# nyashiki/nshogi-engine

Hardware: NVIDIA B200
Metric: nn_leaf_evals_per_sec_batch256 (higher is better)
Workload: dtype bf16

## Files before the change

include/nsb_diag.h:

```cpp
#ifndef NSB_DIAG_H
#define NSB_DIAG_H

#include "nsb.h"

#ifdef __cplusplus
extern "C" {
#endif
#if defined(__GNUC__)
#pragma GCC visibility push(default)
#endif

int nsb_debug_trunk_timeline(nsb_ctx* ctx, int slot, const nsb_feature_bitboard* d_features, size_t n,
                             uint64_t* host_stamps, size_t max_stamps);
int nsb_debug_trunk_timeline_positions(nsb_ctx* ctx, int slot, const nsb_position* d_positions, size_t n,
                                       uint64_t* host_stamps, size_t max_stamps);

int nsb_debug_umma_probe(int gpu, int n_cols, int k_elems, int shift_rows, int layout, int iters,
                         float* max_err, double* cycles_per_mma);

int nsb_debug_bulk_rate_probe(int gpu, int ctas, int tile_bytes, int stages, int split, double* bytes_per_cycle);

#if defined(__GNUC__)
#pragma GCC visibility pop
#endif
#ifdef __cplusplus
}
#endif
#endif
```

nshogi-engine_b200/binding.py:

```python
from __future__ import annotations

import ctypes as C
import os
from typing import Optional

import numpy as np

HERE = os.path.dirname(os.path.abspath(__file__))
LIB_PATH = os.path.join(HERE, "libnsb.so")

NUM_SQUARES = 81
POLICY_SIZE = 2187
FEATURE_CHANNELS = 86
MAX_LEGAL_MOVES = 593
CACHE_MAX_MOVES = 164
DECODE_PROBS = 0
DECODE_LOGITS = 1
DECODE_BOTH = 2
DECODE_NAN_FALLBACK = 0x100
ROW_SKIP_SOFTMAX = 1

FEATURE_BITBOARD = np.dtype([("lo", "<u8"), ("hi", "<u8")])
POSITION = np.dtype(
    {
        "names": ["board", "side", "hands", "ply", "max_ply", "black_draw_value", "white_draw_value"],
        "formats": [("u1", (81,)), "u1", ("u1", (2, 7)), "<u2", "<u2", "<f4", "<f4"],
        "offsets": [0, 81, 82, 96, 98, 100, 104],
        "itemsize": 108,
    }
)


class NetDesc(C.Structure):
    _fields_ = [("in_channels", C.c_int32), ("channels", C.c_int32), ("blocks", C.c_int32),
                ("value_hidden", C.c_int32)]


class NsbError(RuntimeError):
    pass


_lib = None

_P = C.c_void_p
SIGNATURES = {
    "nsb_create": (C.c_int, [C.POINTER(_P), C.c_int, C.c_int, C.c_int, C.POINTER(NetDesc)]),
    "nsb_destroy": (None, [_P]),
    "nsb_bind_thread": (C.c_int, [_P]),
    "nsb_weight_blob_floats": (C.c_size_t, [C.POINTER(NetDesc)]),
    "nsb_weight_blob_random": (C.c_int, [C.POINTER(NetDesc), C.c_uint64, _P]),
    "nsb_load_weights": (C.c_int, [_P, _P, C.c_size_t]),
    "nsb_eval_async": (C.c_int, [_P, C.c_int, _P, C.c_size_t, _P, _P, _P]),
    "nsb_eval_decode_async": (C.c_int, [_P, C.c_int, _P, C.c_size_t, _P, _P, C.c_int, _P, _P, _P, _P]),
    "nsb_eval_positions_async": (C.c_int, [_P, C.c_int, _P, C.c_size_t, _P, _P, _P]),
    "nsb_eval_positions_decode_async": (C.c_int, [_P, C.c_int, _P, C.c_size_t, _P, _P, C.c_int, _P, _P, _P, _P]),
    "nsb_await": (C.c_int, [_P, C.c_int]),
    "nsb_is_computing": (C.c_int, [_P, C.c_int]),
    "nsb_eval_device": (C.c_int, [_P, C.c_int, _P, C.c_size_t, _P, _P, _P]),
    "nsb_eval_decode_device": (C.c_int, [_P, C.c_int, _P, C.c_size_t, _P, _P, C.c_int, _P, _P, _P, _P, _P]),
    "nsb_extract_device": (C.c_int, [_P, C.c_int, _P, C.c_size_t, C.c_int, C.c_int, _P]),
    "nsb_pack_positions_device": (C.c_int, [_P, C.c_int, _P, C.c_size_t, _P]),
    "nsb_decode_device": (C.c_int, [_P, C.c_int, _P, _P, _P, C.c_size_t, _P, _P, C.c_int, _P, _P]),
    "nsb_decode_device_ex": (C.c_int, [_P, C.c_int, _P, _P, _P, C.c_size_t, _P, _P, C.c_int, _P, _P, _P, _P]),
    "nsb_cache_create": (C.c_int, [_P, C.c_size_t]),
    "nsb_cache_clear": (C.c_int, [_P]),
    "nsb_cache_num_bundles": (C.c_uint64, [_P]),
    "nsb_cache_store_device": (C.c_int, [_P, C.c_int, _P, C.c_size_t, _P, _P, _P, _P, _P, _P]),
    "nsb_cache_probe_device": (C.c_int, [_P, C.c_int, _P, C.c_size_t, _P, _P, _P, _P, _P, _P, _P]),
    "nsb_eval_cached_decode_async": (C.c_int, [_P, C.c_int, _P, C.c_size_t, _P, _P, _P, C.c_int, _P, _P, _P, _P, _P]),
    "nsb_eval_positions_cached_decode_async": (C.c_int, [_P, C.c_int, _P, C.c_size_t, _P, _P, _P, C.c_int, _P, _P, _P, _P,
                                                         _P]),
    "nsb_eval_cached_decode_device": (C.c_int, [_P, C.c_int, _P, C.c_size_t, _P, _P, _P, C.c_int, _P, _P, _P, _P, _P]),
    "nsb_stream": (_P, [_P, C.c_int]),
    "nsb_set_timing": (C.c_int, [_P, C.c_int]),
    "nsb_trunk_time": (C.c_int, [_P, C.POINTER(C.c_double), C.POINTER(C.c_uint64)]),
    "nsb_trunk_time_reset": (C.c_int, [_P]),
    "nsb_launch_count": (C.c_uint64, [_P]),
    "nsb_trunk_kernel_name": (C.c_char_p, [_P]),
    "nsb_host_register": (C.c_int, [_P, C.c_size_t]),
    "nsb_host_unregister": (C.c_int, [_P]),
    "nsb_eval_request_async": (C.c_int, [_P, C.c_int, _P]),
    "nsb_cache_attach": (C.c_int, [_P, _P]),
    "nsb_set_io_mode": (C.c_int, [_P, C.c_int]),
    "nsb_io_mode": (C.c_int, [_P]),
    "nsb_host_alloc": (C.c_int, [C.POINTER(_P), C.c_size_t]),
    "nsb_host_free": (C.c_int, [_P]),
    "nsb_host_alloc_near": (C.c_int, [C.POINTER(_P), C.c_size_t, C.c_int]),
    "nsb_gpu_numa_node": (C.c_int, [C.c_int]),
    "nsb_numa_bind_thread": (C.c_int, [C.c_int]),
    "nsb_device_alloc": (C.c_int, [C.POINTER(_P), C.c_size_t]),
    "nsb_device_free": (C.c_int, [_P]),
    "nsb_memcpy_h2d": (C.c_int, [_P, _P, C.c_size_t]),
    "nsb_memcpy_d2h": (C.c_int, [_P, _P, C.c_size_t]),
    "nsb_memset_device": (C.c_int, [_P, C.c_int, C.c_size_t]),
    "nsb_device_sync": (C.c_int, []),
    "nsb_last_error": (C.c_char_p, []),
    "nsb_version": (C.c_char_p, []),
    "nsb_device_count": (C.c_int, []),
    "nsb_umma_selftest": (C.c_int, [C.c_int, C.c_int, C.c_int, C.c_int, C.POINTER(C.c_float), C.POINTER(C.c_float)]),
    "nsb_event_create": (C.c_int, [C.POINTER(_P)]),
    "nsb_event_destroy": (C.c_int, [_P]),
    "nsb_event_record": (C.c_int, [_P, _P, C.c_int]),
    "nsb_event_sync": (C.c_int, [_P]),
    "nsb_event_elapsed_ms": (C.c_int, [_P, _P, C.POINTER(C.c_float)]),
}


DIAG_SIGNATURES = {
    "nsb_debug_trunk_timeline": (C.c_int, [_P, C.c_int, _P, C.c_size_t, _P, C.c_size_t]),
    "nsb_debug_trunk_timeline_positions": (C.c_int, [_P, C.c_int, _P, C.c_size_t, _P, C.c_size_t]),
    "nsb_debug_umma_probe": (C.c_int, [C.c_int, C.c_int, C.c_int, C.c_int, C.c_int, C.c_int, C.POINTER(C.c_float),
                                       C.POINTER(C.c_double)]),
    "nsb_debug_bulk_rate_probe": (C.c_int, [C.c_int, C.c_int, C.c_int, C.c_int, C.c_int, C.POINTER(C.c_double)]),
}
DIAG_LIB_PATH = os.path.join(HERE, "libnsb_diag.so")
_diag = None


def diag_lib() -> C.CDLL:
    global _diag
    if _diag is None:
        if not os.path.exists(DIAG_LIB_PATH):
            raise NsbError(f"{DIAG_LIB_PATH} not built")
        l = C.CDLL(DIAG_LIB_PATH)
        for name, (res, args) in {**SIGNATURES, **DIAG_SIGNATURES}.items():
            fn = getattr(l, name)
            fn.restype = res
            fn.argtypes = args
        _diag = l
    return _diag


def lib() -> C.CDLL:
    global _lib
    if _lib is None:
        if not os.path.exists(LIB_PATH):
            raise NsbError(f"{LIB_PATH} not built: run `python -c 'import __graft_entry__ as g; g.build()'` "
                           "(there is no CPU fallback)")
        l = C.CDLL(LIB_PATH)
        for name, (res, args) in SIGNATURES.items():
            fn = getattr(l, name)
            fn.restype = res
            fn.argtypes = args
        _lib = l
    return _lib


def _check(rc: int, what: str) -> None:
    if rc != 0:
        msg = lib().nsb_last_error().decode()
        if _diag is not None and _diag.nsb_last_error():
            msg = msg or _diag.nsb_last_error().decode()
        raise NsbError(f"{what} failed ({rc}): {msg}")


def _ptr(a) -> Optional[int]:
    if a is None:
        return None
    if isinstance(a, np.ndarray):
        assert a.flags["C_CONTIGUOUS"], "host buffers must be C-contiguous"
        return a.ctypes.data
    return int(a)


def device_count() -> int:
    return lib().nsb_device_count()


def net_desc(channels: int, blocks: int, value_hidden: int = 256, in_channels: int = FEATURE_CHANNELS) -> NetDesc:
    return NetDesc(in_channels, channels, blocks, value_hidden)


def random_blob(desc: NetDesc, seed: int) -> np.ndarray:
    n = lib().nsb_weight_blob_floats(C.byref(desc))
    blob = np.empty(n, dtype=np.float32)
    _check(lib().nsb_weight_blob_random(C.byref(desc), seed, blob.ctypes.data), "nsb_weight_blob_random")
    return blob


class PinnedArray:

    def __init__(self, shape, dtype, gpu: Optional[int] = None):
        self.dtype = np.dtype(dtype)
        self.shape = tuple(shape) if isinstance(shape, (tuple, list)) else (int(shape),)
        nbytes = int(np.prod(self.shape)) * self.dtype.itemsize
        p = _P()
        if gpu is None:
            _check(lib().nsb_host_alloc(C.byref(p), nbytes), "nsb_host_alloc")
        else:
            _check(lib().nsb_host_alloc_near(C.byref(p), nbytes, gpu), "nsb_host_alloc_near")
        self._p = p
        buf = (C.c_uint8 * max(nbytes, 1)).from_address(p.value)
        self.array = np.frombuffer(buf, dtype=self.dtype, count=int(np.prod(self.shape))).reshape(self.shape)

    def free(self):
        if self._p is not None:
            self.array = None
            lib().nsb_host_free(self._p)
            self._p = None


class DecodeRequest(C.Structure):
    _fields_ = [("features", _P), ("positions", _P), ("n", C.c_size_t), ("hashes", _P), ("move_off", _P), ("move_idx", _P),
                ("mode", C.c_int), ("legal_out", _P), ("order_out", _P), ("win", _P), ("draw", _P), ("nan_flag", _P),
                ("hit_flag", _P), ("row_flags", _P), ("logits_out", _P)]


def host_register(arr: np.ndarray) -> bool:
    rc = lib().nsb_host_register(arr.ctypes.data, arr.nbytes)
    if rc < 0:
        _check(rc, "nsb_host_register")
    return rc == 0


def host_unregister(arr: np.ndarray):
    _check(lib().nsb_host_unregister(arr.ctypes.data), "nsb_host_unregister")


class DeviceBuffer:
    def __init__(self, nbytes: int):
        p = _P()
        _check(lib().nsb_device_alloc(C.byref(p), nbytes), "nsb_device_alloc")
        self.ptr = p.value
        self.nbytes = nbytes

    @classmethod
    def from_host(cls, a: np.ndarray) -> "DeviceBuffer":
        a = np.ascontiguousarray(a)
        d = cls(max(a.nbytes, 1))
        if a.nbytes:
            _check(lib().nsb_memcpy_h2d(d.ptr, a.ctypes.data, a.nbytes), "nsb_memcpy_h2d")
        return d

    def to_host(self, shape, dtype) -> np.ndarray:
        out = np.empty(shape, dtype=dtype)
        assert out.nbytes <= self.nbytes
        if out.nbytes:
            _check(lib().nsb_memcpy_d2h(out.ctypes.data, self.ptr, out.nbytes), "nsb_memcpy_d2h")
        return out

    def fill(self, byte: int):
        _check(lib().nsb_memset_device(self.ptr, byte, self.nbytes), "nsb_memset_device")

    def free(self):
        if self.ptr:
            lib().nsb_device_free(self.ptr)
            self.ptr = None


def gpu_numa_node(gpu: int = 0) -> int:
    return lib().nsb_gpu_numa_node(gpu)


def numa_bind_thread(gpu: int = 0) -> bool:
    return lib().nsb_numa_bind_thread(gpu) == 0


def device_sync():
    _check(lib().nsb_device_sync(), "nsb_device_sync")


def umma_selftest(n_cols: int, k_elems: int, shift_rows: int, gpu: int = 0):
    err, epi = C.c_float(-1.0), C.c_float(-1.0)
    _check(lib().nsb_umma_selftest(gpu, n_cols, k_elems, shift_rows, C.byref(err), C.byref(epi)),
           "nsb_umma_selftest")
    return float(err.value), float(epi.value)


def umma_probe(n_cols, k_elems, shift_rows, layout, iters=20, gpu=0):
    err, cyc = C.c_float(-1.0), C.c_double(0)
    _check(diag_lib().nsb_debug_umma_probe(gpu, n_cols, k_elems, shift_rows, layout, iters, C.byref(err), C.byref(cyc)),
           "nsb_debug_umma_probe")
    return float(err.value), float(cyc.value)


def bulk_rate_probe(ctas, tile_bytes, stages, split, gpu=0):
    v = C.c_double(0)
    _check(diag_lib().nsb_debug_bulk_rate_probe(gpu, ctas, tile_bytes, stages, split, C.byref(v)), "nsb_debug_bulk_rate_probe")
    return float(v.value)


class Event:

    def __init__(self):
        p = _P()
        _check(lib().nsb_event_create(C.byref(p)), "nsb_event_create")
        self._p = p

    def record(self, ctx: "Context", slot: int = 0):
        _check(ctx._l.nsb_event_record(self._p, ctx._h, slot), "nsb_event_record")

    def sync(self):
        _check(lib().nsb_event_sync(self._p), "nsb_event_sync")

    def elapsed_ms(self, stop: "Event") -> float:
        ms = C.c_float(0)
        _check(lib().nsb_event_elapsed_ms(self._p, stop._p, C.byref(ms)), "nsb_event_elapsed_ms")
        return float(ms.value)

    def destroy(self):
        if self._p is not None:
            lib().nsb_event_destroy(self._p)
            self._p = None


class Context:

    def __init__(self, desc: NetDesc, batch_max: int, slots: int = 1, gpu: int = 0,
                 blob: Optional[np.ndarray] = None, seed: Optional[int] = None, diag: bool = False):
        self.desc = desc
        self.batch_max = batch_max
        self.slots = slots
        self._l = diag_lib() if diag else lib()
        h = _P()
        _check(self._l.nsb_create(C.byref(h), gpu, batch_max, slots, C.byref(desc)), "nsb_create")
        self._h = h
        if blob is None and seed is not None:
            blob = random_blob(desc, seed)
        if blob is not None:
            self.load_weights(blob)

    def close(self):
        if self._h is not None:
            self._l.nsb_destroy(self._h)
            self._h = None

    def __enter__(self):
        return self

    def __exit__(self, *a):
        self.close()

    def load_weights(self, blob: np.ndarray):
        blob = np.ascontiguousarray(blob, dtype=np.float32)
        _check(self._l.nsb_load_weights(self._h, blob.ctypes.data, blob.size), "nsb_load_weights")

    def bind_thread(self):
        _check(self._l.nsb_bind_thread(self._h), "nsb_bind_thread")

    def eval_async(self, slot, features, n, policy, win, draw):
        _check(self._l.nsb_eval_async(self._h, slot, _ptr(features), n, _ptr(policy), _ptr(win), _ptr(draw)),
               "nsb_eval_async")

    def eval_decode_async(self, slot, features, n, move_off, move_idx, mode, legal_out, win, draw, nan_flag=None):
        _check(self._l.nsb_eval_decode_async(self._h, slot, _ptr(features), n, _ptr(move_off), _ptr(move_idx), mode,
                                           _ptr(legal_out), _ptr(win), _ptr(draw), _ptr(nan_flag)),
               "nsb_eval_decode_async")

    def eval_positions_async(self, slot, positions, n, policy, win, draw):
        _check(self._l.nsb_eval_positions_async(self._h, slot, _ptr(positions), n, _ptr(policy), _ptr(win),
                                              _ptr(draw)), "nsb_eval_positions_async")

    def eval_positions_decode_async(self, slot, positions, n, move_off, move_idx, mode, legal_out, win, draw,
                                    nan_flag=None):
        _check(self._l.nsb_eval_positions_decode_async(self._h, slot, _ptr(positions), n, _ptr(move_off),
                                                     _ptr(move_idx), mode, _ptr(legal_out), _ptr(win), _ptr(draw),
                                                     _ptr(nan_flag)), "nsb_eval_positions_decode_async")

    def await_(self, slot=0):
        _check(self._l.nsb_await(self._h, slot), "nsb_await")

    def is_computing(self, slot=0) -> bool:
        rc = self._l.nsb_is_computing(self._h, slot)
        if rc < 0:
            _check(rc, "nsb_is_computing")
        return rc == 1

    def eval_device(self, slot, d_features, n, d_policy, d_win, d_draw):
        _check(self._l.nsb_eval_device(self._h, slot, _ptr(d_features), n, _ptr(d_policy), _ptr(d_win), _ptr(d_draw)),
               "nsb_eval_device")

    def eval_decode_device(self, slot, d_features, n, d_off, d_idx, mode, d_policy, d_legal, d_win, d_draw, d_flag):
        _check(self._l.nsb_eval_decode_device(self._h, slot, _ptr(d_features), n, _ptr(d_off), _ptr(d_idx), mode,
                                            _ptr(d_policy), _ptr(d_legal), _ptr(d_win), _ptr(d_draw), _ptr(d_flag)),
               "nsb_eval_decode_device")

    def extract_device(self, slot, d_features, n, channels, channels_first, d_planes):
        _check(self._l.nsb_extract_device(self._h, slot, _ptr(d_features), n, channels, int(channels_first),
                                        _ptr(d_planes)), "nsb_extract_device")

    def pack_positions_device(self, slot, d_positions, n, d_features):
        _check(self._l.nsb_pack_positions_device(self._h, slot, _ptr(d_positions), n, _ptr(d_features)),
               "nsb_pack_positions_device")

    def decode_device(self, slot, d_policy, d_win, d_draw, n, d_off, d_idx, mode, d_legal, d_flag):
        _check(self._l.nsb_decode_device(self._h, slot, _ptr(d_policy), _ptr(d_win), _ptr(d_draw), n, _ptr(d_off),
                                       _ptr(d_idx), mode, _ptr(d_legal), _ptr(d_flag)), "nsb_decode_device")

    def decode_device_ex(self, slot, d_policy, d_win, d_draw, n, d_off, d_idx, mode, d_row_flags, d_legal, d_logits, d_flag):
        _check(self._l.nsb_decode_device_ex(self._h, slot, _ptr(d_policy), _ptr(d_win), _ptr(d_draw), n, _ptr(d_off),
                                          _ptr(d_idx), mode, _ptr(d_row_flags), _ptr(d_legal), _ptr(d_logits), _ptr(d_flag)),
               "nsb_decode_device_ex")

    def cache_create(self, memory_mb: int):
        _check(self._l.nsb_cache_create(self._h, memory_mb), "nsb_cache_create")

    def cache_clear(self):
        _check(self._l.nsb_cache_clear(self._h), "nsb_cache_clear")

    def cache_num_bundles(self) -> int:
        return int(self._l.nsb_cache_num_bundles(self._h))

    def cache_store_device(self, slot, d_hashes, n, d_off, d_legal, d_win, d_draw, d_skip=None, d_stored=None):
        _check(self._l.nsb_cache_store_device(self._h, slot, _ptr(d_hashes), n, _ptr(d_off), _ptr(d_legal), _ptr(d_win),
                                            _ptr(d_draw), _ptr(d_skip), _ptr(d_stored)), "nsb_cache_store_device")

    def cache_probe_device(self, slot, d_hashes, n, d_off, d_legal, d_win, d_draw, d_hit, d_miss_idx, d_miss_count):
        _check(self._l.nsb_cache_probe_device(self._h, slot, _ptr(d_hashes), n, _ptr(d_off), _ptr(d_legal), _ptr(d_win),
                                            _ptr(d_draw), _ptr(d_hit), _ptr(d_miss_idx), _ptr(d_miss_count)),
               "nsb_cache_probe_device")

    def eval_cached_decode_async(self, slot, features, n, hashes, move_off, move_idx, mode, legal_out, win, draw,
                                 nan_flag=None, hit_flag=None):
        _check(self._l.nsb_eval_cached_decode_async(self._h, slot, _ptr(features), n, _ptr(hashes), _ptr(move_off),
                                                  _ptr(move_idx), mode, _ptr(legal_out), _ptr(win), _ptr(draw),
                                                  _ptr(nan_flag), _ptr(hit_flag)), "nsb_eval_cached_decode_async")

    def eval_positions_cached_decode_async(self, slot, positions, n, hashes, move_off, move_idx, mode, legal_out, win,
                                           draw, nan_flag=None, hit_flag=None):
        _check(self._l.nsb_eval_positions_cached_decode_async(self._h, slot, _ptr(positions), n, _ptr(hashes),
                                                            _ptr(move_off), _ptr(move_idx), mode, _ptr(legal_out),
                                                            _ptr(win), _ptr(draw), _ptr(nan_flag), _ptr(hit_flag)),
               "nsb_eval_positions_cached_decode_async")

    def eval_cached_decode_device(self, slot, d_features, n, d_hashes, d_off, d_idx, mode, d_legal, d_win, d_draw,
                                  d_flag, d_hit):
        _check(self._l.nsb_eval_cached_decode_device(self._h, slot, _ptr(d_features), n, _ptr(d_hashes), _ptr(d_off),
                                                   _ptr(d_idx), mode, _ptr(d_legal), _ptr(d_win), _ptr(d_draw),
                                                   _ptr(d_flag), _ptr(d_hit)), "nsb_eval_cached_decode_device")

    def debug_trunk_timeline(self, slot, d_features, n, positions=False):
        nl = 2 * self.desc.blocks + 2
        out = np.zeros(nl * 4 + 16 + 3 * 1024, dtype=np.uint64)
        fn = self._l.nsb_debug_trunk_timeline_positions if positions else self._l.nsb_debug_trunk_timeline
        _check(fn(self._h, slot, _ptr(d_features), n, out.ctypes.data, out.size), "nsb_debug_trunk_timeline")
        return out[:nl * 4].reshape(nl, 4), out[nl * 4:]

    def eval_request_async(self, slot, n, move_off, move_idx, mode, legal_out, win, draw, features=None, positions=None,
                           hashes=None, order_out=None, nan_flag=None, hit_flag=None, row_flags=None, logits_out=None):
        r = DecodeRequest(_ptr(features), _ptr(positions), n, _ptr(hashes), _ptr(move_off), _ptr(move_idx), mode,
                          _ptr(legal_out), _ptr(order_out), _ptr(win), _ptr(draw), _ptr(nan_flag), _ptr(hit_flag),
                          _ptr(row_flags), _ptr(logits_out))
        _check(self._l.nsb_eval_request_async(self._h, slot, C.byref(r)), "nsb_eval_request_async")

    def cache_attach(self, owner: "Context"):
        _check(self._l.nsb_cache_attach(self._h, owner._h), "nsb_cache_attach")

    def set_io_mode(self, direct: bool):
        _check(self._l.nsb_set_io_mode(self._h, 1 if direct else 0), "nsb_set_io_mode")

    def io_mode(self) -> str:
        return "direct" if self._l.nsb_io_mode(self._h) == 1 else "staged"

    def stream(self, slot=0) -> int:
        return self._l.nsb_stream(self._h, slot) or 0

    def set_timing(self, on: bool):
        _check(self._l.nsb_set_timing(self._h, int(on)), "nsb_set_timing")

    def trunk_time(self):
        s, n = C.c_double(0), C.c_uint64(0)
        _check(self._l.nsb_trunk_time(self._h, C.byref(s), C.byref(n)), "nsb_trunk_time")
        return float(s.value), int(n.value)

    def trunk_time_reset(self):
        _check(self._l.nsb_trunk_time_reset(self._h), "nsb_trunk_time_reset")

    def trunk_kernel_name(self) -> str:
        return self._l.nsb_trunk_kernel_name(self._h).decode()

    def launch_count(self) -> int:
        return int(self._l.nsb_launch_count(self._h))
```

nshogi-engine_b200/csrc/epilogue.cuh:

```cuda
#pragma once
#include <stdint.h>

#include "umma.cuh"

namespace nsb {

__host__ __device__ constexpr bool is_real_slot(int n) { return (n % 100) < 90 && ((n % 100) % 10) < 9; }

template <int NCG>
struct EpilogueMask {
    uint32_t m[NCG * 4];
    template <int COL0>
    __device__ __forceinline__ void init_at(int lane) {
#pragma unroll
        for (int G = 0; G < NCG * 4; ++G) {
            uint32_t v = 0;
#pragma unroll
            for (int q4 = 0; q4 < 4; ++q4) {
                const int n = COL0 + 8 * G + 2 * q4;
                const uint32_t c = (is_real_slot(n) ? 0x0000FFFFu : 0u) | (is_real_slot(n + 1) ? 0xFFFF0000u : 0u);
                v = (lane & 3) == q4 ? c : v;
            }
            m[G] = v;
        }
    }
    __device__ __forceinline__ void init(int col0, int lane) {
        if (col0 == 0) init_at<0>(lane);
        else init_at<96>(lane);
    }
};

template <int NCG, bool kResidual, int LBS = 2>
__device__ __forceinline__ void epilogue_half(int lb, uint32_t taddr, uint32_t buf, uint32_t pitch, int chunk0,
                                              int col0, const float (&bias)[4], const EpilogueMask<NCG>& mask,
                                              int lane) {
    const int mk = lane >> 3, mi = lane & 7;
    uint32_t v[NCG][16];
#pragma unroll
    for (int cg = 0; cg < NCG; ++cg) tmem_ld_16x256b_x4(taddr + ((uint32_t)(lb * 16) << 16) + cg * 32, v[cg]);
    const uint32_t row_addr =
        buf + (uint32_t)(chunk0 + lb * LBS + (mk & 1)) * pitch + (uint32_t)(col0 + 8 * (mk >> 1) + mi) * 16u;
    uint32_t xr[NCG][2][4];
    if (kResidual) {
#pragma unroll
        for (int cg = 0; cg < NCG; ++cg)
#pragma unroll
            for (int h = 0; h < 2; ++h)
                ldmatrix_x4_trans(row_addr + (uint32_t)(cg * 32 + h * 16) * 16u, xr[cg][h][0], xr[cg][h][1],
                                  xr[cg][h][2], xr[cg][h][3]);
    }
    tmem_ld_wait();
    const float b0 = lb ? bias[2] : bias[0], b1 = lb ? bias[3] : bias[1];
    const uint64_t bb0 = pack_f32x2(b0, b0), bb1 = pack_f32x2(b1, b1);
#pragma unroll
    for (int cg = 0; cg < NCG; ++cg)
#pragma unroll
        for (int h = 0; h < 2; ++h) {
            uint32_t p[4];
#pragma unroll
            for (int m = 0; m < 4; ++m) {
                const int g = 2 * h + (m >> 1), rh = m & 1;
                uint64_t x = add_f32x2(pack_u32x2(v[cg][4 * g + 2 * rh + 0], v[cg][4 * g + 2 * rh + 1]), rh ? bb1 : bb0);
                if (kResidual) x = add_f32x2(x, pack_u32x2(xr[cg][h][m] << 16, xr[cg][h][m] & 0xFFFF0000u));
                p[m] = pack_relu_bf16x2(x) & mask.m[cg * 4 + g];
            }
            stmatrix_x4_trans(row_addr + (uint32_t)(cg * 32 + h * 16) * 16u, p[0], p[1], p[2], p[3]);
        }
}

template <int NCG, bool kResidual>
__device__ __forceinline__ void epilogue_warp(uint32_t taddr, uint32_t buf, uint32_t pitch, int chunk0, int col0,
                                              const float (&bias)[4], const EpilogueMask<NCG>& mask, int lane) {
#pragma unroll
    for (int lb = 0; lb < 2; ++lb)
        epilogue_half<NCG, kResidual>(lb, taddr, buf, pitch, chunk0, col0, bias, mask, lane);
}

}
```

nshogi-engine_b200/csrc/nsb_api.cu:

```cuda
#include <cuda_runtime.h>
#include <stdarg.h>
#include <stdio.h>
#include <stdlib.h>
#include <string.h>

#include <map>
#include <mutex>
#include <new>
#include <vector>

#include "nsb_internal.h"
#ifdef NSB_DIAG
#include "../../include/nsb_diag.h"
#endif

namespace nsb {

static thread_local char g_err[512] = "";

void set_error(const char* fmt, ...) {
    va_list ap;
    va_start(ap, fmt);
    vsnprintf(g_err, sizeof g_err, fmt, ap);
    va_end(ap);
}

static std::mutex g_host_mu;
enum class HostKind { Alloc, NodeAlloc, Registered, Adopted };
struct HostRange {
    size_t bytes = 0;
    bool direct = true;
    HostKind kind = HostKind::Alloc;
};
static std::map<uintptr_t, HostRange> g_host_allocs;

static bool host_mapped(const void* p, size_t bytes) {
    if (p == nullptr) return false;
    const uintptr_t a = (uintptr_t)p;
    std::lock_guard<std::mutex> lock(g_host_mu);
    auto it = g_host_allocs.upper_bound(a);
    if (it == g_host_allocs.begin()) return false;
    --it;
    return it->second.direct && a + bytes <= it->first + it->second.bytes;
}

struct Slot {
    cudaStream_t stream = nullptr;
    nsb_feature_bitboard* d_feat = nullptr;
    nsb_position* d_pos = nullptr;
    float *d_policy = nullptr, *d_win = nullptr, *d_draw = nullptr, *d_legal = nullptr;
    uint32_t* d_off = nullptr;
    uint16_t* d_idx = nullptr;
    uint16_t* d_order = nullptr;
    uint8_t* d_flag = nullptr;
    uint8_t* d_rowflags = nullptr;
    float* d_logits = nullptr;
    uint64_t* d_hash = nullptr;
    uint8_t* d_hit = nullptr;
    int* d_miss_idx = nullptr;
    int* d_miss_count = nullptr;
    std::vector<cudaEvent_t> ev;
    size_t ev_used = 0;
};

}

struct nsb_ctx {
    int gpu = 0, batch_max = 0, num_sms = 0;
    int max_pairs = 0;
    bool use_ts = false;
    bool direct_io = false;
    bool fuse_pack = true;
    int duo_ctas = 0;
    int cluster128 = 1;
    bool duo_always = false;
    bool quad = false;
    nsb::DeviceNet net_duo{};
    void* d_duo_tiles = nullptr;
    double t_classic_wave = 0.129, t_duo_single = 0.157, t_duo_pair = 0.215;
    bool calibrated = false;
    nsb::DeviceCache cache{};
    bool cache_owned = false;
    nsb_net_desc desc{};
    bool loaded = false, timing = false;
    nsb::DeviceNet net{};
    void* d_weights[6] = {nullptr, nullptr, nullptr, nullptr, nullptr, nullptr};
    std::vector<nsb::Slot> slots;
    uint64_t launches = 0;
    double trunk_ms = 0.0;
    uint64_t trunk_launches = 0;
};

using namespace nsb;

#define NSB_CUDA(call)                                                                        \
    do {                                                                                      \
        cudaError_t e__ = (call);                                                             \
        if (e__ != cudaSuccess) {                                                             \
            set_error("%s failed: %s (%s:%d)", #call, cudaGetErrorString(e__), __FILE__, __LINE__); \
            return NSB_ERR_CUDA;                                                              \
        }                                                                                     \
    } while (0)

static int check_ctx(nsb_ctx* c, int slot) {
    if (!c) {
        set_error("null ctx");
        return NSB_ERR_INVALID;
    }
    if (slot < 0 || slot >= (int)c->slots.size()) {
        set_error("slot %d out of range [0,%d)", slot, (int)c->slots.size());
        return NSB_ERR_INVALID;
    }
    return 0;
}

static int check_batch(nsb_ctx* c, size_t n, bool need_weights) {
    if (n > (size_t)c->batch_max) {
        set_error("batch %zu exceeds batch_max %d", n, c->batch_max);
        return NSB_ERR_INVALID;
    }
    if (need_weights && !c->loaded) {
        set_error("weights not loaded (call nsb_load_weights first)");
        return NSB_ERR_STATE;
    }
    return 0;
}

static bool mode_ok(int mode) {
    const int kind = mode & NSB_DECODE_MODE_MASK;
    return (mode & ~(NSB_DECODE_MODE_MASK | NSB_DECODE_NAN_FALLBACK)) == 0 &&
           (kind == NSB_DECODE_PROBS || kind == NSB_DECODE_LOGITS || kind == NSB_DECODE_BOTH);
}

static int check_offsets(const uint32_t* off, size_t n, const char* who) {
    if (off[0] != 0) {
        set_error("%s: move_off must start at 0", who);
        return NSB_ERR_INVALID;
    }
    for (size_t i = 0; i < n; ++i) {
        if (off[i + 1] < off[i] || off[i + 1] - off[i] > (uint32_t)NSB_MAX_LEGAL_MOVES) {
            set_error("%s: move_off[%zu..%zu] = %u..%u: rows must hold 0..%d moves", who, i, i + 1, off[i], off[i + 1],
                      NSB_MAX_LEGAL_MOVES);
            return NSB_ERR_INVALID;
        }
    }
    return 0;
}

static int check_positions_net(const nsb_ctx* c, const char* who) {
    if (c->desc.in_channels != NSB_FEATURE_CHANNELS) {
        set_error("%s: packed positions expand to the %d planes of SimpleFeatures; this net takes %d channels (feed bitboards)",
                  who, NSB_FEATURE_CHANNELS, c->desc.in_channels);
        return NSB_ERR_INVALID;
    }
    return 0;
}

static bool dense_outputs_mapped(size_t n, const float* policy, const float* win, const float* draw) {
    return host_mapped(policy, n * kPolicySize * sizeof(float)) && host_mapped(win, n * sizeof(float)) &&
           host_mapped(draw, n * sizeof(float));
}

extern "C" {

const char* nsb_last_error(void) { return g_err; }
const char* nsb_version(void) { return "nsb 0.3 (sm_100a: tcgen05 position-stationary trunk, cta_group::2 pair trunk, device-resident eval cache)"
#ifdef NSB_DIAG
           " [diagnostic build]"
#endif
        ; }

int nsb_device_count(void) {
    int n = 0;
    if (cudaGetDeviceCount(&n) != cudaSuccess) {
        cudaGetLastError();
        return 0;
    }
    return n;
}

int nsb_create(nsb_ctx** out, int gpu, int batch_max, int slots, const nsb_net_desc* net) {
    if (!out || !net || batch_max <= 0 || batch_max > 65535 || slots < 1 || slots > 16) {
        set_error("nsb_create: bad arguments (batch_max 1..65535, slots 1..16)");
        return NSB_ERR_INVALID;
    }
    if ((net->channels != 128 && net->channels != 192 && net->channels != 256) || net->blocks < 1 || net->blocks > 80 ||
        net->in_channels < 1 || net->in_channels > kMaxInChannels || net->value_hidden < 1 ||
        net->value_hidden > kMaxHidden) {
        set_error("nsb_create: unsupported net (channels 128|192|256, blocks 1..80, in_channels<=%d, hidden<=%d)",
                  kMaxInChannels, kMaxHidden);
        return NSB_ERR_INVALID;
    }
    int ndev = 0;
    if (cudaGetDeviceCount(&ndev) != cudaSuccess || gpu < 0 || gpu >= ndev) {
        cudaGetLastError();
        set_error("nsb_create: no CUDA device %d (found %d); this library has no CPU fallback", gpu, ndev);
        return NSB_ERR_NO_DEVICE;
    }
    cudaDeviceProp prop;
    NSB_CUDA(cudaGetDeviceProperties(&prop, gpu));
    if (prop.major != 10) {
        set_error("nsb_create: device %d is sm_%d%d; the kernels are built for sm_100a only", gpu, prop.major,
                  prop.minor);
        return NSB_ERR_NO_DEVICE;
    }
    NSB_CUDA(cudaSetDevice(gpu));
    int rc = trunk_fused_prepare(net->channels);
    if (rc) return rc;
    int max_pairs = 0;
    const char* t256 = getenv("NSB_TRUNK256");
    const char* t128 = getenv("NSB_TRUNK128");
#ifndef NSB_DIAG
    if ((t256 && strcmp(t256, "single") == 0) || (t128 && strcmp(t128, "ts") == 0)) {
        set_error("nsb_create: NSB_TRUNK256=single / NSB_TRUNK128=ts exist in the diagnostic build only (libnsb_diag.so)");
        return NSB_ERR_INVALID;
    }
#endif
    if (net->channels == 192 || (net->channels == 256 && !(t256 && strcmp(t256, "single") == 0))) {
        if ((rc = trunk_pair_prepare(net->channels, &max_pairs))) return rc;
        if (max_pairs > prop.multiProcessorCount / 2) max_pairs = prop.multiProcessorCount / 2;
    }
    const bool is128 = net->channels == 128;
    const bool use_ts = is128 && t128 && strcmp(t128, "ts") == 0;
    const int cluster128 = (is128 && t128 && strcmp(t128, "mc2") == 0) ? 2 : (is128 && t128 && strcmp(t128, "mc4") == 0) ? 4 : 1;
    const bool want_quad = is128 && (t128 ? strcmp(t128, "quad") == 0 : slots >= 4);
    const bool want_duo = is128 && !use_ts && !want_quad && (t128 ? strcmp(t128, "duo") == 0 : true);
    const bool duo_always = want_duo && (t128 ? true : slots >= 2);
#ifdef NSB_DIAG
    if (use_ts && (rc = trunk_ts_prepare())) return rc;
#endif
    int duo_ctas = 0;
    if (want_duo && (rc = trunk_duo_prepare(&duo_ctas))) return rc;
    if (want_quad && (rc = trunk_quad_prepare())) return rc;
    nsb_ctx* c = new (std::nothrow) nsb_ctx();
    if (!c) {
        set_error("out of host memory");
        return NSB_ERR_NOMEM;
    }
    c->gpu = gpu;
    c->batch_max = batch_max;
    c->num_sms = prop.multiProcessorCount;
    c->max_pairs = max_pairs;
    c->use_ts = use_ts;
    c->duo_ctas = duo_ctas;
    c->duo_always = duo_always;
    c->quad = want_quad;
    c->cluster128 = cluster128;
    if (const char* dc = getenv("NSB_DUO_CTAS")) c->duo_ctas = duo_ctas > 0 ? atoi(dc) : 0;
    if (const char* fp = getenv("NSB_FUSE_PACK")) c->fuse_pack = strcmp(fp, "0") != 0;
    c->direct_io = slots == 1;
    if (const char* io = getenv("NSB_IO")) c->direct_io = strcmp(io, "direct") == 0;
    c->desc = *net;
    c->slots.resize(slots);
    const size_t B = (size_t)batch_max;
    for (auto& s : c->slots) {
        cudaError_t e = cudaStreamCreateWithFlags(&s.stream, cudaStreamNonBlocking);
        if (e == cudaSuccess) e = cudaMalloc(&s.d_feat, B * (size_t)net->in_channels * sizeof(nsb_feature_bitboard));
        if (e == cudaSuccess) e = cudaMalloc(&s.d_pos, B * sizeof(nsb_position));
        if (e == cudaSuccess) e = cudaMalloc(&s.d_policy, B * kPolicySize * sizeof(float));
        if (e == cudaSuccess) e = cudaMalloc(&s.d_win, B * sizeof(float));
        if (e == cudaSuccess) e = cudaMalloc(&s.d_draw, B * sizeof(float));
        if (e == cudaSuccess) e = cudaMalloc(&s.d_legal, B * NSB_MAX_LEGAL_MOVES * sizeof(float));
        if (e == cudaSuccess) e = cudaMalloc(&s.d_off, (B + 1) * sizeof(uint32_t));
        if (e == cudaSuccess) e = cudaMalloc(&s.d_idx, B * NSB_MAX_LEGAL_MOVES * sizeof(uint16_t));
        if (e == cudaSuccess) e = cudaMalloc(&s.d_order, B * NSB_MAX_LEGAL_MOVES * sizeof(uint16_t));
        if (e == cudaSuccess) e = cudaMalloc(&s.d_flag, B);
        if (e == cudaSuccess) e = cudaMalloc(&s.d_rowflags, B);
        if (e != cudaSuccess) {
            set_error("nsb_create: device allocation failed: %s", cudaGetErrorString(e));
            nsb_destroy(c);
            return e == cudaErrorMemoryAllocation ? NSB_ERR_NOMEM : NSB_ERR_CUDA;
        }
    }
    *out = c;
    return 0;
}

void nsb_destroy(nsb_ctx* c) {
    if (!c) return;
    cudaSetDevice(c->gpu);
    for (auto& s : c->slots) {
        if (s.stream) cudaStreamSynchronize(s.stream);
        cudaFree(s.d_feat); cudaFree(s.d_pos); cudaFree(s.d_policy); cudaFree(s.d_win); cudaFree(s.d_draw);
        cudaFree(s.d_legal); cudaFree(s.d_off); cudaFree(s.d_idx); cudaFree(s.d_order); cudaFree(s.d_flag); cudaFree(s.d_rowflags); cudaFree(s.d_logits);
        cudaFree(s.d_hash); cudaFree(s.d_hit); cudaFree(s.d_miss_idx); cudaFree(s.d_miss_count);
        for (cudaEvent_t e : s.ev) cudaEventDestroy(e);
        if (s.stream) cudaStreamDestroy(s.stream);
    }
    for (void* p : c->d_weights) cudaFree(p);
    cudaFree(c->d_duo_tiles);
    if (c->cache_owned) {
        cudaFree(c->cache.entries);
        cudaFree(c->cache.meta);
    }
    delete c;
}

int nsb_bind_thread(nsb_ctx* c) {
    if (!c) {
        set_error("null ctx");
        return NSB_ERR_INVALID;
    }
    NSB_CUDA(cudaSetDevice(c->gpu));
    return 0;
}

size_t nsb_weight_blob_floats(const nsb_net_desc* net) { return net ? blob_floats(*net) : 0; }

int nsb_weight_blob_random(const nsb_net_desc* net, uint64_t seed, float* blob) {
    if (!net || !blob) {
        set_error("nsb_weight_blob_random: null argument");
        return NSB_ERR_INVALID;
    }
    blob_random(*net, seed, blob);
    return 0;
}

static int calibrate_kernel_choice(nsb_ctx* c);

int nsb_load_weights(nsb_ctx* c, const float* blob, size_t n_floats) {
    if (!c || !blob) {
        set_error("nsb_load_weights: null argument");
        return NSB_ERR_INVALID;
    }
    if (n_floats != blob_floats(c->desc)) {
        set_error("nsb_load_weights: blob has %zu floats, net needs %zu", n_floats, blob_floats(c->desc));
        return NSB_ERR_INVALID;
    }
    NSB_CUDA(cudaSetDevice(c->gpu));
    for (auto& s : c->slots) NSB_CUDA(cudaStreamSynchronize(s.stream));
    c->loaded = false;
    const nsb_net_desc& d = c->desc;
    const int C = d.channels, H = d.value_hidden, NL = 2 * d.blocks + 2;
    int stages = stages_per_pass(d);
    std::vector<uint16_t> tiles((size_t)stages * kStageBytes / 2);
    std::vector<float> bias((size_t)NL * C), fc1t((size_t)81 * H), fc1b(H), fc2(2 * (size_t)H), fc2b(2);
    pack_weights(d, blob, tiles.data(), bias.data(), fc1t.data(), fc1b.data(), fc2.data(), fc2b.data());
    const bool ts_only = c->use_ts || c->quad || (c->duo_ctas > 0 && c->duo_always);
    std::vector<uint16_t> ts_tiles;
    int ts_stages = 0;
    if (ts_only || c->duo_ctas > 0) {
        ts_stages = ts_steps_per_pass(d);
        ts_tiles.assign((size_t)ts_stages * 2048, 0);
        pack_weights_ts(d, blob, ts_tiles.data());
        if (ts_only) {
            stages = ts_stages;
            tiles.swap(ts_tiles);
        }
    }
    const void* src[6] = {tiles.data(), bias.data(), fc1t.data(), fc1b.data(), fc2.data(), fc2b.data()};
    const size_t bytes[6] = {tiles.size() * 2, bias.size() * 4, fc1t.size() * 4, fc1b.size() * 4, fc2.size() * 4,
                             fc2b.size() * 4};
    for (int i = 0; i < 6; ++i) {
        if (c->d_weights[i]) {
            cudaFree(c->d_weights[i]);
            c->d_weights[i] = nullptr;
        }
        NSB_CUDA(cudaMalloc(&c->d_weights[i], bytes[i]));
        NSB_CUDA(cudaMemcpy(c->d_weights[i], src[i], bytes[i], cudaMemcpyHostToDevice));
    }
    DeviceNet& n = c->net;
    n.channels = C;
    n.blocks = d.blocks;
    n.in_channels = d.in_channels;
    n.stem_steps = stem_steps(d.in_channels);
    n.hidden = H;
    n.num_layers = NL;
    n.stages_per_pass = stages;
    n.tiles = static_cast<const uint8_t*>(c->d_weights[0]);
    n.bias = static_cast<const float*>(c->d_weights[1]);
    n.fc1t = static_cast<const float*>(c->d_weights[2]);
    n.fc1b = static_cast<const float*>(c->d_weights[3]);
    n.fc2 = static_cast<const float*>(c->d_weights[4]);
    n.fc2b = static_cast<const float*>(c->d_weights[5]);
    if (c->duo_ctas > 0 && !c->duo_always) {
        cudaFree(c->d_duo_tiles);
        c->d_duo_tiles = nullptr;
        NSB_CUDA(cudaMalloc(&c->d_duo_tiles, ts_tiles.size() * 2));
        NSB_CUDA(cudaMemcpy(c->d_duo_tiles, ts_tiles.data(), ts_tiles.size() * 2, cudaMemcpyHostToDevice));
        c->net_duo = n;
        c->net_duo.stages_per_pass = ts_stages;
        c->net_duo.tiles = static_cast<const uint8_t*>(c->d_duo_tiles);
    } else {
        c->net_duo = n;
    }
    c->loaded = true;
    return calibrate_kernel_choice(c);
}

static bool use_duo(const nsb_ctx* c, int n) {
    if (c->duo_ctas <= 0) return false;
    if (c->duo_always) return true;
    const int groups = (n + 1) / 2, sms = c->num_sms;
    const double classic = c->t_classic_wave * ((groups + sms - 1) / sms);
    const int full = groups / (2 * sms), rest = groups % (2 * sms);
    const double duo = c->t_duo_pair * full + (rest == 0 ? 0.0 : rest <= sms ? c->t_duo_single : c->t_duo_pair);
    return duo < classic;
}

static int calibrate_kernel_choice(nsb_ctx* c) {
    const int sms = c->num_sms;
    if (c->duo_ctas <= 0 || c->duo_always || c->batch_max <= 2 * sms) return 0;
    Slot& s = c->slots[0];
    const int n_wave = 2 * sms, n_pair = c->batch_max < 4 * sms ? c->batch_max : 4 * sms;
    NSB_CUDA(cudaMemsetAsync(s.d_feat, 0, (size_t)n_pair * c->desc.in_channels * sizeof(nsb_feature_bitboard), s.stream));
    cudaEvent_t e0, e1;
    NSB_CUDA(cudaEventCreate(&e0));
    NSB_CUDA(cudaEventCreate(&e1));
    auto best_of = [&](bool duo, int n, double* out) -> int {
        EvalArgs a{};
        a.features = s.d_feat;
        a.n = n;
        a.win = s.d_win;
        a.draw = s.d_draw;
        float best = 1e30f;
        for (int it = 0; it < 4; ++it) {
            NSB_CUDA(cudaEventRecord(e0, s.stream));
            const int k = duo ? launch_trunk_duo(c->net_duo, a, sms, c->duo_ctas, s.stream) : launch_trunk_fused(c->net, a, sms, s.stream);
            if (k < 0) return k;
            NSB_CUDA(cudaGetLastError());
            NSB_CUDA(cudaEventRecord(e1, s.stream));
            NSB_CUDA(cudaEventSynchronize(e1));
            float ms = 0.f;
            NSB_CUDA(cudaEventElapsedTime(&ms, e0, e1));
            if (it > 0 && ms < best) best = ms;
        }
        *out = best;
        return 0;
    };
    int rc = best_of(false, n_wave, &c->t_classic_wave);
    if (!rc) rc = best_of(true, n_wave, &c->t_duo_single);
    if (!rc) rc = best_of(true, n_pair, &c->t_duo_pair);
    cudaEventDestroy(e0);
    cudaEventDestroy(e1);
    c->calibrated = rc == 0;
    return rc;
}


static int run_trunk(nsb_ctx* c, Slot& s, const EvalArgs& a) {
    if (c->timing) {
        while (s.ev.size() < s.ev_used + 2) {
            cudaEvent_t e;
            NSB_CUDA(cudaEventCreate(&e));
            s.ev.push_back(e);
        }
        NSB_CUDA(cudaEventRecord(s.ev[s.ev_used], s.stream));
    }
    int k = c->max_pairs > 0 ? launch_trunk_pair(c->net, a, c->max_pairs, s.stream)
            : c->quad        ? launch_trunk_quad(c->net, a, c->num_sms, s.stream)
            : use_duo(c, a.n) ? launch_trunk_duo(c->net_duo, a, c->num_sms, c->duo_ctas, s.stream)
#ifdef NSB_DIAG
            : c->use_ts      ? launch_trunk_ts(c->net, a, c->num_sms, s.stream)
#endif
                             : launch_trunk_fused(c->net, a, c->num_sms, s.stream, c->cluster128);
    if (k < 0) return k;
    NSB_CUDA(cudaGetLastError());
    c->launches += (uint64_t)k;
    if (c->timing) {
        NSB_CUDA(cudaEventRecord(s.ev[s.ev_used + 1], s.stream));
        s.ev_used += 2;
    }
    return 0;
}

static int harvest_timing(nsb_ctx* c, Slot& s) {
    for (size_t i = 0; i + 1 < s.ev_used; i += 2) {
        float ms = 0.f;
        NSB_CUDA(cudaEventElapsedTime(&ms, s.ev[i], s.ev[i + 1]));
        c->trunk_ms += ms;
        c->trunk_launches += 1;
    }
    s.ev_used = 0;
    return 0;
}


int nsb_eval_async(nsb_ctx* c, int slot, const nsb_feature_bitboard* features, size_t n, float* policy,
                   float* win, float* draw) {
    int rc = check_ctx(c, slot);
    if (rc) return rc;
    if ((rc = check_batch(c, n, true))) return rc;
    if (!features || !policy || !win || !draw) {
        set_error("nsb_eval_async: null buffer");
        return NSB_ERR_INVALID;
    }
    if (n == 0) return 0;
    Slot& s = c->slots[slot];
    if (c->direct_io && host_mapped(features, n * (size_t)c->desc.in_channels * sizeof(nsb_feature_bitboard)) &&
        dense_outputs_mapped(n, policy, win, draw)) {
        EvalArgs a{};
        a.features = features;
        a.n = (int)n;
        a.policy = policy;
        a.win = win;
        a.draw = draw;
        return run_trunk(c, s, a);
    }
    NSB_CUDA(cudaMemcpyAsync(s.d_feat, features, n * (size_t)c->desc.in_channels * sizeof(nsb_feature_bitboard),
                             cudaMemcpyHostToDevice, s.stream));
    EvalArgs a{};
    a.features = s.d_feat;
    a.n = (int)n;
    a.policy = s.d_policy;
    a.win = s.d_win;
    a.draw = s.d_draw;
    if ((rc = run_trunk(c, s, a))) return rc;
    NSB_CUDA(cudaMemcpyAsync(policy, s.d_policy, n * kPolicySize * sizeof(float), cudaMemcpyDeviceToHost,
                             s.stream));
    NSB_CUDA(cudaMemcpyAsync(win, s.d_win, n * sizeof(float), cudaMemcpyDeviceToHost, s.stream));
    NSB_CUDA(cudaMemcpyAsync(draw, s.d_draw, n * sizeof(float), cudaMemcpyDeviceToHost, s.stream));
    return 0;
}

static bool decode_buffers_mapped(size_t n, size_t total, const uint32_t* move_off, const uint16_t* move_idx,
                                  const float* legal_out, const float* win, const float* draw, const uint8_t* nan_flag) {
    return host_mapped(move_off, (n + 1) * sizeof(uint32_t)) && host_mapped(move_idx, (total ? total : 1) * sizeof(uint16_t)) &&
           host_mapped(legal_out, (total ? total : 1) * sizeof(float)) && host_mapped(win, n * sizeof(float)) &&
           host_mapped(draw, n * sizeof(float)) && (nan_flag == nullptr || host_mapped(nan_flag, n));
}

static int stage1(nsb_ctx* c, Slot& s, size_t n, const nsb_position** fused) {
    if (c->fuse_pack) {
        *fused = s.d_pos;
        return 0;
    }
    *fused = nullptr;
    int k = launch_pack_positions(s.d_pos, n, s.d_feat, s.stream);
    if (k < 0) return k;
    NSB_CUDA(cudaGetLastError());
    c->launches += (uint64_t)k;
    return 0;
}

static int eval_request(nsb_ctx* c, int slot, const nsb_decode_request& r, const char* who);

int nsb_eval_request_async(nsb_ctx* c, int slot, const nsb_decode_request* request) {
    if (!request) {
        set_error("nsb_eval_request_async: null request");
        return NSB_ERR_INVALID;
    }
    return eval_request(c, slot, *request, "nsb_eval_request_async");
}

int nsb_eval_decode_async(nsb_ctx* c, int slot, const nsb_feature_bitboard* features, size_t n,
                          const uint32_t* move_off, const uint16_t* move_idx, int mode, float* legal_out,
                          float* win, float* draw, uint8_t* nan_flag) {
    nsb_decode_request r{};
    r.features = features;
    r.n = n;
    r.move_off = move_off;
    r.move_idx = move_idx;
    r.mode = mode;
    r.legal_out = legal_out;
    r.win = win;
    r.draw = draw;
    r.nan_flag = nan_flag;
    if (!features) {
        set_error("nsb_eval_decode_async: null buffer or bad mode");
        return NSB_ERR_INVALID;
    }
    return eval_request(c, slot, r, "nsb_eval_decode_async");
}

int nsb_eval_positions_async(nsb_ctx* c, int slot, const nsb_position* positions, size_t n, float* policy,
                             float* win, float* draw) {
    int rc = check_ctx(c, slot);
    if (rc) return rc;
    if ((rc = check_batch(c, n, true))) return rc;
    if (!positions || !policy || !win || !draw) {
        set_error("nsb_eval_positions_async: null buffer");
        return NSB_ERR_INVALID;
    }
    if ((rc = check_positions_net(c, "nsb_eval_positions_async"))) return rc;
    if (n == 0) return 0;
    Slot& s = c->slots[slot];
    if (c->direct_io && c->fuse_pack && host_mapped(positions, n * sizeof(nsb_position)) &&
        dense_outputs_mapped(n, policy, win, draw)) {
        EvalArgs a{};
        a.positions = positions;
        a.n = (int)n;
        a.policy = policy;
        a.win = win;
        a.draw = draw;
        return run_trunk(c, s, a);
    }
    NSB_CUDA(cudaMemcpyAsync(s.d_pos, positions, n * sizeof(nsb_position), cudaMemcpyHostToDevice, s.stream));
    const nsb_position* fused = nullptr;
    if ((rc = stage1(c, s, n, &fused))) return rc;
    EvalArgs a{};
    a.features = s.d_feat;
    a.positions = fused;
    a.n = (int)n;
    a.policy = s.d_policy;
    a.win = s.d_win;
    a.draw = s.d_draw;
    if ((rc = run_trunk(c, s, a))) return rc;
    NSB_CUDA(cudaMemcpyAsync(policy, s.d_policy, n * kPolicySize * sizeof(float), cudaMemcpyDeviceToHost, s.stream));
    NSB_CUDA(cudaMemcpyAsync(win, s.d_win, n * sizeof(float), cudaMemcpyDeviceToHost, s.stream));
    NSB_CUDA(cudaMemcpyAsync(draw, s.d_draw, n * sizeof(float), cudaMemcpyDeviceToHost, s.stream));
    return 0;
}

int nsb_eval_positions_decode_async(nsb_ctx* c, int slot, const nsb_position* positions, size_t n,
                                    const uint32_t* move_off, const uint16_t* move_idx, int mode,
                                    float* legal_out, float* win, float* draw, uint8_t* nan_flag) {
    nsb_decode_request r{};
    r.positions = positions;
    r.n = n;
    r.move_off = move_off;
    r.move_idx = move_idx;
    r.mode = mode;
    r.legal_out = legal_out;
    r.win = win;
    r.draw = draw;
    r.nan_flag = nan_flag;
    if (!positions) {
        set_error("nsb_eval_positions_decode_async: null buffer or bad mode");
        return NSB_ERR_INVALID;
    }
    return eval_request(c, slot, r, "nsb_eval_positions_decode_async");
}

int nsb_await(nsb_ctx* c, int slot) {
    int rc = check_ctx(c, slot);
    if (rc) return rc;
    Slot& s = c->slots[slot];
    NSB_CUDA(cudaStreamSynchronize(s.stream));
    return harvest_timing(c, s);
}

int nsb_is_computing(nsb_ctx* c, int slot) {
    int rc = check_ctx(c, slot);
    if (rc) return rc;
    cudaError_t e = cudaStreamQuery(c->slots[slot].stream);
    if (e == cudaSuccess) return 0;
    if (e == cudaErrorNotReady) return 1;
    set_error("cudaStreamQuery failed: %s", cudaGetErrorString(e));
    return NSB_ERR_CUDA;
}


int nsb_eval_device(nsb_ctx* c, int slot, const nsb_feature_bitboard* d_features, size_t n, float* d_policy,
                    float* d_win, float* d_draw) {
    int rc = check_ctx(c, slot);
    if (rc) return rc;
    if (n > 65535u * 64u) {
        set_error("nsb_eval_device: n too large");
        return NSB_ERR_INVALID;
    }
    if (!c->loaded) {
        set_error("weights not loaded");
        return NSB_ERR_STATE;
    }
    if (!d_features || !d_win || !d_draw) {
        set_error("nsb_eval_device: null buffer");
        return NSB_ERR_INVALID;
    }
    if (n == 0) return 0;
    EvalArgs a{};
    a.features = d_features;
    a.n = (int)n;
    a.policy = d_policy;
    a.win = d_win;
    a.draw = d_draw;
    return run_trunk(c, c->slots[slot], a);
}

int nsb_eval_decode_device(nsb_ctx* c, int slot, const nsb_feature_bitboard* d_features, size_t n,
                           const uint32_t* d_move_off, const uint16_t* d_move_idx, int mode, float* d_policy,
                           float* d_legal_out, float* d_win, float* d_draw, uint8_t* d_nan_flag) {
    int rc = check_ctx(c, slot);
    if (rc) return rc;
    if (!c->loaded) {
        set_error("weights not loaded");
        return NSB_ERR_STATE;
    }
    if (!d_features || !d_win || !d_draw || !d_move_off || !d_move_idx || !d_legal_out || !mode_ok(mode)) {
        set_error("nsb_eval_decode_device: null buffer or bad mode");
        return NSB_ERR_INVALID;
    }
    if (n == 0) return 0;
    EvalArgs a{};
    a.features = d_features;
    a.n = (int)n;
    a.policy = d_policy;
    a.win = d_win;
    a.draw = d_draw;
    a.move_off = d_move_off;
    a.move_idx = d_move_idx;
    a.legal_out = d_legal_out;
    a.nan_flag = d_nan_flag;
    a.decode_mode = mode;
    return run_trunk(c, c->slots[slot], a);
}


int nsb_cache_create(nsb_ctx* c, size_t memory_mb) {
    int rc = check_ctx(c, 0);
    if (rc) return rc;
    if (memory_mb == 0 || memory_mb > 160 * 1024) {
        set_error("nsb_cache_create: memory_mb must be in 1..163840");
        return NSB_ERR_INVALID;
    }
    if (c->cache.num_bundles) {
        set_error("nsb_cache_create: this ctx already has a cache");
        return NSB_ERR_STATE;
    }
    NSB_CUDA(cudaSetDevice(c->gpu));
    const unsigned long long bundles = (unsigned long long)memory_mb * 1024ull * 1024ull / (3ull * sizeof(CacheEntry) + 4ull);
    DeviceCache dc{};
    dc.num_bundles = bundles;
    cudaError_t e = cudaMalloc(&dc.entries, bundles * 3ull * sizeof(CacheEntry));
    if (e == cudaSuccess) e = cudaMalloc(&dc.meta, bundles * sizeof(uint32_t));
    const size_t B = (size_t)c->batch_max;
    for (auto& s : c->slots) {
        if (e == cudaSuccess) e = cudaMalloc(&s.d_hash, B * sizeof(uint64_t));
        if (e == cudaSuccess) e = cudaMalloc(&s.d_hit, B);
        if (e == cudaSuccess) e = cudaMalloc(&s.d_miss_idx, B * sizeof(int));
        if (e == cudaSuccess) e = cudaMalloc(&s.d_miss_count, sizeof(int));
    }
    if (e != cudaSuccess) {
        cudaFree(dc.entries);
        cudaFree(dc.meta);
        set_error("nsb_cache_create: device allocation of %zu MiB failed: %s", memory_mb, cudaGetErrorString(e));
        return e == cudaErrorMemoryAllocation ? NSB_ERR_NOMEM : NSB_ERR_CUDA;
    }
    c->cache = dc;
    c->cache_owned = true;
    return nsb_cache_clear(c);
}

int nsb_cache_attach(nsb_ctx* c, nsb_ctx* owner) {
    int rc = check_ctx(c, 0);
    if (rc) return rc;
    if (!owner || owner == c || !owner->cache.num_bundles || owner->gpu != c->gpu) {
        set_error("nsb_cache_attach: the owner must be another ctx of the same device that has a cache");
        return NSB_ERR_INVALID;
    }
    if (c->cache.num_bundles) {
        set_error("nsb_cache_attach: this ctx already has a cache");
        return NSB_ERR_STATE;
    }
    NSB_CUDA(cudaSetDevice(c->gpu));
    const size_t B = (size_t)c->batch_max;
    cudaError_t e = cudaSuccess;
    for (auto& s : c->slots) {
        if (e == cudaSuccess) e = cudaMalloc(&s.d_hash, B * sizeof(uint64_t));
        if (e == cudaSuccess) e = cudaMalloc(&s.d_hit, B);
        if (e == cudaSuccess) e = cudaMalloc(&s.d_miss_idx, B * sizeof(int));
        if (e == cudaSuccess) e = cudaMalloc(&s.d_miss_count, sizeof(int));
    }
    if (e != cudaSuccess) {
        set_error("nsb_cache_attach: device allocation failed: %s", cudaGetErrorString(e));
        return e == cudaErrorMemoryAllocation ? NSB_ERR_NOMEM : NSB_ERR_CUDA;
    }
    c->cache = owner->cache;
    c->cache_owned = false;
    return 0;
}

int nsb_cache_clear(nsb_ctx* c) {
    int rc = check_ctx(c, 0);
    if (rc) return rc;
    if (!c->cache.num_bundles) {
        set_error("nsb_cache_clear: no cache (call nsb_cache_create)");
        return NSB_ERR_STATE;
    }
    for (auto& s : c->slots) NSB_CUDA(cudaStreamSynchronize(s.stream));
    int k = launch_cache_clear(c->cache, c->slots[0].stream);
    NSB_CUDA(cudaGetLastError());
    c->launches += (uint64_t)k;
    NSB_CUDA(cudaStreamSynchronize(c->slots[0].stream));
    return 0;
}

const char* nsb_trunk_kernel_name(nsb_ctx* c) {
    if (!c) return "";
    if (c->max_pairs > 0)
        return c->desc.channels == 192 ? "trunk_pair_kernel (192 ch, cta_group::2 CTA pair, Cout halves padded to 128 rows)"
                                       : "trunk_pair_kernel (256 ch, cta_group::2 CTA pair)";
    if (c->quad) return "trunk_quad_kernel (128 ch, 4 positions per CTA, weights via TMEM, 1 CTA per SM)";
    if (c->duo_ctas > 0 && c->duo_always) {
        static thread_local char name[96];
        snprintf(name, sizeof name, "trunk_duo_kernel (128 ch, weights via TMEM, %d CTA%s per SM)", c->duo_ctas,
                 c->duo_ctas == 1 ? "" : "s");
        return name;
    }
    if (c->duo_ctas > 0) return "trunk_fused_kernel<128> (trunk_duo_kernel for batches where two CTAs per SM are faster)";
    if (c->use_ts) return "trunk_ts_kernel (128 ch, weights via TMEM, experimental)";
    return c->desc.channels == 128 ? "trunk_fused_kernel<128>" : "trunk_fused_kernel<256>";
}

uint64_t nsb_cache_num_bundles(nsb_ctx* c) { return c ? (uint64_t)c->cache.num_bundles : 0; }

static int check_cache(nsb_ctx* c, int slot, const char* who) {
    int rc = check_ctx(c, slot);
    if (rc) return rc;
    if (!c->cache.num_bundles) {
        set_error("%s: no cache (call nsb_cache_create)", who);
        return NSB_ERR_STATE;
    }
    return 0;
}

int nsb_cache_store_device(nsb_ctx* c, int slot, const uint64_t* d_hashes, size_t n, const uint32_t* d_move_off,
                           const float* d_legal, const float* d_win, const float* d_draw, const uint8_t* d_skip,
                           uint8_t* d_stored) {
    int rc = check_cache(c, slot, "nsb_cache_store_device");
    if (rc) return rc;
    if (!d_hashes || !d_move_off || !d_legal || !d_win || !d_draw) {
        set_error("nsb_cache_store_device: null buffer");
        return NSB_ERR_INVALID;
    }
    int k = launch_cache_store(c->cache, d_hashes, n, d_move_off, d_legal, d_win, d_draw, d_skip, d_stored,
                               c->slots[slot].stream);
    NSB_CUDA(cudaGetLastError());
    c->launches += (uint64_t)k;
    return 0;
}

int nsb_cache_probe_device(nsb_ctx* c, int slot, const uint64_t* d_hashes, size_t n, const uint32_t* d_move_off,
                           float* d_legal_out, float* d_win, float* d_draw, uint8_t* d_hit, int* d_miss_idx,
                           int* d_miss_count) {
    int rc = check_cache(c, slot, "nsb_cache_probe_device");
    if (rc) return rc;
    if (!d_hashes || !d_move_off || !d_legal_out || !d_win || !d_draw || !d_hit || !d_miss_idx || !d_miss_count) {
        set_error("nsb_cache_probe_device: null buffer");
        return NSB_ERR_INVALID;
    }
    Slot& s = c->slots[slot];
    NSB_CUDA(cudaMemsetAsync(d_miss_count, 0, sizeof(int), s.stream));
    int k = launch_cache_probe(c->cache, d_hashes, n, d_move_off, d_legal_out, d_win, d_draw, d_hit, nullptr, d_miss_idx,
                               d_miss_count, s.stream);
    NSB_CUDA(cudaGetLastError());
    c->launches += (uint64_t)k;
    return 0;
}

static int eval_cached_enqueue(nsb_ctx* c, Slot& s, const nsb_feature_bitboard* d_features,
                               const nsb_position* d_positions, size_t n,
                               const uint64_t* d_hashes, const uint32_t* d_off, const uint16_t* d_idx, int mode,
                               float* d_legal, float* d_win, float* d_draw, uint8_t* d_nan_flag, uint8_t* d_hit) {
    NSB_CUDA(cudaMemsetAsync(s.d_miss_count, 0, sizeof(int), s.stream));
    int k = launch_cache_probe(c->cache, d_hashes, n, d_off, d_legal, d_win, d_draw, d_hit, d_nan_flag, s.d_miss_idx,
                               s.d_miss_count, s.stream, nullptr, mode);
    NSB_CUDA(cudaGetLastError());
    c->launches += (uint64_t)k;
    EvalArgs a{};
    a.features = d_features;
    a.positions = d_positions;
    a.n = (int)n;
    a.win = d_win;
    a.draw = d_draw;
    a.move_off = d_off;
    a.move_idx = d_idx;
    a.legal_out = d_legal;
    a.nan_flag = d_nan_flag;
    a.decode_mode = mode;
    a.index = s.d_miss_idx;
    a.count = s.d_miss_count;
    a.hashes = d_hashes;
    a.cache = c->cache;
    return run_trunk(c, s, a);
}

int nsb_eval_cached_decode_device(nsb_ctx* c, int slot, const nsb_feature_bitboard* d_features, size_t n,
                                  const uint64_t* d_hashes, const uint32_t* d_move_off, const uint16_t* d_move_idx,
                                  int mode, float* d_legal_out, float* d_win, float* d_draw, uint8_t* d_nan_flag,
                                  uint8_t* d_hit) {
    int rc = check_cache(c, slot, "nsb_eval_cached_decode_device");
    if (rc) return rc;
    if ((rc = check_batch(c, n, true))) return rc;
    if (!d_features || !d_hashes || !d_move_off || !d_move_idx || !d_legal_out || !d_win || !d_draw || !d_hit ||
        !mode_ok(mode)) {
        set_error("nsb_eval_cached_decode_device: null buffer or bad mode");
        return NSB_ERR_INVALID;
    }
    if (n == 0) return 0;
    return eval_cached_enqueue(c, c->slots[slot], d_features, nullptr, n, d_hashes, d_move_off, d_move_idx, mode, d_legal_out, d_win,
                               d_draw, d_nan_flag, d_hit);
}

int nsb_eval_cached_decode_async(nsb_ctx* c, int slot, const nsb_feature_bitboard* features, size_t n,
                                 const uint64_t* hashes, const uint32_t* move_off, const uint16_t* move_idx, int mode,
                                 float* legal_out, float* win, float* draw, uint8_t* nan_flag, uint8_t* hit_flag) {
    nsb_decode_request r{};
    r.features = features;
    r.n = n;
    r.hashes = hashes;
    r.move_off = move_off;
    r.move_idx = move_idx;
    r.mode = mode;
    r.legal_out = legal_out;
    r.win = win;
    r.draw = draw;
    r.nan_flag = nan_flag;
    r.hit_flag = hit_flag;
    int rc = check_cache(c, slot, "nsb_eval_cached_decode_async");
    if (rc) return rc;
    if (!features || !hashes) {
        set_error("nsb_eval_cached_decode_async: null buffer or bad mode");
        return NSB_ERR_INVALID;
    }
    return eval_request(c, slot, r, "nsb_eval_cached_decode_async");
}

int nsb_eval_positions_cached_decode_async(nsb_ctx* c, int slot, const nsb_position* positions, size_t n,
                                           const uint64_t* hashes, const uint32_t* move_off, const uint16_t* move_idx,
                                           int mode, float* legal_out, float* win, float* draw, uint8_t* nan_flag,
                                           uint8_t* hit_flag) {
    nsb_decode_request r{};
    r.positions = positions;
    r.n = n;
    r.hashes = hashes;
    r.move_off = move_off;
    r.move_idx = move_idx;
    r.mode = mode;
    r.legal_out = legal_out;
    r.win = win;
    r.draw = draw;
    r.nan_flag = nan_flag;
    r.hit_flag = hit_flag;
    int rc = check_cache(c, slot, "nsb_eval_positions_cached_decode_async");
    if (rc) return rc;
    if (!positions || !hashes) {
        set_error("nsb_eval_positions_cached_decode_async: null buffer or bad mode");
        return NSB_ERR_INVALID;
    }
    return eval_request(c, slot, r, "nsb_eval_positions_cached_decode_async");
}

static int eval_request(nsb_ctx* c, int slot, const nsb_decode_request& r, const char* who) {
    int rc = r.hashes ? check_cache(c, slot, who) : check_ctx(c, slot);
    if (rc) return rc;
    const size_t n = r.n;
    if ((rc = check_batch(c, n, true))) return rc;
    if ((r.features != nullptr) == (r.positions != nullptr) || !r.move_off || !r.move_idx || !r.legal_out || !r.win || !r.draw ||
        !mode_ok(r.mode)) {
        set_error("%s: null buffer or bad mode", who);
        return NSB_ERR_INVALID;
    }
    if (r.positions && (rc = check_positions_net(c, who))) return rc;
    if (n == 0) return 0;
    if ((rc = check_offsets(r.move_off, n, who))) return rc;
    const size_t total = r.move_off[n];
    const bool both = (r.mode & NSB_DECODE_MODE_MASK) == NSB_DECODE_BOTH;
    const uint8_t* row_flags = both ? r.row_flags : nullptr;
    float* logits_out = both ? r.logits_out : nullptr;
    Slot& s = c->slots[slot];
    const size_t in_bytes = r.features ? n * (size_t)c->desc.in_channels * sizeof(nsb_feature_bitboard) : n * sizeof(nsb_position);
    const void* in = r.features ? (const void*)r.features : (const void*)r.positions;

    EvalArgs a{};
    a.n = (int)n;
    a.decode_mode = r.mode;
    const bool direct = c->direct_io && (r.features || c->fuse_pack) && host_mapped(in, in_bytes) &&
                        decode_buffers_mapped(n, total, r.move_off, r.move_idx, r.legal_out, r.win, r.draw, r.nan_flag) &&
                        (!r.hashes || host_mapped(r.hashes, n * sizeof(uint64_t))) && (!r.hit_flag || host_mapped(r.hit_flag, n)) &&
                        (!r.order_out || host_mapped(r.order_out, (total ? total : 1) * sizeof(uint16_t))) &&
                        (!row_flags || host_mapped(row_flags, n)) &&
                        (!logits_out || host_mapped(logits_out, (total ? total : 1) * sizeof(float)));
    const uint64_t* hashes = r.hashes;
    uint8_t* hit = r.hit_flag ? r.hit_flag : s.d_hit;
    if (direct) {
        a.features = r.features;
        a.positions = r.positions;
        a.win = r.win;
        a.draw = r.draw;
        a.move_off = r.move_off;
        a.move_idx = r.move_idx;
        a.legal_out = r.legal_out;
        a.order_out = r.order_out;
        a.nan_flag = r.nan_flag ? r.nan_flag : (r.hashes ? s.d_flag : nullptr);
        a.row_flags = row_flags;
        a.logits_out = logits_out;
    } else {
        NSB_CUDA(cudaMemcpyAsync(r.features ? (void*)s.d_feat : (void*)s.d_pos, in, in_bytes, cudaMemcpyHostToDevice, s.stream));
        a.features = s.d_feat;
        if (r.positions && (rc = stage1(c, s, n, &a.positions))) return rc;
        if (r.hashes) {
            NSB_CUDA(cudaMemcpyAsync(s.d_hash, r.hashes, n * sizeof(uint64_t), cudaMemcpyHostToDevice, s.stream));
            hashes = s.d_hash;
            hit = s.d_hit;
        }
        NSB_CUDA(cudaMemcpyAsync(s.d_off, r.move_off, (n + 1) * sizeof(uint32_t), cudaMemcpyHostToDevice, s.stream));
        if (total)
            NSB_CUDA(cudaMemcpyAsync(s.d_idx, r.move_idx, total * sizeof(uint16_t), cudaMemcpyHostToDevice, s.stream));
        a.win = s.d_win;
        a.draw = s.d_draw;
        a.move_off = s.d_off;
        a.move_idx = s.d_idx;
        a.legal_out = s.d_legal;
        a.order_out = r.order_out ? s.d_order : nullptr;
        a.nan_flag = s.d_flag;
        if (row_flags) {
            NSB_CUDA(cudaMemcpyAsync(s.d_rowflags, row_flags, n, cudaMemcpyHostToDevice, s.stream));
            a.row_flags = s.d_rowflags;
        }
        if (logits_out) {
            if (!s.d_logits) NSB_CUDA(cudaMalloc(&s.d_logits, (size_t)c->batch_max * NSB_MAX_LEGAL_MOVES * sizeof(float)));
            a.logits_out = s.d_logits;
        }
    }
    if (r.hashes) {
        NSB_CUDA(cudaMemsetAsync(s.d_miss_count, 0, sizeof(int), s.stream));
        int k = launch_cache_probe(c->cache, hashes, n, a.move_off, a.legal_out, a.win, a.draw, hit, a.nan_flag, s.d_miss_idx,
                                   s.d_miss_count, s.stream, a.order_out, r.mode, a.row_flags, a.logits_out);
        NSB_CUDA(cudaGetLastError());
        c->launches += (uint64_t)k;
        a.index = s.d_miss_idx;
        a.count = s.d_miss_count;
        a.hashes = hashes;
        a.cache = c->cache;
    }
    if ((rc = run_trunk(c, s, a))) return rc;
    if (direct) return 0;
    if (total) {
        NSB_CUDA(cudaMemcpyAsync(r.legal_out, s.d_legal, total * sizeof(float), cudaMemcpyDeviceToHost, s.stream));
        if (r.order_out)
            NSB_CUDA(cudaMemcpyAsync(r.order_out, s.d_order, total * sizeof(uint16_t), cudaMemcpyDeviceToHost, s.stream));
        if (logits_out)
            NSB_CUDA(cudaMemcpyAsync(logits_out, s.d_logits, total * sizeof(float), cudaMemcpyDeviceToHost, s.stream));
    }
    NSB_CUDA(cudaMemcpyAsync(r.win, s.d_win, n * sizeof(float), cudaMemcpyDeviceToHost, s.stream));
    NSB_CUDA(cudaMemcpyAsync(r.draw, s.d_draw, n * sizeof(float), cudaMemcpyDeviceToHost, s.stream));
    if (r.nan_flag) NSB_CUDA(cudaMemcpyAsync(r.nan_flag, s.d_flag, n, cudaMemcpyDeviceToHost, s.stream));
    if (r.hashes && r.hit_flag) NSB_CUDA(cudaMemcpyAsync(r.hit_flag, s.d_hit, n, cudaMemcpyDeviceToHost, s.stream));
    return 0;
}

#ifdef NSB_DIAG
static int debug_timeline(nsb_ctx* c, int slot, const nsb_feature_bitboard* d_features, const nsb_position* d_positions,
                          size_t n, uint64_t* host_stamps, size_t max_stamps) {
    int rc = check_ctx(c, slot);
    if (rc) return rc;
    if (!c->loaded || (!d_features && !d_positions) || !host_stamps || n == 0) {
        set_error("nsb_debug_trunk_timeline: bad arguments or weights not loaded");
        return NSB_ERR_INVALID;
    }
    const size_t need = (size_t)c->net.num_layers * 4 + 16 + 3 * 1024;
    if (max_stamps < need) {
        set_error("nsb_debug_trunk_timeline: need room for %zu stamps", need);
        return NSB_ERR_INVALID;
    }
    Slot& s = c->slots[slot];
    unsigned long long* d_t = nullptr;
    NSB_CUDA(cudaMalloc(&d_t, need * 8));
    NSB_CUDA(cudaMemsetAsync(d_t, 0, need * 8, s.stream));
    EvalArgs a{};
    a.features = d_features;
    a.positions = d_positions;
    a.n = (int)n;
    a.policy = s.d_policy;
    a.win = s.d_win;
    a.draw = s.d_draw;
    a.timeline = d_t;
    if (n > (size_t)c->batch_max) {
        cudaFree(d_t);
        set_error("nsb_debug_trunk_timeline: n exceeds batch_max");
        return NSB_ERR_INVALID;
    }
    rc = run_trunk(c, s, a);
    if (rc == 0) {
        cudaError_t e = cudaStreamSynchronize(s.stream);
        if (e == cudaSuccess) e = cudaMemcpy(host_stamps, d_t, need * 8, cudaMemcpyDeviceToHost);
        if (e != cudaSuccess) {
            set_error("nsb_debug_trunk_timeline: %s", cudaGetErrorString(e));
            rc = NSB_ERR_CUDA;
        }
    }
    cudaFree(d_t);
    return rc;
}

int nsb_debug_trunk_timeline(nsb_ctx* c, int slot, const nsb_feature_bitboard* d_features, size_t n,
                             uint64_t* host_stamps, size_t max_stamps) {
    return debug_timeline(c, slot, d_features, nullptr, n, host_stamps, max_stamps);
}

int nsb_debug_trunk_timeline_positions(nsb_ctx* c, int slot, const nsb_position* d_positions, size_t n,
                                       uint64_t* host_stamps, size_t max_stamps) {
    return debug_timeline(c, slot, nullptr, d_positions, n, host_stamps, max_stamps);
}

#endif

int nsb_extract_device(nsb_ctx* c, int slot, const nsb_feature_bitboard* d_features, size_t n, int channels,
                       int channels_first, float* d_planes) {
    int rc = check_ctx(c, slot);
    if (rc) return rc;
    if (!d_features || !d_planes || channels < 1 || channels > 1024) {
        set_error("nsb_extract_device: bad arguments");
        return NSB_ERR_INVALID;
    }
    int k = launch_extract(d_features, n, channels, channels_first, d_planes, c->slots[slot].stream);
    if (k < 0) return k;
    NSB_CUDA(cudaGetLastError());
    c->launches += (uint64_t)k;
    return 0;
}

int nsb_pack_positions_device(nsb_ctx* c, int slot, const nsb_position* d_positions, size_t n,
                              nsb_feature_bitboard* d_features) {
    int rc = check_ctx(c, slot);
    if (rc) return rc;
    if (!d_positions || !d_features) {
        set_error("nsb_pack_positions_device: null buffer");
        return NSB_ERR_INVALID;
    }
    int k = launch_pack_positions(d_positions, n, d_features, c->slots[slot].stream);
    if (k < 0) return k;
    NSB_CUDA(cudaGetLastError());
    c->launches += (uint64_t)k;
    return 0;
}

int nsb_decode_device(nsb_ctx* c, int slot, const float* d_policy, const float* d_win, const float* d_draw,
                      size_t n, const uint32_t* d_move_off, const uint16_t* d_move_idx, int mode,
                      float* d_legal_out, uint8_t* d_nan_flag) {
    int rc = check_ctx(c, slot);
    if (rc) return rc;
    return nsb_decode_device_ex(c, slot, d_policy, d_win, d_draw, n, d_move_off, d_move_idx, mode, nullptr, d_legal_out,
                                nullptr, d_nan_flag);
}

int nsb_decode_device_ex(nsb_ctx* c, int slot, const float* d_policy, const float* d_win, const float* d_draw,
                         size_t n, const uint32_t* d_move_off, const uint16_t* d_move_idx, int mode,
                         const uint8_t* d_row_flags, float* d_legal_out, float* d_logits_out, uint8_t* d_nan_flag) {
    int rc = check_ctx(c, slot);
    if (rc) return rc;
    if (!d_policy || !d_win || !d_draw || !d_move_off || !d_move_idx || !d_legal_out || !mode_ok(mode)) {
        set_error("nsb_decode_device: null buffer or bad mode");
        return NSB_ERR_INVALID;
    }
    int k = launch_decode(d_policy, d_win, d_draw, n, d_move_off, d_move_idx, mode, d_legal_out, d_nan_flag,
                          c->slots[slot].stream, d_row_flags, d_logits_out);
    if (k < 0) return k;
    NSB_CUDA(cudaGetLastError());
    c->launches += (uint64_t)k;
    return 0;
}

void* nsb_stream(nsb_ctx* c, int slot) {
    if (check_ctx(c, slot)) return nullptr;
    return c->slots[slot].stream;
}

int nsb_set_timing(nsb_ctx* c, int enabled) {
    if (!c) {
        set_error("null ctx");
        return NSB_ERR_INVALID;
    }
    c->timing = enabled != 0;
    return 0;
}

int nsb_trunk_time(nsb_ctx* c, double* sum_ms, uint64_t* launches) {
    if (!c) {
        set_error("null ctx");
        return NSB_ERR_INVALID;
    }
    if (sum_ms) *sum_ms = c->trunk_ms;
    if (launches) *launches = c->trunk_launches;
    return 0;
}

int nsb_trunk_time_reset(nsb_ctx* c) {
    if (!c) {
        set_error("null ctx");
        return NSB_ERR_INVALID;
    }
    c->trunk_ms = 0.0;
    c->trunk_launches = 0;
    return 0;
}

uint64_t nsb_launch_count(nsb_ctx* c) { return c ? c->launches : 0; }


int nsb_host_alloc(void** out, size_t bytes) {
    if (!out) return NSB_ERR_INVALID;
    NSB_CUDA(cudaHostAlloc(out, bytes ? bytes : 1, cudaHostAllocPortable | cudaHostAllocMapped));
    std::lock_guard<std::mutex> lock(g_host_mu);
    g_host_allocs[(uintptr_t)*out] = HostRange{bytes ? bytes : 1, true, HostKind::Alloc};
    return 0;
}
int nsb_host_alloc_near(void** out, size_t bytes, int gpu) {
    if (!out) return NSB_ERR_INVALID;
    int node = -1;
    void* p = alloc_near_gpu(bytes ? bytes : 1, gpu, &node);
    if (!p) {
        set_error("nsb_host_alloc_near: mmap of %zu bytes failed", bytes);
        return NSB_ERR_NOMEM;
    }
    const cudaError_t e = cudaHostRegister(p, bytes ? bytes : 1, cudaHostRegisterPortable | cudaHostRegisterMapped);
    if (e != cudaSuccess) {
        cudaGetLastError();
        free_near_gpu(p, bytes ? bytes : 1);
        set_error("nsb_host_alloc_near: cudaHostRegister failed: %s", cudaGetErrorString(e));
        return NSB_ERR_CUDA;
    }
    void* dp = nullptr;
    const bool direct = cudaHostGetDevicePointer(&dp, p, 0) == cudaSuccess && dp == p;
    if (!direct) cudaGetLastError();
    std::lock_guard<std::mutex> lock(g_host_mu);
    g_host_allocs[(uintptr_t)p] = HostRange{bytes ? bytes : 1, direct, HostKind::NodeAlloc};
    *out = p;
    return 0;
}
int nsb_gpu_numa_node(int gpu) { return gpu_numa_node(gpu); }
int nsb_numa_bind_thread(int gpu) { return numa_bind_thread_to_gpu(gpu); }
int nsb_host_free(void* p) {
    HostRange r{};
    bool known = false;
    {
        std::lock_guard<std::mutex> lock(g_host_mu);
        auto it = g_host_allocs.find((uintptr_t)p);
        if (it != g_host_allocs.end()) {
            r = it->second;
            known = true;
            g_host_allocs.erase(it);
        }
    }
    if (known && r.kind == HostKind::NodeAlloc) {
        NSB_CUDA(cudaHostUnregister(p));
        free_near_gpu(p, r.bytes);
        return 0;
    }
    NSB_CUDA(cudaFreeHost(p));
    return 0;
}
static std::map<uintptr_t, HostRange>::iterator host_find_locked(const void* p, size_t bytes) {
    const uintptr_t a = (uintptr_t)p;
    auto it = g_host_allocs.upper_bound(a);
    if (it == g_host_allocs.begin()) return g_host_allocs.end();
    --it;
    return a + bytes <= it->first + it->second.bytes ? it : g_host_allocs.end();
}

int nsb_host_register(void* p, size_t bytes) {
    if (!p || bytes == 0) {
        set_error("nsb_host_register: bad arguments");
        return NSB_ERR_INVALID;
    }
    {
        std::lock_guard<std::mutex> lock(g_host_mu);
        auto it = host_find_locked(p, bytes);
        if (it != g_host_allocs.end()) {
            if (it->second.kind != HostKind::Adopted) return NSB_HOST_ALREADY_LOCKED;
            void* dp = nullptr;
            if (cudaHostGetDevicePointer(&dp, p, 0) == cudaSuccess && dp == p) return NSB_HOST_ALREADY_LOCKED;
            cudaGetLastError();
            g_host_allocs.erase(it);
        }
    }
    const cudaError_t e = cudaHostRegister(p, bytes, cudaHostRegisterPortable | cudaHostRegisterMapped);
    const bool adopted = e == cudaErrorHostMemoryAlreadyRegistered;
    if (adopted) {
        cudaGetLastError();
    } else if (e != cudaSuccess) {
        cudaGetLastError();
        set_error("cudaHostRegister failed: %s", cudaGetErrorString(e));
        return NSB_ERR_CUDA;
    }
    void* dp = nullptr;
    const bool direct = cudaHostGetDevicePointer(&dp, p, 0) == cudaSuccess && dp == p;
    if (!direct) cudaGetLastError();
    if (direct || !adopted) {
        std::lock_guard<std::mutex> lock(g_host_mu);
        g_host_allocs[(uintptr_t)p] = HostRange{bytes, direct, adopted ? HostKind::Adopted : HostKind::Registered};
    }
    return adopted ? NSB_HOST_ALREADY_LOCKED : NSB_OK;
}
int nsb_host_unregister(void* p) {
    bool ours = false;
    {
        std::lock_guard<std::mutex> lock(g_host_mu);
        auto it = g_host_allocs.find((uintptr_t)p);
        if (it != g_host_allocs.end() && it->second.kind != HostKind::Alloc && it->second.kind != HostKind::NodeAlloc) {
            ours = it->second.kind == HostKind::Registered;
            g_host_allocs.erase(it);
        }
    }
    if (ours) NSB_CUDA(cudaHostUnregister(p));
    return 0;
}
int nsb_set_io_mode(nsb_ctx* c, int mode) {
    if (!c || (mode != NSB_IO_STAGED && mode != NSB_IO_DIRECT)) {
        set_error("nsb_set_io_mode: bad arguments");
        return NSB_ERR_INVALID;
    }
    c->direct_io = mode == NSB_IO_DIRECT;
    return 0;
}
int nsb_io_mode(nsb_ctx* c) { return c && c->direct_io ? NSB_IO_DIRECT : NSB_IO_STAGED; }
int nsb_device_alloc(void** out, size_t bytes) {
    if (!out) return NSB_ERR_INVALID;
    NSB_CUDA(cudaMalloc(out, bytes ? bytes : 1));
    return 0;
}
int nsb_device_free(void* p) {
    NSB_CUDA(cudaFree(p));
    return 0;
}
int nsb_memcpy_h2d(void* dst, const void* src, size_t bytes) {
    NSB_CUDA(cudaMemcpy(dst, src, bytes, cudaMemcpyHostToDevice));
    return 0;
}
int nsb_memcpy_d2h(void* dst, const void* src, size_t bytes) {
    NSB_CUDA(cudaMemcpy(dst, src, bytes, cudaMemcpyDeviceToHost));
    return 0;
}
int nsb_memset_device(void* dst, int value, size_t bytes) {
    NSB_CUDA(cudaMemset(dst, value, bytes));
    return 0;
}
int nsb_device_sync(void) {
    NSB_CUDA(cudaDeviceSynchronize());
    return 0;
}

int nsb_umma_selftest(int gpu, int n_cols, int k_elems, int shift_rows, float* max_err, float* epi_err) {
    return umma_selftest(gpu, n_cols, k_elems, shift_rows, max_err, epi_err);
}

#ifdef NSB_DIAG
int nsb_debug_umma_probe(int gpu, int n_cols, int k_elems, int shift_rows, int layout, int iters, float* max_err,
                         double* cycles_per_mma) {
    return umma_probe(gpu, n_cols, k_elems, shift_rows, layout, iters, max_err, cycles_per_mma);
}

int nsb_debug_bulk_rate_probe(int gpu, int ctas, int tile_bytes, int stages, int split, double* bytes_per_cycle) {
    return bulk_rate_probe(gpu, ctas, tile_bytes, stages, split, bytes_per_cycle);
}

#endif

int nsb_event_create(void** out) {
    if (!out) return NSB_ERR_INVALID;
    cudaEvent_t e;
    NSB_CUDA(cudaEventCreate(&e));
    *out = e;
    return 0;
}
int nsb_event_destroy(void* ev) {
    NSB_CUDA(cudaEventDestroy(static_cast<cudaEvent_t>(ev)));
    return 0;
}
int nsb_event_record(void* ev, nsb_ctx* c, int slot) {
    int rc = check_ctx(c, slot);
    if (rc) return rc;
    NSB_CUDA(cudaEventRecord(static_cast<cudaEvent_t>(ev), c->slots[slot].stream));
    return 0;
}
int nsb_event_sync(void* ev) {
    NSB_CUDA(cudaEventSynchronize(static_cast<cudaEvent_t>(ev)));
    return 0;
}
int nsb_event_elapsed_ms(void* start, void* stop, float* ms) {
    if (!ms) return NSB_ERR_INVALID;
    NSB_CUDA(cudaEventElapsedTime(ms, static_cast<cudaEvent_t>(start), static_cast<cudaEvent_t>(stop)));
    return 0;
}

}
```

nshogi-engine_b200/csrc/nsb_internal.h:

```cpp
#pragma once
#include <cuda_runtime.h>
#include <stddef.h>
#include <stdint.h>

#include "../../include/nsb.h"

namespace nsb {

constexpr int kSquares = NSB_NUM_SQUARES;
constexpr int kPolicyPlanes = NSB_POLICY_PLANES;
constexpr int kPolicySize = NSB_POLICY_SIZE;
constexpr int kStemCin = 128;
constexpr int kMaxInChannels = 96;
constexpr int kFirstScalarChannel = 82;
__host__ __device__ constexpr int stem_twins(int in_channels) { return in_channels > kFirstScalarChannel ? in_channels - kFirstScalarChannel : 0; }
__host__ __device__ constexpr int stem_steps(int in_channels) { return in_channels + stem_twins(in_channels) <= 96 ? 6 : 8; }
__host__ __device__ constexpr int stem_source_channel(int ci, int in_channels) {
    return ci < in_channels ? ci : (ci < in_channels + stem_twins(in_channels) ? kFirstScalarChannel + (ci - in_channels) : -1);
}
constexpr int kStageBytes = 16384;
constexpr int kMaxHidden = 256;

template <int C>
struct TrunkGeom {
    static_assert(C == 128 || C == 256, "trunk width must be 128 or 256");
    static constexpr int KCH = C / 8;
    static constexpr int NPOS = (C == 128) ? 2 : 1;
    static constexpr int NCOLS = NPOS * 96;
    static constexpr int NHALF = C / 128;
    static constexpr int GUARD = 12;
    static constexpr int SPITCH = (GUARD + NCOLS + 11) | 1;
    static constexpr int BUF_BYTES = ((KCH * SPITCH * 16 + 127) / 128) * 128;
    static constexpr int NSTAGES = 6;
    static constexpr int KC64 = C / 64;
    static constexpr int TMEM_COLS = 256;
    static constexpr int SCRATCH_FLOATS = NPOS * kPolicySize;
    static constexpr int OFF_BUF_A = 0;
    static constexpr int OFF_BUF_B = OFF_BUF_A + BUF_BYTES;
    static constexpr int OFF_RING = OFF_BUF_B + BUF_BYTES;
    static constexpr int OFF_SCRATCH = OFF_RING + NSTAGES * kStageBytes;
    static constexpr int OFF_FEAT = OFF_SCRATCH + ((SCRATCH_FLOATS * 4 + 15) / 16) * 16;
    static constexpr int OFF_VBUF = OFF_FEAT + NPOS * kMaxInChannels * 16;
    static constexpr int OFF_RED = OFF_VBUF + ((NPOS * 81 * 4 + 15) / 16) * 16;
    static constexpr int OFF_BARS = OFF_RED + ((8 * NPOS * 2 * 4 + NPOS * 2 * 4 + 15) / 16) * 16;
    static constexpr int SMEM_BYTES = OFF_BARS + (2 * NSTAGES + 2) * 8 + 16 + 128;
    static_assert(NCOLS % 16 == 0 && NCOLS <= 256, "UMMA N");
    static_assert(NHALF * NCOLS <= TMEM_COLS, "TMEM columns");
    static_assert(SMEM_BYTES <= 232448, "exceeds 227 KB of shared memory");
};

template <int C_>
struct PairGeom {
    static_assert(C_ == 192 || C_ == 256, "pair trunk width must be 192 or 256");
    static constexpr int C = C_;
    static constexpr int KCH = C / 8;
    static constexpr int NCOLS = 96;
    static constexpr int NPAIR = 2 * NCOLS;
    static constexpr int GUARD = 12;
    static constexpr int SPITCH = (GUARD + NCOLS + 11) | 1;
    static constexpr int BUF_BYTES = ((KCH * SPITCH * 16 + 127) / 128) * 128;
    static constexpr int XCH = C / 16;
    static constexpr int QUADS = XCH / 4;
    static constexpr int XROW = 89 * 16;
    static constexpr int XPITCH = (NCOLS + 1) * 16;
    static constexpr int XBUF_BYTES = XCH * XPITCH;
    static constexpr int NSTAGES = C == 256 ? 5 : 7;
    static constexpr int KC64 = C / 64;
    static constexpr int TMEM_COLS = 256;
    static constexpr int NBARS = 2 * NSTAGES + 4;
    static constexpr int OFF_BUF_A = 0;
    static constexpr int OFF_BUF_B = OFF_BUF_A + BUF_BYTES;
    static constexpr int OFF_XBUF = OFF_BUF_B + BUF_BYTES;
    static constexpr int OFF_RING = OFF_XBUF + XBUF_BYTES;
    static constexpr int OFF_FEAT = OFF_RING + NSTAGES * kStageBytes;
    static constexpr int OFF_VBUF = OFF_FEAT + kMaxInChannels * 16;
    static constexpr int OFF_RED = OFF_VBUF + ((81 * 4 + 15) / 16) * 16;
    static constexpr int OFF_BARS = OFF_RED + ((8 * 2 * 4 + 2 * 4 + 15) / 16) * 16;
    static constexpr int SMEM_BYTES = OFF_BARS + NBARS * 8 + 16 + 128;
    static_assert(kPolicySize * 4 <= XBUF_BYTES, "logits scratch aliases the exchange buffer");
    static_assert(SMEM_BYTES <= 232448, "exceeds 227 KB of shared memory");
};

struct DeviceNet {
    int channels;
    int blocks;
    int in_channels;
    int stem_steps;
    int hidden;
    int num_layers;
    int stages_per_pass;
    const uint8_t* tiles;
    const float* bias;
    const float* fc1t;
    const float* fc1b;
    const float* fc2;
    const float* fc2b;
};

struct CacheEntry {
    uint64_t hash;
    uint32_t n;
    uint32_t pad0;
    float win, draw;
    float policy[NSB_CACHE_MAX_MOVES];
    uint32_t pad1[2];
};
static_assert(sizeof(CacheEntry) == 688, "cache entry is 688 bytes (16-byte multiple)");
struct DeviceCache {
    CacheEntry* entries;
    uint32_t* meta;
    unsigned long long num_bundles;
};

struct EvalArgs {
    const nsb_feature_bitboard* features;
    const nsb_position* positions;
    int n;
    float* policy;
    float* win;
    float* draw;
    const uint32_t* move_off;
    const uint16_t* move_idx;
    float* legal_out;
    uint16_t* order_out;
    uint8_t* nan_flag;
    int decode_mode;
    const uint8_t* row_flags;
    float* logits_out;
    unsigned long long* timeline;
    const int* index;
    const int* count;
    const uint64_t* hashes;
    DeviceCache cache;
};

size_t blob_floats(const nsb_net_desc& d);
void blob_random(const nsb_net_desc& d, uint64_t seed, float* blob);
int stages_per_pass(const nsb_net_desc& d);
int ts_steps_per_pass(const nsb_net_desc& d);
void pack_weights_ts(const nsb_net_desc& d, const float* blob, uint16_t* stream);
void pack_weights(const nsb_net_desc& d, const float* blob, uint16_t* tiles, float* bias,
                  float* fc1t, float* fc1b, float* fc2, float* fc2b);

int launch_extract(const nsb_feature_bitboard* d_fb, size_t n, int channels, int channels_first,
                   float* d_planes, cudaStream_t s);
int launch_pack_positions(const nsb_position* d_pos, size_t n, nsb_feature_bitboard* d_fb,
                          cudaStream_t s);
int launch_decode(const float* d_policy, const float* d_win, const float* d_draw, size_t n,
                  const uint32_t* d_off, const uint16_t* d_idx, int mode, float* d_out,
                  uint8_t* d_flag, cudaStream_t s, const uint8_t* d_row_flags = nullptr, float* d_logits_out = nullptr);
int launch_trunk_fused(const DeviceNet& net, const EvalArgs& a, int num_sms, cudaStream_t s, int cluster = 1);
int launch_cache_probe(const DeviceCache& c, const uint64_t* d_hashes, size_t n, const uint32_t* d_off, float* d_legal,
                       float* d_win, float* d_draw, uint8_t* d_hit, uint8_t* d_nan_flag, int* d_miss_idx, int* d_miss_count,
                       cudaStream_t s, uint16_t* d_order = nullptr, int mode = 0, const uint8_t* d_row_flags = nullptr,
                       float* d_logits_out = nullptr);
int launch_cache_store(const DeviceCache& c, const uint64_t* d_hashes, size_t n, const uint32_t* d_off,
                       const float* d_legal, const float* d_win, const float* d_draw, const uint8_t* d_skip,
                       uint8_t* d_stored, cudaStream_t s);
int launch_cache_clear(const DeviceCache& c, cudaStream_t s);
int trunk_fused_prepare(int channels);
int trunk_ts_prepare();
int launch_trunk_ts(const DeviceNet& net, const EvalArgs& a, int num_sms, cudaStream_t s);
int trunk_duo_prepare(int* ctas_per_sm);
int launch_trunk_duo(const DeviceNet& net, const EvalArgs& a, int num_sms, int ctas_per_sm, cudaStream_t s);
int trunk_quad_prepare();
int launch_trunk_quad(const DeviceNet& net, const EvalArgs& a, int num_sms, cudaStream_t s);
int trunk_pair_prepare(int channels, int* max_pairs);
int launch_trunk_pair(const DeviceNet& net, const EvalArgs& a, int max_pairs, cudaStream_t s);
int umma_probe(int gpu, int n_cols, int k_elems, int shift_rows, int layout, int iters, float* max_err,
               double* cycles_per_mma);
int bulk_rate_probe(int gpu, int ctas, int tile_bytes, int stages, int split, double* bytes_per_cycle);
int umma_selftest(int gpu, int n_cols, int k_elems, int shift_rows, float* max_err, float* epi_err);

void set_error(const char* fmt, ...);

int gpu_numa_node(int gpu);
int numa_bind_thread_to_gpu(int gpu);
void* alloc_near_gpu(size_t bytes, int gpu, int* node_out);
void free_near_gpu(void* p, size_t bytes);

}
```

nshogi-engine_b200/csrc/trunk_common.cuh:

```cuda
#pragma once
#include <cuda_bf16.h>
#include <cuda_runtime.h>
#include <stdint.h>

#include "cache_device.cuh"
#include "decode_device.cuh"
#include "epilogue.cuh"
#include "nsb_internal.h"
#include "pack_device.cuh"
#include "umma.cuh"

namespace nsb {

constexpr int kThreads = 384;
constexpr int kEpiThreads = 256;
constexpr int kEpiWarps = kEpiThreads / 32;
constexpr uint32_t kEpiBar = 1;

constexpr int kFcPrefetch = 27;

__device__ __forceinline__ uint4 plane_bits(uint4 f) {
    uint32_t s0 = f.x;
    uint32_t s1 = (f.y & 0x7FFFFFFFu) | (f.z << 31);
    uint32_t s2 = (f.z >> 1) & 0x1FFFFu;
    if ((f.z >> 24) & 1u) {
        const uint32_t r0 = __brev(s2), r1 = __brev(s1), r2 = __brev(s0);
        s0 = __funnelshift_r(r0, r1, 15);
        s1 = __funnelshift_r(r1, r2, 15);
        s2 = r2 >> 15;
    }
    const float v = __uint_as_float(f.w);
    const uint32_t hi = (uint32_t)f32_to_bf16_bits(v);
    const float rest = v - __uint_as_float(hi << 16);
    const uint32_t lo = (rest == rest && (hi & 0x7F80u) != 0x7F80u) ? (uint32_t)f32_to_bf16_bits(rest) : 0u;
    return make_uint4(s0, s1, s2, hi | (lo << 16));
}

__device__ __forceinline__ unsigned long long* eval_timeline(const EvalArgs& a) {
#ifdef NSB_DIAG
    return a.timeline;
#else
    (void)a;
    return nullptr;
#endif
}

__device__ __forceinline__ int eval_count(const EvalArgs& a) { return a.count ? __ldg(a.count) : a.n; }
__device__ __forceinline__ int eval_index(const EvalArgs& a, int li, int n_eff) {
    return li < n_eff ? (a.index ? __ldg(a.index + li) : li) : -1;
}

template <int NPOS, int SPITCH, int GUARD, int NT = kEpiThreads>
__device__ __forceinline__ void expand_features(const DeviceNet& net, const EvalArgs& a, int n_eff, int li0, uint4* featS,
                                                uint8_t* stem_buf, int et, unsigned long long* tl,
                                                uint32_t bar = kEpiBar) {
    const int IN = net.in_channels, stem_chunks = 2 * net.stem_steps;
    if (a.positions != nullptr) {
        const int pos = et >> 5, lane = et & 31;
        if (pos < NPOS) {
            uint4* mine = featS + pos * IN;
            const int b = eval_index(a, li0 + pos, n_eff);
            if (b >= 0) {
                pack_position_warp(a.positions + b, lane, mine, [&](int c, uint4 f) { mine[c] = plane_bits(f); });
            } else {
                for (int c = lane; c < IN; c += 32) mine[c] = make_uint4(0, 0, 0, 0);
            }
        }
    } else {
        for (int i = et; i < NPOS * IN; i += NT) {
            const int pos = i / IN, c = i - pos * IN;
            const int b = eval_index(a, li0 + pos, n_eff);
            uint4 f = make_uint4(0, 0, 0, 0);
            if (b >= 0) f = __ldg(reinterpret_cast<const uint4*>(a.features) + (size_t)b * IN + c);
            featS[i] = plane_bits(f);
        }
    }
    if (tl) tl[9] = clock64();
    named_bar_sync(bar, NT);
    if (tl) tl[3] = clock64();
    for (int item = et; item < NPOS * stem_chunks * 9; item += NT) {
        const int pos = item / (stem_chunks * 9);
        const int r2 = item - pos * (stem_chunks * 9);
        const int j = r2 / 9, row = r2 - j * 9;
        const int bit0 = 9 * row, wi = bit0 >> 5, sh = bit0 & 31;
        uint32_t field[8], val[8];
#pragma unroll
        for (int e = 0; e < 8; ++e) {
            const int c = j * 8 + e;
            uint4 f = make_uint4(0, 0, 0, 0);
            const int src = stem_source_channel(c, IN);
            if (src >= 0) f = featS[pos * IN + src];
            const uint32_t lo = wi == 0 ? f.x : (wi == 1 ? f.y : f.z);
            const uint32_t hi = wi == 0 ? f.y : (wi == 1 ? f.z : 0u);
            field[e] = __funnelshift_r(lo, hi, sh);
            val[e] = c < IN ? (f.w & 0xFFFFu) : (f.w >> 16);
        }
        uint8_t* dst = stem_buf + (size_t)((j * SPITCH + GUARD + pos * 100 + row * 10) * 16);
#pragma unroll
        for (int col = 0; col < 9; ++col) {
            uint32_t w[4];
#pragma unroll
            for (int e2 = 0; e2 < 4; ++e2) {
                const uint32_t a0 = val[2 * e2] & (0u - ((field[2 * e2] >> col) & 1u));
                const uint32_t a1 = val[2 * e2 + 1] & (0u - ((field[2 * e2 + 1] >> col) & 1u));
                w[e2] = a0 | (a1 << 16);
            }
            *reinterpret_cast<uint4*>(dst + col * 16) = make_uint4(w[0], w[1], w[2], w[3]);
        }
    }
    if (tl) tl[10] = clock64();
}

template <int COL0>
__device__ __forceinline__ void head_read(uint32_t taddr, float bias, int hp, float* scratch, float* vbuf, int lane) {
#pragma unroll
    for (int j = 0; j < 3; ++j) {
        uint32_t v[32];
        tmem_ld32(taddr + j * 32, v);
        tmem_ld_wait();
        if (lane < 7) {
            float* dst = hp < kPolicyPlanes ? scratch + hp * 81 : vbuf;
            const bool relu = hp == kPolicyPlanes;
#pragma unroll
            for (int i = 0; i < 32; ++i) {
                const int n = COL0 + j * 32 + i;
                if (is_real_slot(n)) {
                    const int pos = n / 100, m = n % 100, t = (m / 10) * 9 + (m % 10);
                    const float x = __uint_as_float(v[i]) + bias;
                    dst[(relu ? pos * 81 : pos * kPolicySize) + t] = relu ? fmaxf(x, 0.f) : x;
                }
            }
        }
    }
}

__device__ __forceinline__ void fc1_prefetch(const DeviceNet& net, int et, float (&wpre)[kFcPrefetch]) {
    const int H = net.hidden;
#pragma unroll
    for (int t = 0; t < kFcPrefetch; ++t) wpre[t] = et < H ? __ldg(net.fc1t + (size_t)t * H + et) : 0.f;
}

template <int NPOS, int NT>
__device__ __forceinline__ void decode_tail(const EvalArgs& a, int n_eff, int li0, float* scratch, const float* wd, int et,
                                            uint32_t bar = kEpiBar) {
    constexpr int NW = NT / 32;
    const int ew = et >> 5, lane = et & 31;
    if (ew < NPOS) {
        const int b = eval_index(a, li0 + ew, n_eff);
        if (b >= 0) {
            const uint32_t mb = __ldg(a.move_off + b), me = __ldg(a.move_off + b + 1);
            const int m = (int)(me - mb);
            const float w = wd[ew * 2 + 0], d = wd[ew * 2 + 1];
            const int rf = a.row_flags ? (int)__ldg(a.row_flags + b) : 0;
            float* row = scratch + ew * kPolicySize;
            float* lout = a.logits_out ? a.logits_out + mb : nullptr;
            bool nan_found;
            if (a.hashes != nullptr) {
                const uint64_t hash = __ldg(a.hashes + b);
                auto store = [&](const float (&v)[kDecodePerLane]) {
                    cache_store_warp_from(a.cache, hash, m, [&](int k) { return v[k]; }, w, d, lane);
                };
                nan_found = a.order_out ? warp_decode_row<true>(row, a.move_idx + mb, m, a.decode_mode, rf, w, d, a.legal_out + mb, lout, lane, row, store)
                                        : warp_decode_row<false>(row, a.move_idx + mb, m, a.decode_mode, rf, w, d, a.legal_out + mb, lout, lane, nullptr, store);
            } else {
                nan_found = a.order_out ? warp_decode_row<true>(row, a.move_idx + mb, m, a.decode_mode, rf, w, d, a.legal_out + mb, lout, lane, row)
                                        : warp_decode_row<false>(row, a.move_idx + mb, m, a.decode_mode, rf, w, d, a.legal_out + mb, lout, lane);
            }
            if (a.nan_flag && lane == 0) a.nan_flag[b] = nan_found ? 1 : 0;
        }
    }
    if (a.order_out != nullptr) {
        named_bar_sync(bar, NT);
        const int pos = ew % NPOS;
        const int b = eval_index(a, li0 + pos, n_eff);
        uint16_t* ostage = reinterpret_cast<uint16_t*>(scratch + pos * kPolicySize + 608);
        if (b >= 0) {
            const uint32_t mb = __ldg(a.move_off + b), me = __ldg(a.move_off + b + 1);
            rank_row_coop(scratch + pos * kPolicySize, (int)(me - mb), ew / NPOS, NW / NPOS, lane, ostage);
        }
        named_bar_sync(bar, NT);
        if (b >= 0) {
            const uint32_t mb = __ldg(a.move_off + b), me = __ldg(a.move_off + b + 1);
            rank_row_copy_out(ostage, (int)(me - mb), ew / NPOS, NW / NPOS, lane, a.order_out + mb);
        }
    }
}

__device__ __forceinline__ int block_steps(const DeviceNet& net, int L, int kc) { return (L == 0 && kc == 1) ? net.stem_steps - 4 : 4; }

template <int NPOS, int NT>
__device__ __forceinline__ void heads_tail_small(const DeviceNet& net, const EvalArgs& a, int n_eff, int li0,
                                                 float* scratch, const float* vbuf, float* red, int et,
                                                 uint32_t bar = kEpiBar) {
    constexpr int NW = NT / 32;
    const int ew = et >> 5, lane = et & 31;
    const int H = net.hidden;
    if (a.policy != nullptr) {
        for (int idx = et; idx < NPOS * kPolicySize; idx += NT) {
            const int pos = idx / kPolicySize, b = eval_index(a, li0 + pos, n_eff);
            if (b >= 0) a.policy[(size_t)b * kPolicySize + (idx - pos * kPolicySize)] = scratch[idx];
        }
    }
    float o[NPOS][2];
#pragma unroll
    for (int pos = 0; pos < NPOS; ++pos) o[pos][0] = o[pos][1] = 0.f;
    for (int h = et; h < H; h += NT) {
        float acc[NPOS];
        const float b1 = __ldg(net.fc1b + h);
#pragma unroll
        for (int pos = 0; pos < NPOS; ++pos) acc[pos] = b1;
#pragma unroll 9
        for (int t = 0; t < 81; ++t) {
            const float w = __ldg(net.fc1t + (size_t)t * H + h);
#pragma unroll
            for (int pos = 0; pos < NPOS; ++pos) acc[pos] += w * vbuf[pos * 81 + t];
        }
        const float w0 = __ldg(net.fc2 + h), w1 = __ldg(net.fc2 + H + h);
#pragma unroll
        for (int pos = 0; pos < NPOS; ++pos) {
            const float hid = fmaxf(acc[pos], 0.f);
            o[pos][0] += w0 * hid;
            o[pos][1] += w1 * hid;
        }
    }
#pragma unroll
    for (int pos = 0; pos < NPOS; ++pos)
#pragma unroll
        for (int k = 0; k < 2; ++k) {
            const float s = warp_sum(o[pos][k]);
            if (lane == 0) red[(ew * NPOS + pos) * 2 + k] = s;
        }
    named_bar_sync(bar, NT);
    if (et < NPOS * 2) {
        const int pos = et >> 1, k = et & 1;
        float s = __ldg(net.fc2b + k);
#pragma unroll
        for (int qq = 0; qq < NW; ++qq) s += red[(qq * NPOS + pos) * 2 + k];
        const float val = 1.0f / (1.0f + expf(-s));
        red[NW * NPOS * 2 + pos * 2 + k] = val;
        const int b = eval_index(a, li0 + pos, n_eff);
        if (b >= 0) (k == 0 ? a.win : a.draw)[b] = val;
    }
    if (a.move_off != nullptr) {
        named_bar_sync(bar, NT);
        decode_tail<NPOS, NT>(a, n_eff, li0, scratch, red + NW * NPOS * 2, et, bar);
    }
    named_bar_sync(bar, NT);
}

template <int NPOS>
__device__ __forceinline__ void heads_tail(const DeviceNet& net, const EvalArgs& a, int n_eff, int li0, float* scratch,
                                           const float* vbuf, float* red, const float (&wpre)[kFcPrefetch], int et,
                                           unsigned long long* tl) {
    const int ew = et >> 5, lane = et & 31;
    const int H = net.hidden;
    if (a.policy != nullptr) {
        for (int idx = et; idx < NPOS * kPolicySize; idx += kEpiThreads) {
            const int pos = idx / kPolicySize, b = eval_index(a, li0 + pos, n_eff);
            if (b >= 0) a.policy[(size_t)b * kPolicySize + (idx - pos * kPolicySize)] = scratch[idx];
        }
    }
    if (tl) tl[5] = clock64();
    {
        float o[NPOS][2];
#pragma unroll
        for (int pos = 0; pos < NPOS; ++pos) o[pos][0] = o[pos][1] = 0.f;
        if (et < H) {
            const int h = et;
            float acc[NPOS];
            const float b1 = __ldg(net.fc1b + h);
            const float w0 = __ldg(net.fc2 + h), w1 = __ldg(net.fc2 + H + h);
#pragma unroll
            for (int pos = 0; pos < NPOS; ++pos) acc[pos] = b1;
#pragma unroll
            for (int t0 = 0; t0 < 81; t0 += kFcPrefetch) {
                float w[kFcPrefetch];
#pragma unroll
                for (int t = 0; t < kFcPrefetch; ++t)
                    w[t] = t0 == 0 ? wpre[t] : __ldg(net.fc1t + (size_t)(t0 + t) * H + h);
#pragma unroll
                for (int t = 0; t < kFcPrefetch; ++t)
#pragma unroll
                    for (int pos = 0; pos < NPOS; ++pos) acc[pos] += w[t] * vbuf[pos * 81 + t0 + t];
            }
#pragma unroll
            for (int pos = 0; pos < NPOS; ++pos) {
                const float hid = fmaxf(acc[pos], 0.f);
                o[pos][0] = w0 * hid;
                o[pos][1] = w1 * hid;
            }
        }
#pragma unroll
        for (int pos = 0; pos < NPOS; ++pos)
#pragma unroll
            for (int k = 0; k < 2; ++k) {
                const float s = warp_sum(o[pos][k]);
                if (lane == 0) red[(ew * NPOS + pos) * 2 + k] = s;
            }
        named_bar_sync(kEpiBar, kEpiThreads);
        if (et < NPOS * 2) {
            const int pos = et >> 1, k = et & 1;
            float s = __ldg(net.fc2b + k);
#pragma unroll
            for (int qq = 0; qq < kEpiWarps; ++qq) s += red[(qq * NPOS + pos) * 2 + k];
            const float val = 1.0f / (1.0f + expf(-s));
            red[kEpiWarps * NPOS * 2 + pos * 2 + k] = val;
            const int b = eval_index(a, li0 + pos, n_eff);
            if (b >= 0) (k == 0 ? a.win : a.draw)[b] = val;
        }
    }
    if (tl) tl[6] = clock64();
    if (a.move_off != nullptr) {
        named_bar_sync(kEpiBar, kEpiThreads);
        decode_tail<NPOS, kEpiThreads>(a, n_eff, li0, scratch, red + kEpiWarps * NPOS * 2, et);
    }
    named_bar_sync(kEpiBar, kEpiThreads);
    if (tl) tl[7] = clock64();
}

}
```

nshogi-engine_b200/csrc/trunk_tmem.cu:

```cuda
#include <cuda_bf16.h>
#include <cuda_runtime.h>
#include <stdint.h>

#include "trunk_common.cuh"

namespace nsb {

namespace {

template <int NGRP_>
struct TmemGeom {
    static constexpr int C = 128;
    static constexpr int KCH = C / 8;
    static constexpr int NGRP = NGRP_;
    static constexpr int NPOS = 2;
    static constexpr int QPOS = NGRP * NPOS;
    static constexpr int NCOLS = NPOS * 96;
    static constexpr int GUARD = 12;
    static constexpr int SPITCH = (GUARD + NCOLS + 11) | 1;
    static constexpr int BUF_BYTES = ((KCH * SPITCH * 16 + 127) / 128) * 128;
    static constexpr int KC64 = C / 64;
    static constexpr int TMEM_COLS = 256 * NGRP;
    static constexpr int A_COL0 = NGRP * NCOLS;
    static constexpr int A_STAGES = 4 * NGRP;
    static constexpr int A_STAGE_COLS = 16;
    static constexpr int THREADS = 128 * (2 + NGRP);
    static constexpr int GRP_THREADS = 128;
    static constexpr int EPI_WARPS = GRP_THREADS / 32;
    static constexpr int MMA_WARP = 4 + 4 * NGRP;
    static constexpr int MIN_BLOCKS = NGRP == 1 ? 2 : 1;
    static constexpr int PRODUCER_REGS = 72, EPI_REGS = NGRP == 1 ? 128 : 168, MMA_REGS = 40;
    static constexpr int NBARS = 2 * A_STAGES + 2;
    static constexpr int SCRATCH_BYTES = ((NPOS * kPolicySize * 4 + 15) / 16) * 16;
    static constexpr int FEAT_BYTES = NPOS * kMaxInChannels * 16;
    static constexpr int VBUF_BYTES = ((NPOS * 81 * 4 + 15) / 16) * 16;
    static constexpr int RED_BYTES = ((EPI_WARPS * NPOS * 2 * 4 + NPOS * 2 * 4 + 15) / 16) * 16;
    static constexpr int GRP_BYTES = 2 * BUF_BYTES;
    static constexpr int OFF_BUF_A = 0;
    static constexpr int OFF_BUF_B = BUF_BYTES;
    static constexpr int OFF_VBUF = NGRP * GRP_BYTES;
    static constexpr int OFF_RED = OFF_VBUF + NGRP * VBUF_BYTES;
    static constexpr int OFF_BARS = OFF_RED + NGRP * RED_BYTES;
    static constexpr int SMEM_BYTES = OFF_BARS + NBARS * 8 + 16 + 128;
    static_assert(BUF_BYTES == 55040, "each group has the duo kernel's activation layout");
    static_assert(NGRP > 1 || (OFF_VBUF == 110080 && OFF_RED == 110736 && OFF_BARS == 110816 && SMEM_BYTES == 111040),
                  "one group keeps the duo kernel's shared memory map");
    static_assert(SCRATCH_BYTES <= BUF_BYTES && FEAT_BYTES <= BUF_BYTES, "aliases fit into buffer A");
    static_assert(A_COL0 + A_STAGES * A_STAGE_COLS == TMEM_COLS, "accumulators + the ring fill the allocation");
    static_assert(MIN_BLOCKS * (SMEM_BYTES + 1024) <= 233472, "MIN_BLOCKS CTAs per SM");
    static_assert(128 * (PRODUCER_REGS + NGRP * EPI_REGS + MMA_REGS) <= 65536 / MIN_BLOCKS,
                  "re-balanced registers of MIN_BLOCKS CTAs fit the SM");
};

template <int NGRP>
__device__ __forceinline__ void trunk_tmem_body(const DeviceNet& net, const EvalArgs& a) {
    using G = TmemGeom<NGRP>;
    constexpr int C = G::C;
    extern __shared__ uint8_t smem_raw[];
    uint8_t* smem = reinterpret_cast<uint8_t*>(((uintptr_t)smem_raw + 127) & ~(uintptr_t)127);
    const uint32_t sbase = smem_u32(smem);
    const uint32_t bars = sbase + G::OFF_BARS;
    auto bar_afull = [&](int s) { return bars + 8u * s; };
    auto bar_aempty = [&](int s) { return bars + 8u * (G::A_STAGES + s); };
    const uint32_t bar_act = bars + 8u * (2 * G::A_STAGES);
    const uint32_t bar_acc = bars + 8u * (2 * G::A_STAGES + 1);
    volatile uint32_t* tmem_holder = reinterpret_cast<volatile uint32_t*>(smem + G::OFF_BARS + 8 * G::NBARS);

    const int warp = threadIdx.x >> 5, lane = threadIdx.x & 31;
    const int n_eff = eval_count(a);
    const int units = (n_eff + G::QPOS - 1) / G::QPOS;
    const int my_passes =
        (int)blockIdx.x < units ? (units - (int)blockIdx.x + (int)gridDim.x - 1) / (int)gridDim.x : 0;
    const int NL = net.num_layers;
    const bool stamp = eval_timeline(a) && blockIdx.x == 0;
    unsigned long long* cta_rec = (eval_timeline(a) && blockIdx.x < 1024) ? eval_timeline(a) + 4 * NL + 16 + 3 * blockIdx.x : nullptr;
    if (cta_rec && threadIdx.x == 0) {
        unsigned smid;
        unsigned long long t;
        asm volatile("mov.u32 %0, %%smid;" : "=r"(smid));
        asm volatile("mov.u64 %0, %%globaltimer;" : "=l"(t));
        cta_rec[0] = smid;
        cta_rec[1] = t;
    }

    for (int i = threadIdx.x; i < G::NGRP * G::GRP_BYTES / 16; i += G::THREADS)
        reinterpret_cast<uint4*>(smem)[i] = make_uint4(0, 0, 0, 0);
    if (threadIdx.x == 0) {
        for (int s = 0; s < G::A_STAGES; ++s) {
            mbar_init(bar_afull(s), 4);
            mbar_init(bar_aempty(s), 1);
        }
        mbar_init(bar_act, G::NGRP * G::EPI_WARPS);
        mbar_init(bar_acc, 1);
        fence_mbar_init();
    }
    fence_proxy_async_smem();
    if (warp == G::MMA_WARP) tmem_alloc(smem_u32(const_cast<uint32_t*>(tmem_holder)), G::TMEM_COLS);
    tc_fence_before();
    __syncthreads();
    tc_fence_after();
    const uint32_t tmem_base = *tmem_holder;

    if (warp < 4) {
        setmaxnreg_dec<G::PRODUCER_REGS>();
        const int row = threadIdx.x;
        const uint32_t lane_addr = tmem_base + ((uint32_t)(warp * 32) << 16) + G::A_COL0;
        const int steps_per_pass = net.stages_per_pass;
        uint32_t slot = 0, phase = 0;
        auto load_stage = [&](uint4 (&dst)[4], const uint4* s) {
            dst[0] = __ldg(s);
            dst[1] = __ldg(s + 1);
            dst[2] = __ldg(s + 256);
            dst[3] = __ldg(s + 257);
        };
        auto store_stage = [&](const uint4 (&buf)[4]) {
            mbar_wait(bar_aempty(slot), phase ^ 1u);
            tc_fence_after();
            asm volatile(
                "tcgen05.st.sync.aligned.32x32b.x16.b32 [%0], "
                "{%1, %2, %3, %4, %5, %6, %7, %8, %9, %10, %11, %12, %13, %14, %15, %16};"
                ::"r"(lane_addr + slot * G::A_STAGE_COLS), "r"(buf[0].x), "r"(buf[0].y), "r"(buf[0].z), "r"(buf[0].w),
                  "r"(buf[1].x), "r"(buf[1].y), "r"(buf[1].z), "r"(buf[1].w), "r"(buf[2].x), "r"(buf[2].y), "r"(buf[2].z),
                  "r"(buf[2].w), "r"(buf[3].x), "r"(buf[3].y), "r"(buf[3].z), "r"(buf[3].w)
                : "memory");
            tmem_st_wait();
            tc_fence_before();
            __syncwarp();
            if (lane == 0) mbar_arrive(bar_afull(slot));
            if (++slot == G::A_STAGES) { slot = 0; phase ^= 1u; }
        };
        const int stages_per_pass = steps_per_pass / 2;
        for (int p = 0; p < my_passes; ++p) {
            const uint4* src = reinterpret_cast<const uint4*>(net.tiles) + (size_t)row * 2;
            uint4 b0[4], b1[4], b2[4];
            int ld = 0, st = 0;
            if (ld < stages_per_pass) { load_stage(b0, src + (size_t)ld * 512); ++ld; }
            if (ld < stages_per_pass) { load_stage(b1, src + (size_t)ld * 512); ++ld; }
            if (ld < stages_per_pass) { load_stage(b2, src + (size_t)ld * 512); ++ld; }
            for (;;) {
                store_stage(b0); ++st;
                if (ld < stages_per_pass) { load_stage(b0, src + (size_t)ld * 512); ++ld; }
                if (st >= stages_per_pass) break;
                store_stage(b1); ++st;
                if (ld < stages_per_pass) { load_stage(b1, src + (size_t)ld * 512); ++ld; }
                if (st >= stages_per_pass) break;
                store_stage(b2); ++st;
                if (ld < stages_per_pass) { load_stage(b2, src + (size_t)ld * 512); ++ld; }
                if (st >= stages_per_pass) break;
            }
        }
    } else if (warp >= G::MMA_WARP) {
        setmaxnreg_dec<G::MMA_REGS>();
        if (warp == G::MMA_WARP) {
            constexpr uint32_t idesc = make_idesc_bf16_f32(128, G::NCOLS);
            constexpr uint32_t b_lbo = G::SPITCH * 16;
            uint32_t slot = 0, phase = 0, act_phase = 0;
            for (int p = 0; p < my_passes; ++p) {
                for (int L = 0; L < NL; ++L) {
                    mbar_wait(bar_act, act_phase);
                    act_phase ^= 1u;
                    tc_fence_after();
                    if (stamp && p == 0 && lane == 0) eval_timeline(a)[4 * L + 0] = clock64();
                    const bool head = (L == NL - 1);
                    const uint32_t in_buf = sbase + ((L & 1) ? G::OFF_BUF_A : G::OFF_BUF_B);
                    const int ntaps = head ? 1 : 9;
                    for (int kc = 0; kc < G::KC64; ++kc) {
                        const int halves = block_steps(net, L, kc) / 2;
                        for (int tap = 0; tap < ntaps; ++tap) {
                            const int shift = head ? 0 : (tap / 3 - 1) * 10 + (tap % 3 - 1);
                            const uint32_t b_base = in_buf + (uint32_t)((kc * 8 * G::SPITCH + G::GUARD + shift) * 16);
                            if (halves == 2) {
                                const uint32_t s0 = slot, s1 = (slot + 1) % G::A_STAGES;
                                const uint32_t ph1 = s1 == 0 ? phase ^ 1u : phase;
                                mbar_wait(bar_afull(s0), phase);
                                mbar_wait(bar_afull(s1), ph1);
                                tc_fence_after();
                                if (elect_one()) {
#pragma unroll
                                    for (int h = 0; h < 2; ++h) {
                                        const uint32_t a_base = tmem_base + G::A_COL0 + (h ? s1 : s0) * G::A_STAGE_COLS;
#pragma unroll
                                        for (int g = 0; g < G::NGRP; ++g) {
                                            const uint32_t b_lo = smem_desc_lo(b_base + g * G::GRP_BYTES, b_lbo);
#pragma unroll
                                            for (int k2 = 0; k2 < 2; ++k2) {
                                                const int k = 2 * h + k2;
                                                umma_bf16_ts(tmem_base + g * G::NCOLS, a_base + k2 * 8,
                                                             smem_desc_from(b_lo + (uint32_t)(2 * k * G::SPITCH), 128),
                                                             idesc, (uint32_t)((kc | tap | k) != 0));
                                            }
                                        }
                                        umma_commit(bar_aempty(h ? s1 : s0));
                                    }
                                }
                                __syncwarp();
                                slot = (slot + 2) % G::A_STAGES;
                                if (slot < 2) phase ^= 1u;
                                continue;
                            }
                            for (int h = 0; h < halves; ++h) {
                                mbar_wait(bar_afull(slot), phase);
                                tc_fence_after();
                                if (elect_one()) {
                                    const uint32_t a_base = tmem_base + G::A_COL0 + slot * G::A_STAGE_COLS;
#pragma unroll
                                    for (int g = 0; g < G::NGRP; ++g) {
                                        const uint32_t b_lo =
                                            smem_desc_lo(b_base + g * G::GRP_BYTES, b_lbo) + (uint32_t)(4 * h * G::SPITCH);
#pragma unroll
                                        for (int k2 = 0; k2 < 2; ++k2)
                                            umma_bf16_ts(tmem_base + g * G::NCOLS, a_base + k2 * 8,
                                                         smem_desc_from(b_lo + (uint32_t)(2 * k2 * G::SPITCH), 128),
                                                         idesc, (uint32_t)((kc | tap | h | k2) != 0));
                                    }
                                    umma_commit(bar_aempty(slot));
                                }
                                __syncwarp();
                                if (++slot == G::A_STAGES) { slot = 0; phase ^= 1u; }
                            }
                        }
                    }
                    if (elect_one()) umma_commit(bar_acc);
                    __syncwarp();
                    if (stamp && p == 0 && lane == 0) eval_timeline(a)[4 * L + 1] = clock64();
                }
            }
        }
    } else {
        setmaxnreg_inc<G::EPI_REGS>();
        const int g = NGRP == 1 ? 0 : (warp - 4) >> 2;
        const int et = threadIdx.x - 128 - g * G::GRP_THREADS;
        const int q = warp & 3;
        const uint32_t bar = kEpiBar + g;
        uint8_t* gsmem = smem + g * G::GRP_BYTES;
        const uint32_t bufA = sbase + g * G::GRP_BYTES + G::OFF_BUF_A, bufB = sbase + g * G::GRP_BYTES + G::OFF_BUF_B;
        float* scratch = reinterpret_cast<float*>(gsmem + G::OFF_BUF_A);
        uint4* featS = reinterpret_cast<uint4*>(gsmem + G::OFF_BUF_A);
        float* vbuf = reinterpret_cast<float*>(smem + G::OFF_VBUF + g * G::VBUF_BYTES);
        float* red = reinterpret_cast<float*>(smem + G::OFF_RED + g * G::RED_BYTES);
        const uint32_t taddr = tmem_base + ((uint32_t)(q * 32) << 16) + g * G::NCOLS;
        const bool stamper = stamp && g == 0 && et == 0;
        EpilogueMask<3> mask0, mask1;
        mask0.init(0, lane);
        mask1.init(96, lane);
        uint32_t acc_phase = 0;
        for (int p = 0; p < my_passes; ++p) {
            const int b0 = ((int)blockIdx.x + p * (int)gridDim.x) * G::QPOS + g * G::NPOS;

            expand_features<G::NPOS, G::SPITCH, G::GUARD, G::GRP_THREADS>(net, a, n_eff, b0, featS, gsmem + G::OFF_BUF_B, et, nullptr, bar);
            named_bar_sync(bar, G::GRP_THREADS);
            for (int i = et; i < G::FEAT_BYTES / 16; i += G::GRP_THREADS) featS[i] = make_uint4(0, 0, 0, 0);
            fence_proxy_async_smem();
            __syncwarp();
            if (lane == 0) mbar_arrive(bar_act);

            for (int L = 0; L < NL - 1; ++L) {
                float bias[4];
#pragma unroll
                for (int k = 0; k < 4; ++k)
                    bias[k] = __ldg(net.bias + (size_t)L * C + 64 * (k >> 1) + 16 * q + 8 * (k & 1) + (lane >> 2));
                mbar_wait(bar_acc, acc_phase);
                acc_phase ^= 1u;
                tc_fence_after();
                if (stamper && p == 0) eval_timeline(a)[4 * L + 2] = clock64();
                const uint32_t out_buf = ((L & 1) ? bufB : bufA) + G::GUARD * 16;
                const bool residual = (L >= 2) && ((L & 1) == 0);
#pragma unroll
                for (int part = 0; part < 2; ++part)
#pragma unroll
                    for (int lb = 0; lb < 2; ++lb) {
                        if (residual)
                            epilogue_half<3, true, 8>(lb, taddr + 96 * part, out_buf, G::SPITCH * 16, 2 * q, 96 * part, bias,
                                                      part ? mask1 : mask0, lane);
                        else
                            epilogue_half<3, false, 8>(lb, taddr + 96 * part, out_buf, G::SPITCH * 16, 2 * q, 96 * part, bias,
                                                       part ? mask1 : mask0, lane);
                    }
                tc_fence_before();
                fence_proxy_async_smem();
                __syncwarp();
                if (lane == 0) mbar_arrive(bar_act);
                if (stamper && p == 0) eval_timeline(a)[4 * L + 3] = clock64();
            }

            const int hp = 7 * q + lane;
            const float hbias = lane < 7 ? __ldg(net.bias + (size_t)(NL - 1) * C + hp) : 0.f;
            mbar_wait(bar_acc, acc_phase);
            acc_phase ^= 1u;
            tc_fence_after();
            head_read<0>(taddr, hbias, hp, scratch, vbuf, lane);
            head_read<96>(taddr + 96, hbias, hp, scratch, vbuf, lane);
            tc_fence_before();
            named_bar_sync(bar, G::GRP_THREADS);
            heads_tail_small<G::NPOS, G::GRP_THREADS>(net, a, n_eff, b0, scratch, vbuf, red, et, bar);
            if (p + 1 < my_passes) {
                for (int i = et; i < G::SCRATCH_BYTES / 16; i += G::GRP_THREADS)
                    reinterpret_cast<uint4*>(scratch)[i] = make_uint4(0, 0, 0, 0);
                named_bar_sync(bar, G::GRP_THREADS);
            }
        }
    }

    tc_fence_before();
    __syncthreads();
    if (cta_rec && threadIdx.x == 0) {
        unsigned long long t;
        asm volatile("mov.u64 %0, %%globaltimer;" : "=l"(t));
        cta_rec[2] = t;
    }
    if (warp == G::MMA_WARP) {
        __syncwarp();
        tmem_dealloc(tmem_base, G::TMEM_COLS);
    }
}

__global__ void __launch_bounds__(TmemGeom<1>::THREADS, TmemGeom<1>::MIN_BLOCKS)
    trunk_duo_kernel(const DeviceNet net, const EvalArgs a) { trunk_tmem_body<1>(net, a); }
__global__ void __launch_bounds__(TmemGeom<2>::THREADS, TmemGeom<2>::MIN_BLOCKS)
    trunk_quad_kernel(const DeviceNet net, const EvalArgs a) { trunk_tmem_body<2>(net, a); }

template <int NGRP>
constexpr auto tmem_kernel = NGRP == 1 ? trunk_duo_kernel : trunk_quad_kernel;

template <int NGRP>
int tmem_prepare(int* ctas_per_sm) {
    using G = TmemGeom<NGRP>;
    cudaError_t e = cudaFuncSetAttribute(tmem_kernel<NGRP>, cudaFuncAttributeMaxDynamicSharedMemorySize, G::SMEM_BYTES);
    if (e == cudaSuccess)
        e = cudaFuncSetAttribute(tmem_kernel<NGRP>, cudaFuncAttributePreferredSharedMemoryCarveout, 100);
    int nb = 0;
    if (e == cudaSuccess)
        e = cudaOccupancyMaxActiveBlocksPerMultiprocessor(&nb, tmem_kernel<NGRP>, G::THREADS, G::SMEM_BYTES);
    if (e != cudaSuccess || nb < 1) {
        set_error("trunk %s: cannot configure the kernel: %s (is this an sm_100a device?)", NGRP == 1 ? "duo" : "quad",
                  cudaGetErrorString(e));
        return NSB_ERR_NO_DEVICE;
    }
    if (ctas_per_sm) *ctas_per_sm = nb < G::MIN_BLOCKS ? G::MIN_BLOCKS : nb;
    return 0;
}

template <int NGRP>
int tmem_launch(const DeviceNet& net, const EvalArgs& a, int num_sms, int ctas_per_sm, cudaStream_t s) {
    using G = TmemGeom<NGRP>;
    if (a.n <= 0) return 0;
    const int units = (a.n + G::QPOS - 1) / G::QPOS;
    const int cap = num_sms * (ctas_per_sm > 0 ? ctas_per_sm : 1);
    const int grid = units < cap ? units : cap;
    tmem_kernel<NGRP><<<grid, G::THREADS, G::SMEM_BYTES, s>>>(net, a);
    return 1;
}

}

int trunk_duo_prepare(int* ctas_per_sm) { return tmem_prepare<1>(ctas_per_sm); }

int launch_trunk_duo(const DeviceNet& net, const EvalArgs& a, int num_sms, int ctas_per_sm, cudaStream_t s) {
    return tmem_launch<1>(net, a, num_sms, ctas_per_sm, s);
}

int trunk_quad_prepare() { return tmem_prepare<2>(nullptr); }

int launch_trunk_quad(const DeviceNet& net, const EvalArgs& a, int num_sms, cudaStream_t s) {
    return tmem_launch<2>(net, a, num_sms, 1, s);
}

}
```

nshogi-engine_b200/csrc/umma.cuh:

```cuda
#pragma once
#include <cuda_bf16.h>
#include <stdint.h>

namespace nsb {

__device__ __forceinline__ uint32_t smem_u32(const void* p) {
    return (uint32_t)__cvta_generic_to_shared(p);
}

__device__ __forceinline__ bool elect_one() {
    uint32_t pred;
    asm volatile(
        "{\n\t.reg .pred P1;\n\t"
        "elect.sync _|P1, 0xffffffff;\n\t"
        "selp.u32 %0, 1, 0, P1;\n\t}"
        : "=r"(pred));
    return pred != 0;
}

__device__ __forceinline__ void mbar_init(uint32_t bar, uint32_t count) {
    asm volatile("mbarrier.init.shared::cta.b64 [%0], %1;" ::"r"(bar), "r"(count) : "memory");
}
__device__ __forceinline__ void fence_mbar_init() {
    asm volatile("fence.mbarrier_init.release.cluster;" ::: "memory");
}
__device__ __forceinline__ void mbar_arrive(uint32_t bar) {
    asm volatile("mbarrier.arrive.shared::cta.b64 _, [%0];" ::"r"(bar) : "memory");
}
__device__ __forceinline__ void mbar_arrive_expect_tx(uint32_t bar, uint32_t bytes) {
    asm volatile("mbarrier.arrive.expect_tx.shared::cta.b64 _, [%0], %1;" ::"r"(bar), "r"(bytes)
                 : "memory");
}
__device__ __forceinline__ bool mbar_try_wait(uint32_t bar, uint32_t parity) {
    uint32_t done;
    asm volatile(
        "{\n\t.reg .pred p;\n\t"
        "mbarrier.try_wait.parity.shared::cta.b64 p, [%1], %2;\n\t"
        "selp.u32 %0, 1, 0, p;\n\t}"
        : "=r"(done)
        : "r"(bar), "r"(parity)
        : "memory");
    return done != 0;
}
__device__ __forceinline__ void mbar_wait(uint32_t bar, uint32_t parity) {
    while (!mbar_try_wait(bar, parity)) {
    }
}

__device__ __forceinline__ void fence_proxy_async_smem() {
    asm volatile("fence.proxy.async.shared::cta;" ::: "memory");
}
__device__ __forceinline__ void tc_fence_before() {
    asm volatile("tcgen05.fence::before_thread_sync;" ::: "memory");
}
__device__ __forceinline__ void tc_fence_after() {
    asm volatile("tcgen05.fence::after_thread_sync;" ::: "memory");
}
__device__ __forceinline__ void named_bar_sync(uint32_t id, uint32_t nthreads) {
    asm volatile("bar.sync %0, %1;" ::"r"(id), "r"(nthreads) : "memory");
}
__device__ __forceinline__ void named_bar_arrive(uint32_t id, uint32_t nthreads) {
    asm volatile("bar.arrive %0, %1;" ::"r"(id), "r"(nthreads) : "memory");
}

__device__ __forceinline__ void bulk_g2s(uint32_t dst_smem, const void* src, uint32_t bytes,
                                         uint32_t bar) {
    asm volatile(
        "cp.async.bulk.shared::cluster.global.mbarrier::complete_tx::bytes [%0], [%1], %2, [%3];"
        ::"r"(dst_smem), "l"(src), "r"(bytes), "r"(bar)
        : "memory");
}

__device__ __forceinline__ void bulk_g2s_multicast(uint32_t dst_smem, const void* src, uint32_t bytes, uint32_t bar,
                                                   uint16_t cta_mask) {
    asm volatile(
        "cp.async.bulk.shared::cluster.global.mbarrier::complete_tx::bytes.multicast::cluster [%0], [%1], %2, [%3], %4;"
        ::"r"(dst_smem), "l"(src), "r"(bytes), "r"(bar), "h"(cta_mask)
        : "memory");
}

__device__ __forceinline__ void tmem_alloc(uint32_t dst_smem, uint32_t ncols) {
    asm volatile("tcgen05.alloc.cta_group::1.sync.aligned.shared::cta.b32 [%0], %1;" ::"r"(dst_smem),
                 "r"(ncols)
                 : "memory");
    asm volatile("tcgen05.relinquish_alloc_permit.cta_group::1.sync.aligned;" ::: "memory");
}
__device__ __forceinline__ void tmem_dealloc(uint32_t taddr, uint32_t ncols) {
    asm volatile("tcgen05.dealloc.cta_group::1.sync.aligned.b32 %0, %1;" ::"r"(taddr), "r"(ncols)
                 : "memory");
}

__device__ __forceinline__ uint64_t make_smem_desc(uint32_t smem_addr, uint32_t lbo_bytes,
                                                   uint32_t sbo_bytes) {
    uint64_t d = 0;
    d |= (uint64_t)((smem_addr & 0x3FFFFu) >> 4);
    d |= (uint64_t)((lbo_bytes >> 4) & 0x3FFFu) << 16;
    d |= (uint64_t)((sbo_bytes >> 4) & 0x3FFFu) << 32;
    d |= 1ull << 46;
    return d;
}

__device__ __forceinline__ uint32_t smem_desc_lo(uint32_t smem_addr, uint32_t lbo_bytes) {
    return ((smem_addr & 0x3FFFFu) >> 4) | ((lbo_bytes >> 4) << 16);
}
__device__ __forceinline__ uint64_t smem_desc_from(uint32_t lo, uint32_t sbo_bytes) {
    return ((uint64_t)(((sbo_bytes >> 4) & 0x3FFFu) | (1u << 14)) << 32) | lo;
}

__host__ __device__ constexpr uint32_t make_idesc_bf16_f32(int m, int n) {
    return (1u << 4) | (1u << 7) | (1u << 10) | ((uint32_t)(n >> 3) << 17) |
           ((uint32_t)(m >> 4) << 24);
}

__device__ __forceinline__ void umma_bf16(uint32_t d_tmem, uint64_t a_desc, uint64_t b_desc,
                                          uint32_t idesc, uint32_t accumulate) {
    asm volatile(
        "{\n\t.reg .pred p;\n\t"
        "setp.ne.b32 p, %4, 0;\n\t"
        "tcgen05.mma.cta_group::1.kind::f16 [%0], %1, %2, %3, p;\n\t}"
        ::"r"(d_tmem), "l"(a_desc), "l"(b_desc), "r"(idesc), "r"(accumulate)
        : "memory");
}
__device__ __forceinline__ void umma_bf16_ts(uint32_t d_tmem, uint32_t a_tmem, uint64_t b_desc, uint32_t idesc,
                                             uint32_t accumulate) {
    asm volatile(
        "{\n\t.reg .pred p;\n\t"
        "setp.ne.b32 p, %4, 0;\n\t"
        "tcgen05.mma.cta_group::1.kind::f16 [%0], [%1], %2, %3, p;\n\t}"
        ::"r"(d_tmem), "r"(a_tmem), "l"(b_desc), "r"(idesc), "r"(accumulate)
        : "memory");
}
__device__ __forceinline__ void tmem_st_32x32b_x8(uint32_t taddr, const uint32_t (&v)[8]) {
    asm volatile("tcgen05.st.sync.aligned.32x32b.x8.b32 [%0], {%1, %2, %3, %4, %5, %6, %7, %8};" ::"r"(taddr),
                 "r"(v[0]), "r"(v[1]), "r"(v[2]), "r"(v[3]), "r"(v[4]), "r"(v[5]), "r"(v[6]), "r"(v[7])
                 : "memory");
}
__device__ __forceinline__ void tmem_st_32x32b_x32(uint32_t taddr, const uint32_t (&v)[32]) {
    asm volatile(
        "tcgen05.st.sync.aligned.32x32b.x32.b32 [%0], "
        "{%1, %2, %3, %4, %5, %6, %7, %8, %9, %10, %11, %12, %13, %14, %15, %16, "
        "%17, %18, %19, %20, %21, %22, %23, %24, %25, %26, %27, %28, %29, %30, %31, %32};"
        ::"r"(taddr), "r"(v[0]), "r"(v[1]), "r"(v[2]), "r"(v[3]), "r"(v[4]), "r"(v[5]), "r"(v[6]), "r"(v[7]), "r"(v[8]),
          "r"(v[9]), "r"(v[10]), "r"(v[11]), "r"(v[12]), "r"(v[13]), "r"(v[14]), "r"(v[15]), "r"(v[16]), "r"(v[17]),
          "r"(v[18]), "r"(v[19]), "r"(v[20]), "r"(v[21]), "r"(v[22]), "r"(v[23]), "r"(v[24]), "r"(v[25]), "r"(v[26]),
          "r"(v[27]), "r"(v[28]), "r"(v[29]), "r"(v[30]), "r"(v[31])
        : "memory");
}
__device__ __forceinline__ void tmem_st_32x32b_x32(uint32_t taddr, const uint4 (&q)[8]) {
    asm volatile(
        "tcgen05.st.sync.aligned.32x32b.x32.b32 [%0], "
        "{%1, %2, %3, %4, %5, %6, %7, %8, %9, %10, %11, %12, %13, %14, %15, %16, "
        "%17, %18, %19, %20, %21, %22, %23, %24, %25, %26, %27, %28, %29, %30, %31, %32};"
        ::"r"(taddr), "r"(q[0].x), "r"(q[0].y), "r"(q[0].z), "r"(q[0].w), "r"(q[1].x), "r"(q[1].y), "r"(q[1].z), "r"(q[1].w),
          "r"(q[2].x), "r"(q[2].y), "r"(q[2].z), "r"(q[2].w), "r"(q[3].x), "r"(q[3].y), "r"(q[3].z), "r"(q[3].w),
          "r"(q[4].x), "r"(q[4].y), "r"(q[4].z), "r"(q[4].w), "r"(q[5].x), "r"(q[5].y), "r"(q[5].z), "r"(q[5].w),
          "r"(q[6].x), "r"(q[6].y), "r"(q[6].z), "r"(q[6].w), "r"(q[7].x), "r"(q[7].y), "r"(q[7].z), "r"(q[7].w)
        : "memory");
}
__device__ __forceinline__ void tmem_st_32x32b_x16(uint32_t taddr, const uint4 (&q)[8]) {
    asm volatile(
        "tcgen05.st.sync.aligned.32x32b.x16.b32 [%0], "
        "{%1, %2, %3, %4, %5, %6, %7, %8, %9, %10, %11, %12, %13, %14, %15, %16};"
        ::"r"(taddr), "r"(q[0].x), "r"(q[0].y), "r"(q[0].z), "r"(q[0].w), "r"(q[1].x), "r"(q[1].y), "r"(q[1].z), "r"(q[1].w),
          "r"(q[2].x), "r"(q[2].y), "r"(q[2].z), "r"(q[2].w), "r"(q[3].x), "r"(q[3].y), "r"(q[3].z), "r"(q[3].w)
        : "memory");
}
__device__ __forceinline__ void tmem_st_32x32b_x16(uint32_t taddr, const uint32_t* v) {
    asm volatile(
        "tcgen05.st.sync.aligned.32x32b.x16.b32 [%0], "
        "{%1, %2, %3, %4, %5, %6, %7, %8, %9, %10, %11, %12, %13, %14, %15, %16};"
        ::"r"(taddr), "r"(v[0]), "r"(v[1]), "r"(v[2]), "r"(v[3]), "r"(v[4]), "r"(v[5]), "r"(v[6]), "r"(v[7]), "r"(v[8]),
          "r"(v[9]), "r"(v[10]), "r"(v[11]), "r"(v[12]), "r"(v[13]), "r"(v[14]), "r"(v[15])
        : "memory");
}
template <int N>
__device__ __forceinline__ void setmaxnreg_inc() {
    asm volatile("setmaxnreg.inc.sync.aligned.u32 %0;" ::"n"(N));
}
template <int N>
__device__ __forceinline__ void setmaxnreg_dec() {
    asm volatile("setmaxnreg.dec.sync.aligned.u32 %0;" ::"n"(N));
}
__device__ __forceinline__ void umma_commit(uint32_t bar) {
    asm volatile("tcgen05.commit.cta_group::1.mbarrier::arrive::one.shared::cluster.b64 [%0];" ::"r"(bar)
                 : "memory");
}

__device__ __forceinline__ void tmem_ld32(uint32_t taddr, uint32_t (&v)[32]) {
    asm volatile(
        "tcgen05.ld.sync.aligned.32x32b.x32.b32 "
        "{%0, %1, %2, %3, %4, %5, %6, %7, %8, %9, %10, %11, %12, %13, %14, %15, "
        "%16, %17, %18, %19, %20, %21, %22, %23, %24, %25, %26, %27, %28, %29, %30, %31}, [%32];"
        : "=r"(v[0]), "=r"(v[1]), "=r"(v[2]), "=r"(v[3]), "=r"(v[4]), "=r"(v[5]), "=r"(v[6]),
          "=r"(v[7]), "=r"(v[8]), "=r"(v[9]), "=r"(v[10]), "=r"(v[11]), "=r"(v[12]), "=r"(v[13]),
          "=r"(v[14]), "=r"(v[15]), "=r"(v[16]), "=r"(v[17]), "=r"(v[18]), "=r"(v[19]),
          "=r"(v[20]), "=r"(v[21]), "=r"(v[22]), "=r"(v[23]), "=r"(v[24]), "=r"(v[25]),
          "=r"(v[26]), "=r"(v[27]), "=r"(v[28]), "=r"(v[29]), "=r"(v[30]), "=r"(v[31])
        : "r"(taddr)
        : "memory");
}
__device__ __forceinline__ void tmem_ld_16x256b_x4(uint32_t taddr, uint32_t (&v)[16]) {
    asm volatile(
        "tcgen05.ld.sync.aligned.16x256b.x4.b32 "
        "{%0, %1, %2, %3, %4, %5, %6, %7, %8, %9, %10, %11, %12, %13, %14, %15}, [%16];"
        : "=r"(v[0]), "=r"(v[1]), "=r"(v[2]), "=r"(v[3]), "=r"(v[4]), "=r"(v[5]), "=r"(v[6]),
          "=r"(v[7]), "=r"(v[8]), "=r"(v[9]), "=r"(v[10]), "=r"(v[11]), "=r"(v[12]), "=r"(v[13]),
          "=r"(v[14]), "=r"(v[15])
        : "r"(taddr)
        : "memory");
}
__device__ __forceinline__ void stmatrix_x4_trans(uint32_t addr, uint32_t r0, uint32_t r1, uint32_t r2,
                                                  uint32_t r3) {
    asm volatile("stmatrix.sync.aligned.m8n8.x4.trans.shared.b16 [%0], {%1, %2, %3, %4};" ::"r"(addr),
                 "r"(r0), "r"(r1), "r"(r2), "r"(r3)
                 : "memory");
}
__device__ __forceinline__ void ldmatrix_x4_trans(uint32_t addr, uint32_t& r0, uint32_t& r1, uint32_t& r2,
                                                  uint32_t& r3) {
    asm volatile("ldmatrix.sync.aligned.m8n8.x4.trans.shared.b16 {%0, %1, %2, %3}, [%4];"
                 : "=r"(r0), "=r"(r1), "=r"(r2), "=r"(r3)
                 : "r"(addr)
                 : "memory");
}
__device__ __forceinline__ uint32_t pack_bf16x2(float lo, float hi) {
    uint32_t d;
    asm("cvt.rn.bf16x2.f32 %0, %1, %2;" : "=r"(d) : "f"(hi), "f"(lo));
    return d;
}
__device__ __forceinline__ uint32_t pack_relu_bf16x2(float lo, float hi) {
    uint32_t d;
    asm("cvt.rn.relu.bf16x2.f32 %0, %1, %2;" : "=r"(d) : "f"(hi), "f"(lo));
    return d;
}
__device__ __forceinline__ uint64_t pack_f32x2(float lo, float hi) {
    uint64_t r;
    asm("mov.b64 %0, {%1, %2};" : "=l"(r) : "f"(lo), "f"(hi));
    return r;
}
__device__ __forceinline__ uint64_t pack_u32x2(uint32_t lo, uint32_t hi) {
    uint64_t r;
    asm("mov.b64 %0, {%1, %2};" : "=l"(r) : "r"(lo), "r"(hi));
    return r;
}
__device__ __forceinline__ uint64_t add_f32x2(uint64_t a, uint64_t b) {
    uint64_t r;
    asm("add.rn.f32x2 %0, %1, %2;" : "=l"(r) : "l"(a), "l"(b));
    return r;
}
__device__ __forceinline__ uint32_t pack_relu_bf16x2(uint64_t v) {
    uint32_t d;
    asm("{\n\t.reg .f32 lo, hi;\n\t"
        "mov.b64 {lo, hi}, %1;\n\t"
        "cvt.rn.relu.bf16x2.f32 %0, hi, lo;\n\t}"
        : "=r"(d)
        : "l"(v));
    return d;
}
__device__ __forceinline__ void tmem_ld_wait() {
    asm volatile("tcgen05.wait::ld.sync.aligned;" ::: "memory");
}

__device__ __forceinline__ uint32_t cluster_ctarank() {
    uint32_t r;
    asm volatile("mov.u32 %0, %%cluster_ctarank;" : "=r"(r));
    return r;
}
__device__ __forceinline__ void cluster_sync_all() {
    asm volatile("barrier.cluster.arrive.release.aligned;" ::: "memory");
    asm volatile("barrier.cluster.wait.acquire.aligned;" ::: "memory");
}
__device__ __forceinline__ uint32_t map_to_cta(uint32_t smem_addr, uint32_t rank) {
    uint32_t r;
    asm volatile("mapa.shared::cluster.u32 %0, %1, %2;" : "=r"(r) : "r"(smem_addr), "r"(rank));
    return r;
}
__device__ __forceinline__ void mbar_arrive_remote(uint32_t cluster_bar) {
    asm volatile("mbarrier.arrive.shared::cluster.b64 _, [%0];" ::"r"(cluster_bar) : "memory");
}
__device__ __forceinline__ void mbar_arrive_expect_tx_remote(uint32_t cluster_bar, uint32_t bytes) {
    asm volatile("mbarrier.arrive.expect_tx.shared::cluster.b64 _, [%0], %1;" ::"r"(cluster_bar),
                 "r"(bytes)
                 : "memory");
}
__device__ __forceinline__ void bulk_s2peer(uint32_t dst_cluster, uint32_t src_smem, uint32_t bytes,
                                            uint32_t bar_cluster) {
    asm volatile(
        "cp.async.bulk.shared::cluster.shared::cta.mbarrier::complete_tx::bytes [%0], [%1], %2, [%3];"
        ::"r"(dst_cluster), "r"(src_smem), "r"(bytes), "r"(bar_cluster)
        : "memory");
}
__device__ __forceinline__ void tmem_alloc_pair(uint32_t dst_smem, uint32_t ncols) {
    asm volatile("tcgen05.alloc.cta_group::2.sync.aligned.shared::cta.b32 [%0], %1;" ::"r"(dst_smem), "r"(ncols)
                 : "memory");
    asm volatile("tcgen05.relinquish_alloc_permit.cta_group::2.sync.aligned;" ::: "memory");
}
__device__ __forceinline__ void tmem_dealloc_pair(uint32_t taddr, uint32_t ncols) {
    asm volatile("tcgen05.dealloc.cta_group::2.sync.aligned.b32 %0, %1;" ::"r"(taddr), "r"(ncols) : "memory");
}
__device__ __forceinline__ void umma_bf16_pair(uint32_t d_tmem, uint64_t a_desc, uint64_t b_desc, uint32_t idesc,
                                               uint32_t accumulate) {
    asm volatile(
        "{\n\t.reg .pred p;\n\t"
        "setp.ne.b32 p, %4, 0;\n\t"
        "tcgen05.mma.cta_group::2.kind::f16 [%0], %1, %2, %3, p;\n\t}"
        ::"r"(d_tmem), "l"(a_desc), "l"(b_desc), "r"(idesc), "r"(accumulate)
        : "memory");
}
__device__ __forceinline__ void umma_commit_multicast(uint32_t bar, uint16_t cta_mask) {
    asm volatile(
        "tcgen05.commit.cta_group::1.mbarrier::arrive::one.shared::cluster.multicast::cluster.b64 [%0], %1;"
        ::"r"(bar), "h"(cta_mask)
        : "memory");
}
__device__ __forceinline__ void umma_commit_pair(uint32_t bar, uint16_t cta_mask) {
    asm volatile(
        "tcgen05.commit.cta_group::2.mbarrier::arrive::one.shared::cluster.multicast::cluster.b64 [%0], %1;"
        ::"r"(bar), "h"(cta_mask)
        : "memory");
}
__device__ __forceinline__ void tmem_st_16x128b_x4(uint32_t taddr, const uint32_t (&v)[8]) {
    asm volatile("tcgen05.st.sync.aligned.16x128b.x4.b32 [%0], {%1, %2, %3, %4, %5, %6, %7, %8};" ::"r"(taddr),
                 "r"(v[0]), "r"(v[1]), "r"(v[2]), "r"(v[3]), "r"(v[4]), "r"(v[5]), "r"(v[6]), "r"(v[7])
                 : "memory");
}
__device__ __forceinline__ void tmem_ld_16x128b_x4(uint32_t taddr, uint32_t (&v)[8]) {
    asm volatile("tcgen05.ld.sync.aligned.16x128b.x4.b32 {%0, %1, %2, %3, %4, %5, %6, %7}, [%8];"
                 : "=r"(v[0]), "=r"(v[1]), "=r"(v[2]), "=r"(v[3]), "=r"(v[4]), "=r"(v[5]), "=r"(v[6]), "=r"(v[7])
                 : "r"(taddr)
                 : "memory");
}
__device__ __forceinline__ void tmem_st_wait() {
    asm volatile("tcgen05.wait::st.sync.aligned;" ::: "memory");
}

__device__ __forceinline__ uint16_t f32_to_bf16_bits(float f) {
    return __bfloat16_as_ushort(__float2bfloat16_rn(f));
}
__device__ __forceinline__ float bf16_bits_to_f32(uint16_t b) {
    return __uint_as_float((uint32_t)b << 16);
}

}
```

nshogi-engine_b200/csrc/umma_probe.cu:

```cuda
#include <cuda_runtime.h>
#include <math.h>
#include <stdint.h>
#include <string.h>

#include <vector>

#include "nsb_internal.h"
#include "umma.cuh"

namespace nsb {
namespace {

__device__ __forceinline__ uint64_t make_desc_sw128(uint32_t addr) {
    uint64_t d = 0;
    d |= (uint64_t)((addr & 0x3FFFFu) >> 4);
    d |= (uint64_t)1 << 16;
    d |= (uint64_t)(1024 >> 4) << 32;
    d |= 1ull << 46;
    d |= 2ull << 61;
    return d;
}

__device__ __forceinline__ uint32_t elem_off(int layout, int r, int k, int pitch_rows) {
    if (layout == 0) return (uint32_t)(((k >> 3) * pitch_rows + r) * 16 + (k & 7) * 2);
    const int kc = k >> 6, c = (k >> 3) & 7;
    return (uint32_t)(kc * pitch_rows * 128 + r * 128 + ((c ^ (r & 7)) << 4) + (k & 7) * 2);
}

__global__ void __launch_bounds__(128, 1)
umma_probe_kernel(const uint16_t* __restrict__ a, const uint16_t* __restrict__ b, int N, int K, int rows,
                  int shift, int layout, int iters, float* __restrict__ d, unsigned long long* __restrict__ cycles) {
    extern __shared__ uint8_t smem_raw[];
    uint8_t* smem = reinterpret_cast<uint8_t*>(((uintptr_t)smem_raw + 1023) & ~(uintptr_t)1023);
    const int a_rows = 128, b_rows = (rows + 7) & ~7;
    const size_t a_bytes = (size_t)a_rows * K * 2, b_bytes = (size_t)b_rows * K * 2;
    uint8_t* sa = smem;
    uint8_t* sb = sa + ((a_bytes + 1023) & ~(size_t)1023);
    uint8_t* tail = sb + ((b_bytes + 1023) & ~(size_t)1023);
    const uint32_t bar = smem_u32(tail);
    volatile uint32_t* holder = reinterpret_cast<volatile uint32_t*>(tail + 8);
    for (int i = threadIdx.x; i < 128 * K; i += blockDim.x)
        *reinterpret_cast<uint16_t*>(sa + elem_off(layout, i / K, i % K, a_rows)) = a[i];
    for (int i = threadIdx.x; i < rows * K; i += blockDim.x)
        *reinterpret_cast<uint16_t*>(sb + elem_off(layout, i / K, i % K, b_rows)) = b[i];
    if (threadIdx.x == 0) {
        mbar_init(bar, 1);
        mbar_init(bar + 16, 1);
        fence_mbar_init();
    }
    fence_proxy_async_smem();
    const int warp = threadIdx.x >> 5;
    if (warp == 0) tmem_alloc(smem_u32(const_cast<uint32_t*>(holder)), 256);
    tc_fence_before();
    __syncthreads();
    tc_fence_after();
    const uint32_t tmem_base = *holder;
    if (warp == 0) {
        const uint32_t idesc = make_idesc_bf16_f32(128, N);
        uint32_t parity = 0;
        const uint32_t a0 = smem_u32(sa), b0 = smem_u32(sb);
        for (int it = 0; it < iters + 1; ++it) {
            const unsigned long long t0 = clock64();
            const int reps = it == 0 ? 1 : 16;
            for (int rep = 0; rep < reps; ++rep) {
                if (elect_one()) {
                    if (layout == 0) {
                        const uint32_t a_lo = smem_desc_lo(a0, a_rows * 16);
                        const uint32_t b_lo = smem_desc_lo(b0 + (uint32_t)(shift * 16), b_rows * 16);
                        for (int k4 = 0; k4 < K / 64; ++k4) {
#pragma unroll
                            for (int kk = 0; kk < 4; ++kk) {
                                const int k16 = k4 * 4 + kk;
                                umma_bf16(tmem_base, smem_desc_from(a_lo + (uint32_t)(k16 * 2 * a_rows), 128),
                                          smem_desc_from(b_lo + (uint32_t)(k16 * 2 * b_rows), 128), idesc,
                                          (it == 0 && rep == 0 && k16 == 0) ? 0u : 1u);
                            }
                            if (iters & 1) umma_commit(bar + 16);
                        }
                    } else
                    for (int k16 = 0; k16 < K / 16; ++k16) {
                        uint64_t ad, bd;
                        if (layout == 0) {
                            ad = make_smem_desc(a0 + (uint32_t)(k16 * 2 * a_rows * 16), a_rows * 16, 128);
                            bd = make_smem_desc(b0 + (uint32_t)((k16 * 2 * b_rows + shift) * 16), b_rows * 16, 128);
                        } else {
                            const int kc = k16 >> 2, kk = k16 & 3;
                            ad = make_desc_sw128(a0 + (uint32_t)(kc * a_rows * 128 + kk * 32));
                            bd = make_desc_sw128(b0 + (uint32_t)(kc * b_rows * 128 + shift * 128 + kk * 32));
                        }
                        umma_bf16(tmem_base, ad, bd, idesc, (it == 0 && rep == 0 && k16 == 0) ? 0u : 1u);
                        if ((iters & 1) && (k16 & 3) == 3) umma_commit(bar + 16);
                    }
                }
                __syncwarp();
            }
            if (elect_one()) umma_commit(bar);
            __syncwarp();
            mbar_wait(bar, parity);
            parity ^= 1u;
            const unsigned long long t1 = clock64();
            if (threadIdx.x == 0) {
                if (it == 1) cycles[0] = 0;
                if (it >= 1) cycles[0] += t1 - t0;
            }
        }
    }
    __syncthreads();
    if (threadIdx.x == 0) {
        const uint32_t idesc = make_idesc_bf16_f32(128, N);
        for (int k16 = 0; k16 < K / 16; ++k16) {
            uint64_t ad, bd;
            if (layout == 0) {
                ad = make_smem_desc(smem_u32(sa) + (uint32_t)(k16 * 2 * a_rows * 16), a_rows * 16, 128);
                bd = make_smem_desc(smem_u32(sb) + (uint32_t)((k16 * 2 * b_rows + shift) * 16), b_rows * 16, 128);
            } else {
                const int kc = k16 >> 2, kk = k16 & 3;
                ad = make_desc_sw128(smem_u32(sa) + (uint32_t)(kc * a_rows * 128 + kk * 32));
                bd = make_desc_sw128(smem_u32(sb) + (uint32_t)(kc * b_rows * 128 + shift * 128 + kk * 32));
            }
            umma_bf16(tmem_base, ad, bd, idesc, k16 != 0);
        }
        umma_commit(bar);
        mbar_wait(bar, (uint32_t)((iters + 1) & 1));
    }
    __syncthreads();
    tc_fence_after();
    for (int j = 0; j < N / 32; ++j) {
        uint32_t v[32];
        tmem_ld32(tmem_base + ((uint32_t)(warp * 32) << 16) + j * 32, v);
        tmem_ld_wait();
#pragma unroll
        for (int i = 0; i < 32; ++i) d[(size_t)threadIdx.x * N + j * 32 + i] = __uint_as_float(v[i]);
    }
    tc_fence_before();
    __syncthreads();
    if (warp == 0) tmem_dealloc(tmem_base, 256);
}


__global__ void __launch_bounds__(128, 1)
umma_ts_probe_kernel(const uint16_t* __restrict__ a, const uint16_t* __restrict__ b, int N, int K, int rows,
                     int shift, int smem_noise, int iters, float* __restrict__ d, unsigned long long* __restrict__ cycles) {
    extern __shared__ uint8_t smem_raw[];
    uint8_t* smem = reinterpret_cast<uint8_t*>(((uintptr_t)smem_raw + 1023) & ~(uintptr_t)1023);
    const int b_rows = (rows + 7) & ~7;
    const size_t b_bytes = (size_t)b_rows * K * 2;
    uint8_t* sb = smem;
    uint8_t* noise = sb + ((b_bytes + 1023) & ~(size_t)1023);
    uint8_t* tail = noise + 32768;
    const uint32_t bar = smem_u32(tail);
    volatile uint32_t* holder = reinterpret_cast<volatile uint32_t*>(tail + 8);
    volatile int* stop = reinterpret_cast<volatile int*>(tail + 16);
    for (int i = threadIdx.x; i < rows * K; i += blockDim.x)
        *reinterpret_cast<uint16_t*>(sb + elem_off(0, i / K, i % K, b_rows)) = b[i];
    if (threadIdx.x == 0) {
        mbar_init(bar, 1);
        fence_mbar_init();
        *stop = 0;
    }
    fence_proxy_async_smem();
    const int warp = threadIdx.x >> 5;
    if (warp == 0) tmem_alloc(smem_u32(const_cast<uint32_t*>(holder)), 512);
    tc_fence_before();
    __syncthreads();
    tc_fence_after();
    const uint32_t tmem_base = *holder;
    const uint32_t a_tmem = tmem_base + 256;
    {
        const uint32_t lane_addr = a_tmem + ((uint32_t)(warp * 32) << 16);
        for (int k16 = 0; k16 < K / 16; ++k16) {
            uint32_t v[8];
#pragma unroll
            for (int j = 0; j < 8; ++j)
                v[j] = (uint32_t)a[(size_t)threadIdx.x * K + k16 * 16 + 2 * j] |
                       ((uint32_t)a[(size_t)threadIdx.x * K + k16 * 16 + 2 * j + 1] << 16);
            tmem_st_32x32b_x8(lane_addr + k16 * 8, v);
        }
        tmem_st_wait();
    }
    tc_fence_before();
    __syncthreads();
    tc_fence_after();
    const uint32_t idesc = make_idesc_bf16_f32(128, N);
    const uint32_t b0 = smem_u32(sb);
    auto issue_all = [&](bool fresh) {
        for (int k16 = 0; k16 < K / 16; ++k16) {
            const uint64_t bd = make_smem_desc(b0 + (uint32_t)((k16 * 2 * b_rows + shift) * 16), b_rows * 16, 128);
            umma_bf16_ts(tmem_base, a_tmem + k16 * 8, bd, idesc, (fresh && k16 == 0) ? 0u : 1u);
        }
    };
    const int ring_mmas = (iters & 1) ? 2 : 4;
    if (threadIdx.x == 0) {
        mbar_init(bar + 32, 1);
        mbar_init(bar + 40, 1);
        fence_mbar_init();
        mbar_arrive(bar + 40);
    }
    __syncthreads();
    if (warp == 0) {
        uint32_t parity = 0;
        for (int it = 0; it < iters + 1; ++it) {
            const unsigned long long t0 = clock64();
            const int reps = it == 0 ? 1 : 16;
            for (int rep = 0; rep < reps; ++rep) {
                if (smem_noise == 2) {
                    for (int k0 = 0; k0 < K / 16; k0 += ring_mmas) {
                        mbar_wait(bar + 40, 0);
                        tc_fence_after();
                        if (elect_one()) {
                            for (int k16 = k0; k16 < k0 + ring_mmas; ++k16) {
                                const uint64_t bd =
                                    make_smem_desc(b0 + (uint32_t)((k16 * 2 * b_rows + shift) * 16), b_rows * 16, 128);
                                umma_bf16_ts(tmem_base, a_tmem + k16 * 8, bd, idesc, (it == 0 && rep == 0 && k16 == 0) ? 0u : 1u);
                            }
                            umma_commit(bar + 32);
                        }
                        __syncwarp();
                    }
                    continue;
                }
                if (elect_one()) issue_all(it == 0 && rep == 0);
                __syncwarp();
            }
            if (elect_one()) umma_commit(bar);
            __syncwarp();
            mbar_wait(bar, parity);
            parity ^= 1u;
            const unsigned long long t1 = clock64();
            if (threadIdx.x == 0) {
                if (it == 1) cycles[0] = 0;
                if (it >= 1) cycles[0] += t1 - t0;
            }
        }
        if (elect_one()) {
            issue_all(true);
            umma_commit(bar);
        }
        __syncwarp();
        mbar_wait(bar, parity);
        if (threadIdx.x == 0) *stop = 1;
    } else if (smem_noise == 1) {
        uint4* dst = reinterpret_cast<uint4*>(noise);
        unsigned k = threadIdx.x;
        while (*stop == 0) {
#pragma unroll
            for (int r = 0; r < 8; ++r) {
                dst[k & 2047] = make_uint4(k, k, k, k);
                k += 96;
            }
        }
    }
    __syncthreads();
    tc_fence_after();
    for (int j = 0; j < N / 32; ++j) {
        uint32_t v[32];
        tmem_ld32(tmem_base + ((uint32_t)(warp * 32) << 16) + j * 32, v);
        tmem_ld_wait();
#pragma unroll
        for (int i = 0; i < 32; ++i) d[(size_t)threadIdx.x * N + j * 32 + i] = __uint_as_float(v[i]);
    }
    tc_fence_before();
    __syncthreads();
    if (warp == 0) tmem_dealloc(tmem_base, 512);
}

__global__ void __cluster_dims__(2, 1, 1) __launch_bounds__(128, 1)
umma_pair_probe_kernel(const uint16_t* __restrict__ a, const uint16_t* __restrict__ b, int N, int K, int rows,
                       int shift, int layout, int iters, float* __restrict__ d, unsigned long long* __restrict__ cycles) {
    extern __shared__ uint8_t smem_raw[];
    uint8_t* smem = reinterpret_cast<uint8_t*>(((uintptr_t)smem_raw + 1023) & ~(uintptr_t)1023);
    const uint32_t rank = cluster_ctarank();
    const int a_rows = 128, b_rows = (rows + 7) & ~7;
    const size_t a_bytes = (size_t)a_rows * K * 2, b_bytes = (size_t)b_rows * K * 2;
    uint8_t* sa = smem;
    uint8_t* sb = sa + ((a_bytes + 1023) & ~(size_t)1023);
    uint8_t* tail = sb + ((b_bytes + 1023) & ~(size_t)1023);
    const uint32_t bar = smem_u32(tail);
    volatile uint32_t* holder = reinterpret_cast<volatile uint32_t*>(tail + 8);
    for (int i = threadIdx.x; i < 128 * K; i += blockDim.x)
        *reinterpret_cast<uint16_t*>(sa + elem_off(layout, i / K, i % K, a_rows)) = a[(size_t)rank * 128 * K + i];
    for (int i = threadIdx.x; i < rows * K; i += blockDim.x)
        *reinterpret_cast<uint16_t*>(sb + elem_off(layout, i / K, i % K, b_rows)) = b[(size_t)rank * rows * K + i];
    if (threadIdx.x == 0) {
        mbar_init(bar, 1);
        fence_mbar_init();
    }
    fence_proxy_async_smem();
    const int warp = threadIdx.x >> 5;
    if (warp == 0) tmem_alloc_pair(smem_u32(const_cast<uint32_t*>(holder)), 256);
    tc_fence_before();
    cluster_sync_all();
    tc_fence_after();
    const uint32_t tmem_base = *holder;
    const uint32_t idesc = make_idesc_bf16_f32(256, N);
    const uint32_t a0 = smem_u32(sa), b0 = smem_u32(sb);
    auto issue_all = [&](bool fresh) {
        for (int k16 = 0; k16 < K / 16; ++k16) {
            uint64_t ad, bd;
            if (layout == 0) {
                ad = make_smem_desc(a0 + (uint32_t)(k16 * 2 * a_rows * 16), a_rows * 16, 128);
                bd = make_smem_desc(b0 + (uint32_t)((k16 * 2 * b_rows + shift) * 16), b_rows * 16, 128);
            } else {
                const int kc = k16 >> 2, kk = k16 & 3;
                ad = make_desc_sw128(a0 + (uint32_t)(kc * a_rows * 128 + kk * 32));
                bd = make_desc_sw128(b0 + (uint32_t)(kc * b_rows * 128 + shift * 128 + kk * 32));
            }
            umma_bf16_pair(tmem_base, ad, bd, idesc, (fresh && k16 == 0) ? 0u : 1u);
        }
    };
    uint32_t parity = 0;
    if (warp == 0) {
        for (int it = 0; it < iters + 1; ++it) {
            const unsigned long long t0 = clock64();
            if (rank == 0) {
                const int reps = it == 0 ? 1 : 16;
                for (int rep = 0; rep < reps; ++rep) {
                    if (elect_one()) issue_all(it == 0 && rep == 0);
                    __syncwarp();
                }
                if (elect_one()) umma_commit_pair(bar, 3);
                __syncwarp();
            }
            mbar_wait(bar, parity);
            parity ^= 1u;
            const unsigned long long t1 = clock64();
            if (threadIdx.x == 0 && rank == 0) {
                if (it == 1) cycles[0] = 0;
                if (it >= 1) cycles[0] += t1 - t0;
            }
        }
        if (rank == 0) {
            if (elect_one()) {
                issue_all(true);
                umma_commit_pair(bar, 3);
            }
            __syncwarp();
        }
        mbar_wait(bar, parity);
    }
    __syncthreads();
    tc_fence_after();
    for (int j = 0; j < N / 32; ++j) {
        uint32_t v[32];
        tmem_ld32(tmem_base + ((uint32_t)(warp * 32) << 16) + j * 32, v);
        tmem_ld_wait();
#pragma unroll
        for (int i = 0; i < 32; ++i)
            d[((size_t)rank * 128 + threadIdx.x) * N + j * 32 + i] = __uint_as_float(v[i]);
    }
    tc_fence_before();
    cluster_sync_all();
    if (warp == 0) tmem_dealloc_pair(tmem_base, 256);
}

}

int umma_probe(int gpu, int n_cols, int k_elems, int shift_rows, int layout, int iters, float* max_err,
               double* cycles_per_mma) {
    const bool ts = layout >= 4;
    const bool pair = layout == 2 || layout == 3;
    const int lay = ts ? 0 : (layout & 1);
    if (n_cols % 32 || n_cols < 32 || n_cols > 256 || k_elems % 64 || k_elems <= 0 || shift_rows < 0 ||
        shift_rows > 64 || iters < 1 || layout < 0 || layout > 6) {
        set_error("umma_probe: bad arguments");
        return NSB_ERR_INVALID;
    }
    if (cudaSetDevice(gpu) != cudaSuccess) return NSB_ERR_NO_DEVICE;
    const int N = n_cols, K = k_elems, M = pair ? 256 : 128;
    const int n_cta = pair ? N / 2 : N;
    const int rows = n_cta + shift_rows + 8;
    const int nct = pair ? 2 : 1;
    std::vector<uint16_t> ha((size_t)M * K), hb((size_t)nct * rows * K);
    std::vector<float> fa(ha.size()), fb(hb.size());
    uint64_t s = 0x9E3779B97F4A7C15ull;
    auto rnd = [&]() { s ^= s << 13; s ^= s >> 7; s ^= s << 17; return (float)((int)(s % 17) - 8) / 8.0f; };
    auto bits = [](float f) { uint32_t u; memcpy(&u, &f, 4); return (uint16_t)(u >> 16); };
    for (size_t i = 0; i < ha.size(); ++i) { fa[i] = rnd(); ha[i] = bits(fa[i]); }
    for (size_t i = 0; i < hb.size(); ++i) { fb[i] = rnd(); hb[i] = bits(fb[i]); }
    uint16_t *da = nullptr, *db = nullptr;
    float* dd = nullptr;
    unsigned long long* dc = nullptr;
    cudaError_t e = cudaMalloc(&da, ha.size() * 2);
    if (e == cudaSuccess) e = cudaMalloc(&db, hb.size() * 2);
    if (e == cudaSuccess) e = cudaMalloc(&dd, (size_t)M * N * 4);
    if (e == cudaSuccess) e = cudaMalloc(&dc, 16);
    if (e == cudaSuccess) e = cudaMemcpy(da, ha.data(), ha.size() * 2, cudaMemcpyHostToDevice);
    if (e == cudaSuccess) e = cudaMemcpy(db, hb.data(), hb.size() * 2, cudaMemcpyHostToDevice);
    const size_t smem = (size_t)128 * K * 2 + (size_t)((rows + 7) & ~7) * K * 2 + 4096 + (ts ? 32768 : 0);
    if (e == cudaSuccess)
        e = cudaFuncSetAttribute(ts ? (const void*)umma_ts_probe_kernel
                                    : (pair ? (const void*)umma_pair_probe_kernel : (const void*)umma_probe_kernel),
                                 cudaFuncAttributeMaxDynamicSharedMemorySize, (int)smem);
    if (e == cudaSuccess) {
        if (ts)
            umma_ts_probe_kernel<<<1, 128, smem>>>(da, db, N, K, rows, shift_rows, layout - 4, iters, dd, dc);
        else if (pair)
            umma_pair_probe_kernel<<<2, 128, smem>>>(da, db, N, K, rows, shift_rows, lay, iters, dd, dc);
        else
            umma_probe_kernel<<<1, 128, smem>>>(da, db, N, K, rows, shift_rows, lay, iters, dd, dc);
        e = cudaDeviceSynchronize();
    }
    std::vector<float> hd((size_t)M * N);
    unsigned long long hc[2] = {0, 0};
    if (e == cudaSuccess) e = cudaMemcpy(hd.data(), dd, hd.size() * 4, cudaMemcpyDeviceToHost);
    if (e == cudaSuccess) e = cudaMemcpy(hc, dc, 16, cudaMemcpyDeviceToHost);
    cudaFree(da); cudaFree(db); cudaFree(dd); cudaFree(dc);
    if (e != cudaSuccess) {
        set_error("umma_probe: CUDA error: %s", cudaGetErrorString(e));
        return NSB_ERR_CUDA;
    }
    float worst = 0.f;
    for (int m = 0; m < M; ++m)
        for (int n = 0; n < N; ++n) {
            const int cta = n / n_cta, r = n % n_cta + shift_rows;
            float acc = 0.f;
            for (int k = 0; k < K; ++k) acc += fa[(size_t)m * K + k] * fb[((size_t)cta * rows + r) * K + k];
            worst = fmaxf(worst, fabsf(acc - hd[(size_t)m * N + n]));
        }
    if (max_err) *max_err = worst;
    if (cycles_per_mma) *cycles_per_mma = (double)hc[0] / ((double)iters * 16.0 * (K / 16));
    return 0;
}

}

namespace nsb {
namespace {
__global__ void __launch_bounds__(64, 1)
bulk_rate_kernel(const uint8_t* __restrict__ src, int src_bytes, int tile_bytes, int stages, int split, int iters,
                 unsigned long long* __restrict__ cycles) {
    extern __shared__ uint8_t smem_raw[];
    uint8_t* smem = reinterpret_cast<uint8_t*>(((uintptr_t)smem_raw + 127) & ~(uintptr_t)127);
    const uint32_t ring = smem_u32(smem);
    const uint32_t bars = ring + (uint32_t)(stages * tile_bytes);
    if (threadIdx.x == 0) {
        for (int s = 0; s < stages; ++s) {
            mbar_init(bars + 8u * s, 1);
            mbar_init(bars + 8u * (stages + s), 1);
        }
        fence_mbar_init();
    }
    __syncthreads();
    const int tiles = src_bytes / tile_bytes;
    const int part = tile_bytes / split;
    if (threadIdx.x == 0) {
        uint32_t stage = 0, phase = 0;
        for (int it = 0; it < iters; ++it)
            for (int t = 0; t < tiles; ++t) {
                mbar_wait(bars + 8u * (stages + stage), phase ^ 1u);
                mbar_arrive_expect_tx(bars + 8u * stage, (uint32_t)tile_bytes);
                for (int k = 0; k < split; ++k)
                    bulk_g2s(ring + stage * tile_bytes + k * part, src + (size_t)t * tile_bytes + k * part, (uint32_t)part,
                             bars + 8u * stage);
                if (++stage == (uint32_t)stages) { stage = 0; phase ^= 1u; }
            }
    } else if (threadIdx.x == 32) {
        uint32_t stage = 0, phase = 0;
        const unsigned long long t0 = clock64();
        for (int it = 0; it < iters; ++it)
            for (int t = 0; t < tiles; ++t) {
                mbar_wait(bars + 8u * stage, phase);
                mbar_arrive(bars + 8u * (stages + stage));
                if (++stage == (uint32_t)stages) { stage = 0; phase ^= 1u; }
            }
        if (blockIdx.x == 0) cycles[0] = clock64() - t0;
    }
}
}

int bulk_rate_probe(int gpu, int ctas, int tile_bytes, int stages, int split, double* bytes_per_cycle) {
    if (cudaSetDevice(gpu) != cudaSuccess) return NSB_ERR_NO_DEVICE;
    if (tile_bytes % (16 * split) || stages < 1 || stages * tile_bytes > 200 * 1024 || ctas < 1) {
        set_error("bulk_rate_probe: bad arguments");
        return NSB_ERR_INVALID;
    }
    const int src_bytes = (288 * 1024 / tile_bytes) * tile_bytes, iters = 20;
    uint8_t* d = nullptr;
    unsigned long long* dc = nullptr;
    cudaError_t e = cudaMalloc(&d, src_bytes);
    if (e == cudaSuccess) e = cudaMemset(d, 1, src_bytes);
    if (e == cudaSuccess) e = cudaMalloc(&dc, 8);
    const size_t smem = (size_t)stages * tile_bytes + 16 * stages + 256;
    if (e == cudaSuccess) e = cudaFuncSetAttribute(bulk_rate_kernel, cudaFuncAttributeMaxDynamicSharedMemorySize, (int)smem);
    if (e == cudaSuccess) {
        bulk_rate_kernel<<<ctas, 64, smem>>>(d, src_bytes, tile_bytes, stages, split, iters, dc);
        bulk_rate_kernel<<<ctas, 64, smem>>>(d, src_bytes, tile_bytes, stages, split, iters, dc);
        e = cudaDeviceSynchronize();
    }
    unsigned long long hc = 0;
    if (e == cudaSuccess) e = cudaMemcpy(&hc, dc, 8, cudaMemcpyDeviceToHost);
    cudaFree(d);
    cudaFree(dc);
    if (e != cudaSuccess) {
        set_error("bulk_rate_probe: %s", cudaGetErrorString(e));
        return NSB_ERR_CUDA;
    }
    if (bytes_per_cycle) *bytes_per_cycle = (double)src_bytes * iters / (double)hc;
    return 0;
}
}
```

nshogi-engine_b200/csrc/weights.cc:

```cpp
#include <cmath>
#include <cstring>

#include "nsb_internal.h"

namespace nsb {

size_t blob_floats(const nsb_net_desc& d) {
    const size_t C = d.channels, IN = d.in_channels, H = d.value_hidden, NB = d.blocks;
    return C * IN * 9 + C + NB * 2 * (C * C * 9 + C) + kPolicyPlanes * C + kPolicyPlanes + C + 1 +
           H * 81 + H + 2 * H + 2;
}

static inline int cout_halves(int channels) { return channels == 128 ? 1 : 2; }

int stages_per_pass(const nsb_net_desc& d) {
    const int nhalf = cout_halves(d.channels), kc64 = d.channels / 64;
    return 9 * (kStemCin / 64) * nhalf + 2 * d.blocks * 9 * kc64 * nhalf + kc64;
}

static inline uint16_t bf16_bits_rne(float x) {
    uint32_t u;
    std::memcpy(&u, &x, 4);
    if ((u & 0x7F800000u) == 0x7F800000u) return (uint16_t)(u >> 16);
    u += 0x7FFFu + ((u >> 16) & 1u);
    return (uint16_t)(u >> 16);
}
static inline float bf16_round(float x) {
    const uint32_t u = (uint32_t)bf16_bits_rne(x) << 16;
    float r;
    std::memcpy(&r, &u, 4);
    return r;
}

namespace {
struct Rng {
    uint64_t s;
    uint64_t next() {
        uint64_t z = (s += 0x9E3779B97F4A7C15ull);
        z = (z ^ (z >> 30)) * 0xBF58476D1CE4E5B9ull;
        z = (z ^ (z >> 27)) * 0x94D049BB133111EBull;
        return z ^ (z >> 31);
    }
    double uniform() { return ((double)(next() >> 11) + 0.5) * (1.0 / 9007199254740992.0); }
    float normal(float std) {
        const double u1 = uniform(), u2 = uniform();
        return (float)(std * std::sqrt(-2.0 * std::log(u1)) * std::cos(6.283185307179586 * u2));
    }
};
}

void blob_random(const nsb_net_desc& d, uint64_t seed, float* blob) {
    const int C = d.channels, IN = d.in_channels, H = d.value_hidden, NB = d.blocks;
    Rng r{seed * 0x2545F4914F6CDD1Dull + 0x1234567ull};
    float* w = blob;
    auto fill = [&](size_t n, float std) {
        for (size_t i = 0; i < n; ++i) *w++ = bf16_round(r.normal(std));
    };
    fill((size_t)C * IN * 9, std::sqrt(2.0f / (float)(IN * 9)));
    fill(C, 0.05f);
    for (int b = 0; b < NB; ++b) {
        fill((size_t)C * C * 9, std::sqrt(2.0f / (float)(C * 9)));
        fill(C, 0.05f);
        fill((size_t)C * C * 9, 0.25f * std::sqrt(2.0f / (float)(C * 9)));
        fill(C, 0.05f);
    }
    fill((size_t)kPolicyPlanes * C, std::sqrt(1.0f / (float)C));
    fill(kPolicyPlanes, 0.05f);
    fill(C, std::sqrt(1.0f / (float)C));
    fill(1, 0.05f);
    fill((size_t)H * 81, std::sqrt(2.0f / 81.0f));
    fill(H, 0.05f);
    fill((size_t)2 * H, std::sqrt(1.0f / (float)H));
    fill(2, 0.05f);
}

static inline size_t tile_index(int j, int row, int e) { return ((size_t)j * 128 + row) * 8 + e; }

void pack_weights(const nsb_net_desc& d, const float* blob, uint16_t* tiles, float* bias,
                  float* fc1t, float* fc1b, float* fc2, float* fc2b) {
    const int C = d.channels, IN = d.in_channels, H = d.value_hidden, NB = d.blocks;
    const int nhalf = cout_halves(C), rows = C / nhalf, kc64 = C / 64;
    const size_t tile_elems = kStageBytes / 2;
    const float* w = blob;
    uint16_t* t = tiles;
    int layer = 0;
    auto pack_conv = [&](const float* cw, int cin_real, int cin_pad, bool stem = false) {
        for (int tap = 0; tap < 9; ++tap)
            for (int kc = 0; kc < cin_pad / 64; ++kc)
                for (int half = 0; half < nhalf; ++half) {
                    for (int j = 0; j < 8; ++j)
                        for (int row = 0; row < 128; ++row)
                            for (int e = 0; e < 8; ++e) {
                                const int co = half * rows + row, ci = kc * 64 + j * 8 + e;
                                const int src = stem ? stem_source_channel(ci, cin_real) : (ci < cin_real ? ci : -1);
                                const float v = src >= 0 && row < rows ? cw[((size_t)co * cin_real + src) * 9 + tap] : 0.f;
                                t[tile_index(j, row, e)] = bf16_bits_rne(v);
                            }
                    t += tile_elems;
                }
    };
    pack_conv(w, IN, kStemCin, true);
    w += (size_t)C * IN * 9;
    std::memcpy(bias + (size_t)layer * C, w, sizeof(float) * C);
    w += C;
    ++layer;
    for (int b = 0; b < 2 * NB; ++b) {
        pack_conv(w, C, C);
        w += (size_t)C * C * 9;
        std::memcpy(bias + (size_t)layer * C, w, sizeof(float) * C);
        w += C;
        ++layer;
    }
    const float* pw = w;
    const float* pb = w + (size_t)kPolicyPlanes * C;
    const float* vw = pb + kPolicyPlanes;
    const float* vb = vw + C;
    for (int kc = 0; kc < kc64; ++kc) {
        for (int j = 0; j < 8; ++j)
            for (int row = 0; row < 128; ++row)
                for (int e = 0; e < 8; ++e) {
                    const int ci = kc * 64 + j * 8 + e;
                    float v = 0.f;
                    const int hc = (row % 32) < 7 ? 7 * (row / 32) + (row % 32) : -1;
                    if (hc >= 0 && hc < kPolicyPlanes) v = pw[(size_t)hc * C + ci];
                    else if (hc == kPolicyPlanes) v = vw[ci];
                    t[tile_index(j, row, e)] = bf16_bits_rne(v);
                }
        t += tile_elems;
    }
    float* hb = bias + (size_t)layer * C;
    std::memset(hb, 0, sizeof(float) * C);
    std::memcpy(hb, pb, sizeof(float) * kPolicyPlanes);
    hb[kPolicyPlanes] = vb[0];
    w = vb + 1;
    for (int h = 0; h < H; ++h)
        for (int s = 0; s < 81; ++s) fc1t[(size_t)s * H + h] = w[(size_t)h * 81 + s];
    w += (size_t)H * 81;
    std::memcpy(fc1b, w, sizeof(float) * H);
    w += H;
    std::memcpy(fc2, w, sizeof(float) * 2 * H);
    w += 2 * H;
    std::memcpy(fc2b, w, sizeof(float) * 2);
}


int ts_steps_per_pass(const nsb_net_desc& d) {
    const int kc64 = d.channels / 64;
    return 9 * stem_steps(d.in_channels) + 2 * d.blocks * 9 * kc64 * 4 + kc64 * 4;
}

void pack_weights_ts(const nsb_net_desc& d, const float* blob, uint16_t* stream) {
    const int C = d.channels, IN = d.in_channels, NB = d.blocks;
    const int kc64 = C / 64;
    const float* w = blob;
    uint16_t* t = stream;
    auto row_channel = [](int row) { return 64 * ((row >> 4) & 1) + 16 * (row >> 5) + (row & 15); };
    auto pack_conv = [&](const float* cw, int cin_real, int kblocks, int last_block_steps, bool stem = false) {
        for (int kc = 0; kc < kblocks; ++kc)
            for (int tap = 0; tap < 9; ++tap)
                for (int k = 0; k < (kc + 1 == kblocks ? last_block_steps : 4); ++k) {
                    for (int row = 0; row < 128; ++row)
                        for (int e = 0; e < 16; ++e) {
                            const int co = row_channel(row), ci = kc * 64 + k * 16 + e;
                            const int src = stem ? stem_source_channel(ci, cin_real) : (ci < cin_real ? ci : -1);
                            const float v = src >= 0 ? cw[((size_t)co * cin_real + src) * 9 + tap] : 0.f;
                            t[row * 16 + e] = bf16_bits_rne(v);
                        }
                    t += 128 * 16;
                }
    };
    pack_conv(w, IN, 2, stem_steps(IN) - 4, true);
    w += (size_t)C * IN * 9 + C;
    for (int b = 0; b < 2 * NB; ++b) {
        pack_conv(w, C, kc64, 4);
        w += (size_t)C * C * 9 + C;
    }
    const float* pw = w;
    const float* vw = w + (size_t)kPolicyPlanes * C + kPolicyPlanes;
    for (int kc = 0; kc < kc64; ++kc)
        for (int k = 0; k < 4; ++k) {
            for (int row = 0; row < 128; ++row)
                for (int e = 0; e < 16; ++e) {
                    const int ci = kc * 64 + k * 16 + e;
                    const int hc = (row % 32) < 7 ? 7 * (row / 32) + (row % 32) : -1;
                    float v = 0.f;
                    if (hc >= 0 && hc < kPolicyPlanes) v = pw[(size_t)hc * C + ci];
                    else if (hc == kPolicyPlanes) v = vw[ci];
                    t[row * 16 + e] = bf16_bits_rne(v);
                }
            t += 128 * 16;
        }
}

}
```

Measured before the change: 2.605 million.

## Pack boards at 9-column pitch and fix horizontal-tap edges with TMEM patches

Changes the activation layout in the duo/TS trunk kernel from a 10-slot row pitch (100 slots per board) to a 9-slot pitch (91 per board). This lets the MMA N dimension shrink from 192 to 176 columns. Without padding columns, the horizontal taps wrap across rows. To handle this, taps are grouped by dx class: the weights are repacked class-major and the epilogue warps save, zero and restore edge columns in TMEM between classes, synchronized by new mbarriers. The aim is less tensor-core work per layer, paid for with extra MMA/epilogue handshakes and tcgen05 ld/st per layer that could stall the pipeline.

```diff
diff --git a/include/nsb_diag.h b/include/nsb_diag.h
--- a/include/nsb_diag.h
+++ b/include/nsb_diag.h
@@ -20,6 +20,9 @@
 
 int nsb_debug_bulk_rate_probe(int gpu, int ctas, int tile_bytes, int stages, int split, double* bytes_per_cycle);
 
+int nsb_debug_pack_weights_ts(const nsb_net_desc* net, const float* blob, int dw_class_major, uint16_t* stream,
+                              size_t max_steps);
+
 #if defined(__GNUC__)
 #pragma GCC visibility pop
 #endif
diff --git a/nshogi-engine_b200/binding.py b/nshogi-engine_b200/binding.py
--- a/nshogi-engine_b200/binding.py
+++ b/nshogi-engine_b200/binding.py
@@ -112,6 +112,7 @@
     "nsb_debug_umma_probe": (C.c_int, [C.c_int, C.c_int, C.c_int, C.c_int, C.c_int, C.c_int, C.POINTER(C.c_float),
                                        C.POINTER(C.c_double)]),
     "nsb_debug_bulk_rate_probe": (C.c_int, [C.c_int, C.c_int, C.c_int, C.c_int, C.c_int, C.POINTER(C.c_double)]),
+    "nsb_debug_pack_weights_ts": (C.c_int, [_P, _P, C.c_int, _P, C.c_size_t]),
 }
 DIAG_LIB_PATH = os.path.join(HERE, "libnsb_diag.so")
 _diag = None
@@ -267,6 +268,17 @@
     return float(err.value), float(epi.value)
 
 
+def pack_weights_ts(desc: NetDesc, blob: np.ndarray, dw_class_major: bool) -> np.ndarray:
+    blob = np.ascontiguousarray(blob, dtype=np.float32)
+    max_steps = 9 * 8 + 2 * desc.blocks * 9 * 8 + 8
+    out = np.zeros((max_steps, 128, 16), dtype=np.uint16)
+    rc = diag_lib().nsb_debug_pack_weights_ts(C.byref(desc), blob.ctypes.data, int(dw_class_major), out.ctypes.data,
+                                              max_steps)
+    if rc < 0:
+        _check(rc, "nsb_debug_pack_weights_ts")
+    return out[:rc]
+
+
 def umma_probe(n_cols, k_elems, shift_rows, layout, iters=20, gpu=0):
     err, cyc = C.c_float(-1.0), C.c_double(0)
     _check(diag_lib().nsb_debug_umma_probe(gpu, n_cols, k_elems, shift_rows, layout, iters, C.byref(err), C.byref(cyc)),
@@ -431,7 +443,7 @@
 
     def debug_trunk_timeline(self, slot, d_features, n, positions=False):
         nl = 2 * self.desc.blocks + 2
-        out = np.zeros(nl * 4 + 16 + 3 * 1024, dtype=np.uint64)
+        out = np.zeros(nl * 6 + 16 + 3 * 1024, dtype=np.uint64)
         fn = self._l.nsb_debug_trunk_timeline_positions if positions else self._l.nsb_debug_trunk_timeline
         _check(fn(self._h, slot, _ptr(d_features), n, out.ctypes.data, out.size), "nsb_debug_trunk_timeline")
         return out[:nl * 4].reshape(nl, 4), out[nl * 4:]
diff --git a/nshogi-engine_b200/csrc/epilogue.cuh b/nshogi-engine_b200/csrc/epilogue.cuh
--- a/nshogi-engine_b200/csrc/epilogue.cuh
+++ b/nshogi-engine_b200/csrc/epilogue.cuh
@@ -6,8 +6,11 @@
 namespace nsb {
 
 __host__ __device__ constexpr bool is_real_slot(int n) { return (n % 100) < 90 && ((n % 100) % 10) < 9; }
+__host__ __device__ constexpr bool is_real_slot9(int n) { return n < 172 && (n % 91) < 81; }
+template <int W>
+__host__ __device__ constexpr bool is_real_slot_w(int n) { return W == 9 ? is_real_slot9(n) : is_real_slot(n); }
 
-template <int NCG>
+template <int NCG, int W = 10>
 struct EpilogueMask {
     uint32_t m[NCG * 4];
     template <int COL0>
@@ -18,7 +21,7 @@
 #pragma unroll
             for (int q4 = 0; q4 < 4; ++q4) {
                 const int n = COL0 + 8 * G + 2 * q4;
-                const uint32_t c = (is_real_slot(n) ? 0x0000FFFFu : 0u) | (is_real_slot(n + 1) ? 0xFFFF0000u : 0u);
+                const uint32_t c = (is_real_slot_w<W>(n) ? 0x0000FFFFu : 0u) | (is_real_slot_w<W>(n + 1) ? 0xFFFF0000u : 0u);
                 v = (lane & 3) == q4 ? c : v;
             }
             m[G] = v;
@@ -30,9 +33,9 @@
     }
 };
 
-template <int NCG, bool kResidual, int LBS = 2>
+template <int NCG, bool kResidual, int LBS = 2, int W = 10>
 __device__ __forceinline__ void epilogue_half(int lb, uint32_t taddr, uint32_t buf, uint32_t pitch, int chunk0,
-                                              int col0, const float (&bias)[4], const EpilogueMask<NCG>& mask,
+                                              int col0, const float (&bias)[4], const EpilogueMask<NCG, W>& mask,
                                               int lane) {
     const int mk = lane >> 3, mi = lane & 7;
     uint32_t v[NCG][16];
diff --git a/nshogi-engine_b200/csrc/nsb_api.cu b/nshogi-engine_b200/csrc/nsb_api.cu
--- a/nshogi-engine_b200/csrc/nsb_api.cu
+++ b/nshogi-engine_b200/csrc/nsb_api.cu
@@ -342,7 +342,7 @@
     if (ts_only || c->duo_ctas > 0) {
         ts_stages = ts_steps_per_pass(d);
         ts_tiles.assign((size_t)ts_stages * 2048, 0);
-        pack_weights_ts(d, blob, ts_tiles.data());
+        pack_weights_ts(d, blob, ts_tiles.data(), c->use_ts ? TsOrder::kBlockMajor : TsOrder::kDwClassMajor);
         if (ts_only) {
             stages = ts_stages;
             tiles.swap(ts_tiles);
@@ -1039,7 +1039,7 @@
         set_error("nsb_debug_trunk_timeline: bad arguments or weights not loaded");
         return NSB_ERR_INVALID;
     }
-    const size_t need = (size_t)c->net.num_layers * 4 + 16 + 3 * 1024;
+    const size_t need = (size_t)c->net.num_layers * 6 + 16 + 3 * 1024;
     if (max_stamps < need) {
         set_error("nsb_debug_trunk_timeline: need room for %zu stamps", need);
         return NSB_ERR_INVALID;
@@ -1335,6 +1335,21 @@
     return bulk_rate_probe(gpu, ctas, tile_bytes, stages, split, bytes_per_cycle);
 }
 
+int nsb_debug_pack_weights_ts(const nsb_net_desc* net, const float* blob, int dw_class_major, uint16_t* stream,
+                              size_t max_steps) {
+    if (!net || !blob || !stream || net->channels != 128) {
+        set_error("nsb_debug_pack_weights_ts: bad arguments (128-channel nets only)");
+        return NSB_ERR_INVALID;
+    }
+    const int steps = ts_steps_per_pass(*net);
+    if (max_steps < (size_t)steps) {
+        set_error("nsb_debug_pack_weights_ts: need room for %d steps", steps);
+        return NSB_ERR_INVALID;
+    }
+    pack_weights_ts(*net, blob, stream, dw_class_major ? TsOrder::kDwClassMajor : TsOrder::kBlockMajor);
+    return steps;
+}
+
 #endif
 
 int nsb_event_create(void** out) {
diff --git a/nshogi-engine_b200/csrc/nsb_internal.h b/nshogi-engine_b200/csrc/nsb_internal.h
--- a/nshogi-engine_b200/csrc/nsb_internal.h
+++ b/nshogi-engine_b200/csrc/nsb_internal.h
@@ -18,6 +18,8 @@
 __host__ __device__ constexpr int stem_source_channel(int ci, int in_channels) {
     return ci < in_channels ? ci : (ci < in_channels + stem_twins(in_channels) ? kFirstScalarChannel + (ci - in_channels) : -1);
 }
+enum class TsOrder { kBlockMajor, kDwClassMajor };
+__host__ __device__ constexpr int dw_class_tap(int c, int i) { return 3 * i + (c == 0 ? 2 : (c == 1 ? 0 : 1)); }
 constexpr int kStageBytes = 16384;
 constexpr int kMaxHidden = 256;
 
@@ -138,7 +140,7 @@
 void blob_random(const nsb_net_desc& d, uint64_t seed, float* blob);
 int stages_per_pass(const nsb_net_desc& d);
 int ts_steps_per_pass(const nsb_net_desc& d);
-void pack_weights_ts(const nsb_net_desc& d, const float* blob, uint16_t* stream);
+void pack_weights_ts(const nsb_net_desc& d, const float* blob, uint16_t* stream, TsOrder order);
 void pack_weights(const nsb_net_desc& d, const float* blob, uint16_t* tiles, float* bias,
                   float* fc1t, float* fc1b, float* fc2, float* fc2b);
 
diff --git a/nshogi-engine_b200/csrc/trunk_common.cuh b/nshogi-engine_b200/csrc/trunk_common.cuh
--- a/nshogi-engine_b200/csrc/trunk_common.cuh
+++ b/nshogi-engine_b200/csrc/trunk_common.cuh
@@ -50,7 +50,7 @@
     return li < n_eff ? (a.index ? __ldg(a.index + li) : li) : -1;
 }
 
-template <int NPOS, int SPITCH, int GUARD, int NT = kEpiThreads>
+template <int NPOS, int SPITCH, int GUARD, int NT = kEpiThreads, int POS_SLOTS = 100, int ROW_SLOTS = 10>
 __device__ __forceinline__ void expand_features(const DeviceNet& net, const EvalArgs& a, int n_eff, int li0, uint4* featS,
                                                 uint8_t* stem_buf, int et, unsigned long long* tl,
                                                 uint32_t bar = kEpiBar) {
@@ -95,7 +95,7 @@
             field[e] = __funnelshift_r(lo, hi, sh);
             val[e] = c < IN ? (f.w & 0xFFFFu) : (f.w >> 16);
         }
-        uint8_t* dst = stem_buf + (size_t)((j * SPITCH + GUARD + pos * 100 + row * 10) * 16);
+        uint8_t* dst = stem_buf + (size_t)((j * SPITCH + GUARD + pos * POS_SLOTS + row * ROW_SLOTS) * 16);
 #pragma unroll
         for (int col = 0; col < 9; ++col) {
             uint32_t w[4];
@@ -111,7 +111,7 @@
     if (tl) tl[10] = clock64();
 }
 
-template <int COL0>
+template <int COL0, int W = 10>
 __device__ __forceinline__ void head_read(uint32_t taddr, float bias, int hp, float* scratch, float* vbuf, int lane) {
 #pragma unroll
     for (int j = 0; j < 3; ++j) {
@@ -124,8 +124,9 @@
 #pragma unroll
             for (int i = 0; i < 32; ++i) {
                 const int n = COL0 + j * 32 + i;
-                if (is_real_slot(n)) {
-                    const int pos = n / 100, m = n % 100, t = (m / 10) * 9 + (m % 10);
+                if (is_real_slot_w<W>(n)) {
+                    const int pos = W == 9 ? n / 91 : n / 100, m = W == 9 ? n % 91 : n % 100;
+                    const int t = W == 9 ? m : (m / 10) * 9 + (m % 10);
                     const float x = __uint_as_float(v[i]) + bias;
                     dst[(relu ? pos * 81 : pos * kPolicySize) + t] = relu ? fmaxf(x, 0.f) : x;
                 }
diff --git a/nshogi-engine_b200/csrc/trunk_tmem.cu b/nshogi-engine_b200/csrc/trunk_tmem.cu
--- a/nshogi-engine_b200/csrc/trunk_tmem.cu
+++ b/nshogi-engine_b200/csrc/trunk_tmem.cu
@@ -16,6 +16,8 @@
     static constexpr int NPOS = 2;
     static constexpr int QPOS = NGRP * NPOS;
     static constexpr int NCOLS = NPOS * 96;
+    static constexpr int POS_SLOTS = 91, ROW_SLOTS = 9;
+    static constexpr int NMMA = 176;
     static constexpr int GUARD = 12;
     static constexpr int SPITCH = (GUARD + NCOLS + 11) | 1;
     static constexpr int BUF_BYTES = ((KCH * SPITCH * 16 + 127) / 128) * 128;
@@ -30,7 +32,7 @@
     static constexpr int MMA_WARP = 4 + 4 * NGRP;
     static constexpr int MIN_BLOCKS = NGRP == 1 ? 2 : 1;
     static constexpr int PRODUCER_REGS = 72, EPI_REGS = NGRP == 1 ? 128 : 168, MMA_REGS = 40;
-    static constexpr int NBARS = 2 * A_STAGES + 2;
+    static constexpr int NBARS = 2 * A_STAGES + 2 + 2 * NGRP;
     static constexpr int SCRATCH_BYTES = ((NPOS * kPolicySize * 4 + 15) / 16) * 16;
     static constexpr int FEAT_BYTES = NPOS * kMaxInChannels * 16;
     static constexpr int VBUF_BYTES = ((NPOS * 81 * 4 + 15) / 16) * 16;
@@ -43,8 +45,10 @@
     static constexpr int OFF_BARS = OFF_RED + NGRP * RED_BYTES;
     static constexpr int SMEM_BYTES = OFF_BARS + NBARS * 8 + 16 + 128;
     static_assert(BUF_BYTES == 55040, "each group has the duo kernel's activation layout");
-    static_assert(NGRP > 1 || (OFF_VBUF == 110080 && OFF_RED == 110736 && OFF_BARS == 110816 && SMEM_BYTES == 111040),
-                  "one group keeps the duo kernel's shared memory map");
+    static_assert(NGRP > 1 || (OFF_VBUF == 110080 && OFF_RED == 110736 && OFF_BARS == 110816 && SMEM_BYTES == 111056),
+                  "one group keeps the duo kernel's shared memory map (plus the two barriers of the edge fixes)");
+    static_assert(POS_SLOTS + 81 <= NMMA && NMMA <= NCOLS && NMMA % 16 == 0, "N covers both boards of a group");
+    static_assert(GUARD >= ROW_SLOTS + 1 && GUARD + NMMA - 1 + ROW_SLOTS + 1 < SPITCH, "every tap reads inside its chunk");
     static_assert(SCRATCH_BYTES <= BUF_BYTES && FEAT_BYTES <= BUF_BYTES, "aliases fit into buffer A");
     static_assert(A_COL0 + A_STAGES * A_STAGE_COLS == TMEM_COLS, "accumulators + the ring fill the allocation");
     static_assert(MIN_BLOCKS * (SMEM_BYTES + 1024) <= 233472, "MIN_BLOCKS CTAs per SM");
@@ -64,6 +68,8 @@
     auto bar_aempty = [&](int s) { return bars + 8u * (G::A_STAGES + s); };
     const uint32_t bar_act = bars + 8u * (2 * G::A_STAGES);
     const uint32_t bar_acc = bars + 8u * (2 * G::A_STAGES + 1);
+    auto bar_cls = [&](int g) { return bars + 8u * (2 * G::A_STAGES + 2 + g); };
+    auto bar_fix = [&](int g) { return bars + 8u * (2 * G::A_STAGES + 2 + G::NGRP + g); };
     volatile uint32_t* tmem_holder = reinterpret_cast<volatile uint32_t*>(smem + G::OFF_BARS + 8 * G::NBARS);
 
     const int warp = threadIdx.x >> 5, lane = threadIdx.x & 31;
@@ -73,6 +79,7 @@
         (int)blockIdx.x < units ? (units - (int)blockIdx.x + (int)gridDim.x - 1) / (int)gridDim.x : 0;
     const int NL = net.num_layers;
     const bool stamp = eval_timeline(a) && blockIdx.x == 0;
+    if (stamp && threadIdx.x == 0) eval_timeline(a)[4 * NL + 0] = clock64();
     unsigned long long* cta_rec = (eval_timeline(a) && blockIdx.x < 1024) ? eval_timeline(a) + 4 * NL + 16 + 3 * blockIdx.x : nullptr;
     if (cta_rec && threadIdx.x == 0) {
         unsigned smid;
@@ -92,6 +99,10 @@
         }
         mbar_init(bar_act, G::NGRP * G::EPI_WARPS);
         mbar_init(bar_acc, 1);
+        for (int g = 0; g < G::NGRP; ++g) {
+            mbar_init(bar_cls(g), 1);
+            mbar_init(bar_fix(g), G::EPI_WARPS);
+        }
         fence_mbar_init();
     }
     fence_proxy_async_smem();
@@ -100,6 +111,7 @@
     __syncthreads();
     tc_fence_after();
     const uint32_t tmem_base = *tmem_holder;
+    if (stamp && threadIdx.x == 0) eval_timeline(a)[4 * NL + 1] = clock64();
 
     if (warp < 4) {
         setmaxnreg_dec<G::PRODUCER_REGS>();
@@ -152,9 +164,9 @@
     } else if (warp >= G::MMA_WARP) {
         setmaxnreg_dec<G::MMA_REGS>();
         if (warp == G::MMA_WARP) {
-            constexpr uint32_t idesc = make_idesc_bf16_f32(128, G::NCOLS);
+            constexpr uint32_t idesc = make_idesc_bf16_f32(128, G::NMMA);
             constexpr uint32_t b_lbo = G::SPITCH * 16;
-            uint32_t slot = 0, phase = 0, act_phase = 0;
+            uint32_t slot = 0, phase = 0, act_phase = 0, fix_phase = 0;
             for (int p = 0; p < my_passes; ++p) {
                 for (int L = 0; L < NL; ++L) {
                     mbar_wait(bar_act, act_phase);
@@ -163,60 +175,66 @@
                     if (stamp && p == 0 && lane == 0) eval_timeline(a)[4 * L + 0] = clock64();
                     const bool head = (L == NL - 1);
                     const uint32_t in_buf = sbase + ((L & 1) ? G::OFF_BUF_A : G::OFF_BUF_B);
-                    const int ntaps = head ? 1 : 9;
-                    for (int kc = 0; kc < G::KC64; ++kc) {
-                        const int halves = block_steps(net, L, kc) / 2;
-                        for (int tap = 0; tap < ntaps; ++tap) {
-                            const int shift = head ? 0 : (tap / 3 - 1) * 10 + (tap % 3 - 1);
-                            const uint32_t b_base = in_buf + (uint32_t)((kc * 8 * G::SPITCH + G::GUARD + shift) * 16);
-                            if (halves == 2) {
-                                const uint32_t s0 = slot, s1 = (slot + 1) % G::A_STAGES;
-                                const uint32_t ph1 = s1 == 0 ? phase ^ 1u : phase;
-                                mbar_wait(bar_afull(s0), phase);
-                                mbar_wait(bar_afull(s1), ph1);
-                                tc_fence_after();
-                                if (elect_one()) {
-#pragma unroll
-                                    for (int h = 0; h < 2; ++h) {
-                                        const uint32_t a_base = tmem_base + G::A_COL0 + (h ? s1 : s0) * G::A_STAGE_COLS;
-#pragma unroll
-                                        for (int g = 0; g < G::NGRP; ++g) {
-                                            const uint32_t b_lo = smem_desc_lo(b_base + g * G::GRP_BYTES, b_lbo);
-#pragma unroll
-                                            for (int k2 = 0; k2 < 2; ++k2) {
-                                                const int k = 2 * h + k2;
-                                                umma_bf16_ts(tmem_base + g * G::NCOLS, a_base + k2 * 8,
-                                                             smem_desc_from(b_lo + (uint32_t)(2 * k * G::SPITCH), 128),
-                                                             idesc, (uint32_t)((kc | tap | k) != 0));
-                                            }
+                    const int ncls = head ? 1 : 3, ndh = head ? 1 : 3;
+                    for (int cls = 0; cls < ncls; ++cls) {
+                        for (int kc = 0; kc < G::KC64; ++kc) {
+                            const int halves = block_steps(net, L, kc) / 2;
+                            for (int i = 0; i < ndh; ++i) {
+                                const int tap = head ? 0 : dw_class_tap(cls, i);
+                                const int shift = head ? 0 : (tap / 3 - 1) * G::ROW_SLOTS + (tap % 3 - 1);
+                                const uint32_t b_base = in_buf + (uint32_t)((kc * 8 * G::SPITCH + G::GUARD + shift) * 16);
+                                const uint32_t acc0 = (uint32_t)((cls | kc | i) != 0);
+                                const bool fix_wait = cls > 0 && kc == 0 && i == 0;
+                                const bool fix_signal = !head && cls < 2 && kc == G::KC64 - 1 && i == ndh - 1;
+                                auto issue_group = [&](int g, bool first_stage, bool last_stage, uint32_t a_base,
+                                                       uint32_t b_off, int k0) {
+                                    if (fix_wait && first_stage) {
+                                        mbar_wait(bar_fix(g), fix_phase);
+                                        tc_fence_after();
+                                    }
+                                    const uint32_t b_lo = smem_desc_lo(b_base + g * G::GRP_BYTES, b_lbo) + b_off;
+#pragma unroll
+                                    for (int k2 = 0; k2 < 2; ++k2)
+                                        umma_bf16_ts(tmem_base + g * G::NCOLS, a_base + k2 * 8,
+                                                     smem_desc_from(b_lo + (uint32_t)(2 * k2 * G::SPITCH), 128), idesc,
+                                                     acc0 | (uint32_t)((k0 | k2) != 0));
+                                    if (fix_signal && last_stage) umma_commit(bar_cls(g));
+                                };
+                                if (halves == 2) {
+                                    const uint32_t s0 = slot, s1 = (slot + 1) % G::A_STAGES;
+                                    const uint32_t ph1 = s1 == 0 ? phase ^ 1u : phase;
+                                    mbar_wait(bar_afull(s0), phase);
+                                    mbar_wait(bar_afull(s1), ph1);
+                                    tc_fence_after();
+                                    if (elect_one()) {
+#pragma unroll
+                                        for (int h = 0; h < 2; ++h) {
+                                            const uint32_t a_base = tmem_base + G::A_COL0 + (h ? s1 : s0) * G::A_STAGE_COLS;
+#pragma unroll
+                                            for (int g = 0; g < G::NGRP; ++g)
+                                                issue_group(g, h == 0, h == 1, a_base, (uint32_t)(4 * h * G::SPITCH), 2 * h);
+                                            umma_commit(bar_aempty(h ? s1 : s0));
                                         }
-                                        umma_commit(bar_aempty(h ? s1 : s0));
+                                    }
+                                    __syncwarp();
+                                    slot = (slot + 2) % G::A_STAGES;
+                                    if (slot < 2) phase ^= 1u;
+                                } else {
+                                    for (int h = 0; h < halves; ++h) {
+                                        mbar_wait(bar_afull(slot), phase);
+                                        tc_fence_after();
+                                        if (elect_one()) {
+                                            const uint32_t a_base = tmem_base + G::A_COL0 + slot * G::A_STAGE_COLS;
+#pragma unroll
+                                            for (int g = 0; g < G::NGRP; ++g)
+                                                issue_group(g, h == 0, h == halves - 1, a_base, (uint32_t)(4 * h * G::SPITCH), 2 * h);
+                                            umma_commit(bar_aempty(slot));
+                                        }
+                                        __syncwarp();
+                                        if (++slot == G::A_STAGES) { slot = 0; phase ^= 1u; }
                                     }
                                 }
-                                __syncwarp();
-                                slot = (slot + 2) % G::A_STAGES;
-                                if (slot < 2) phase ^= 1u;
-                                continue;
-                            }
-                            for (int h = 0; h < halves; ++h) {
-                                mbar_wait(bar_afull(slot), phase);
-                                tc_fence_after();
-                                if (elect_one()) {
-                                    const uint32_t a_base = tmem_base + G::A_COL0 + slot * G::A_STAGE_COLS;
-#pragma unroll
-                                    for (int g = 0; g < G::NGRP; ++g) {
-                                        const uint32_t b_lo =
-                                            smem_desc_lo(b_base + g * G::GRP_BYTES, b_lbo) + (uint32_t)(4 * h * G::SPITCH);
-#pragma unroll
-                                        for (int k2 = 0; k2 < 2; ++k2)
-                                            umma_bf16_ts(tmem_base + g * G::NCOLS, a_base + k2 * 8,
-                                                         smem_desc_from(b_lo + (uint32_t)(2 * k2 * G::SPITCH), 128),
-                                                         idesc, (uint32_t)((kc | tap | h | k2) != 0));
-                                    }
-                                    umma_commit(bar_aempty(slot));
-                                }
-                                __syncwarp();
-                                if (++slot == G::A_STAGES) { slot = 0; phase ^= 1u; }
+                                if (fix_wait) fix_phase ^= 1u;
                             }
                         }
                     }
@@ -240,25 +258,55 @@
         float* red = reinterpret_cast<float*>(smem + G::OFF_RED + g * G::RED_BYTES);
         const uint32_t taddr = tmem_base + ((uint32_t)(q * 32) << 16) + g * G::NCOLS;
         const bool stamper = stamp && g == 0 && et == 0;
-        EpilogueMask<3> mask0, mask1;
+        EpilogueMask<3, 9> mask0, mask1;
         mask0.init(0, lane);
         mask1.init(96, lane);
-        uint32_t acc_phase = 0;
+        uint32_t acc_phase = 0, cls_phase = 0;
         for (int p = 0; p < my_passes; ++p) {
             const int b0 = ((int)blockIdx.x + p * (int)gridDim.x) * G::QPOS + g * G::NPOS;
 
-            expand_features<G::NPOS, G::SPITCH, G::GUARD, G::GRP_THREADS>(net, a, n_eff, b0, featS, gsmem + G::OFF_BUF_B, et, nullptr, bar);
+            expand_features<G::NPOS, G::SPITCH, G::GUARD, G::GRP_THREADS, G::POS_SLOTS, G::ROW_SLOTS>(
+                net, a, n_eff, b0, featS, gsmem + G::OFF_BUF_B, et, nullptr, bar);
             named_bar_sync(bar, G::GRP_THREADS);
             for (int i = et; i < G::FEAT_BYTES / 16; i += G::GRP_THREADS) featS[i] = make_uint4(0, 0, 0, 0);
             fence_proxy_async_smem();
             __syncwarp();
             if (lane == 0) mbar_arrive(bar_act);
+            if (stamper && p == 0) eval_timeline(a)[4 * NL + 2] = clock64();
 
             for (int L = 0; L < NL - 1; ++L) {
                 float bias[4];
 #pragma unroll
                 for (int k = 0; k < 4; ++k)
                     bias[k] = __ldg(net.bias + (size_t)L * C + 64 * (k >> 1) + 16 * q + 8 * (k & 1) + (lane >> 2));
+                uint32_t col0[2 * 9];
+                mbar_wait(bar_cls(g), cls_phase);
+                cls_phase ^= 1u;
+                tc_fence_after();
+#pragma unroll
+                for (int r = 0; r < 2 * 9; ++r) {
+                    const uint32_t c = taddr + (r / 9) * G::POS_SLOTS + (r % 9) * G::ROW_SLOTS;
+                    tmem_ld_32x32b_x1(c, col0[r]);
+                    tmem_st_32x32b_x1(c + 8, 0u);
+                }
+                tmem_ld_wait();
+                tmem_st_wait();
+                tc_fence_before();
+                __syncwarp();
+                if (lane == 0) mbar_arrive(bar_fix(g));
+                if (stamper && p == 0) eval_timeline(a)[4 * NL + 16 + 3 * 1024 + 2 * L] = clock64();
+                mbar_wait(bar_cls(g), cls_phase);
+                cls_phase ^= 1u;
+                tc_fence_after();
+#pragma unroll
+                for (int r = 0; r < 2 * 9; ++r)
+                    tmem_st_32x32b_x1(taddr + (r / 9) * G::POS_SLOTS + (r % 9) * G::ROW_SLOTS, col0[r]);
+                tmem_st_wait();
+                tc_fence_before();
+                __syncwarp();
+                if (lane == 0) mbar_arrive(bar_fix(g));
+                if (stamper && p == 0) eval_timeline(a)[4 * NL + 16 + 3 * 1024 + 2 * L + 1] = clock64();
+
                 mbar_wait(bar_acc, acc_phase);
                 acc_phase ^= 1u;
                 tc_fence_after();
@@ -288,11 +336,13 @@
             mbar_wait(bar_acc, acc_phase);
             acc_phase ^= 1u;
             tc_fence_after();
-            head_read<0>(taddr, hbias, hp, scratch, vbuf, lane);
-            head_read<96>(taddr + 96, hbias, hp, scratch, vbuf, lane);
+            head_read<0, 9>(taddr, hbias, hp, scratch, vbuf, lane);
+            head_read<96, 9>(taddr + 96, hbias, hp, scratch, vbuf, lane);
             tc_fence_before();
             named_bar_sync(bar, G::GRP_THREADS);
+            if (stamper && p == 0) eval_timeline(a)[4 * NL + 4] = clock64();
             heads_tail_small<G::NPOS, G::GRP_THREADS>(net, a, n_eff, b0, scratch, vbuf, red, et, bar);
+            if (stamper && p == 0) eval_timeline(a)[4 * NL + 7] = clock64();
             if (p + 1 < my_passes) {
                 for (int i = et; i < G::SCRATCH_BYTES / 16; i += G::GRP_THREADS)
                     reinterpret_cast<uint4*>(scratch)[i] = make_uint4(0, 0, 0, 0);
diff --git a/nshogi-engine_b200/csrc/umma.cuh b/nshogi-engine_b200/csrc/umma.cuh
--- a/nshogi-engine_b200/csrc/umma.cuh
+++ b/nshogi-engine_b200/csrc/umma.cuh
@@ -172,6 +172,12 @@
         ::"r"(taddr), "r"(v[0]), "r"(v[1]), "r"(v[2]), "r"(v[3]), "r"(v[4]), "r"(v[5]), "r"(v[6]), "r"(v[7]), "r"(v[8]),
           "r"(v[9]), "r"(v[10]), "r"(v[11]), "r"(v[12]), "r"(v[13]), "r"(v[14]), "r"(v[15])
         : "memory");
+}
+__device__ __forceinline__ void tmem_st_32x32b_x1(uint32_t taddr, uint32_t v) {
+    asm volatile("tcgen05.st.sync.aligned.32x32b.x1.b32 [%0], {%1};" ::"r"(taddr), "r"(v) : "memory");
+}
+__device__ __forceinline__ void tmem_ld_32x32b_x1(uint32_t taddr, uint32_t& v) {
+    asm volatile("tcgen05.ld.sync.aligned.32x32b.x1.b32 {%0}, [%1];" : "=r"(v) : "r"(taddr) : "memory");
 }
 template <int N>
 __device__ __forceinline__ void setmaxnreg_inc() {
diff --git a/nshogi-engine_b200/csrc/umma_probe.cu b/nshogi-engine_b200/csrc/umma_probe.cu
--- a/nshogi-engine_b200/csrc/umma_probe.cu
+++ b/nshogi-engine_b200/csrc/umma_probe.cu
@@ -125,12 +125,13 @@
     }
     __syncthreads();
     tc_fence_after();
-    for (int j = 0; j < N / 32; ++j) {
+    for (int j = 0; j < (N + 31) / 32; ++j) {
         uint32_t v[32];
         tmem_ld32(tmem_base + ((uint32_t)(warp * 32) << 16) + j * 32, v);
         tmem_ld_wait();
 #pragma unroll
-        for (int i = 0; i < 32; ++i) d[(size_t)threadIdx.x * N + j * 32 + i] = __uint_as_float(v[i]);
+        for (int i = 0; i < 32; ++i)
+            if (j * 32 + i < N) d[(size_t)threadIdx.x * N + j * 32 + i] = __uint_as_float(v[i]);
     }
     tc_fence_before();
     __syncthreads();
@@ -252,12 +253,13 @@
     }
     __syncthreads();
     tc_fence_after();
-    for (int j = 0; j < N / 32; ++j) {
+    for (int j = 0; j < (N + 31) / 32; ++j) {
         uint32_t v[32];
         tmem_ld32(tmem_base + ((uint32_t)(warp * 32) << 16) + j * 32, v);
         tmem_ld_wait();
 #pragma unroll
-        for (int i = 0; i < 32; ++i) d[(size_t)threadIdx.x * N + j * 32 + i] = __uint_as_float(v[i]);
+        for (int i = 0; i < 32; ++i)
+            if (j * 32 + i < N) d[(size_t)threadIdx.x * N + j * 32 + i] = __uint_as_float(v[i]);
     }
     tc_fence_before();
     __syncthreads();
@@ -340,7 +342,7 @@
     }
     __syncthreads();
     tc_fence_after();
-    for (int j = 0; j < N / 32; ++j) {
+    for (int j = 0; j < (N + 31) / 32; ++j) {
         uint32_t v[32];
         tmem_ld32(tmem_base + ((uint32_t)(warp * 32) << 16) + j * 32, v);
         tmem_ld_wait();
@@ -360,7 +362,7 @@
     const bool ts = layout >= 4;
     const bool pair = layout == 2 || layout == 3;
     const int lay = ts ? 0 : (layout & 1);
-    if (n_cols % 32 || n_cols < 32 || n_cols > 256 || k_elems % 64 || k_elems <= 0 || shift_rows < 0 ||
+    if (n_cols % (pair ? 32 : 16) || n_cols < 32 || n_cols > 256 || k_elems % 64 || k_elems <= 0 || shift_rows < 0 ||
         shift_rows > 64 || iters < 1 || layout < 0 || layout > 6) {
         set_error("umma_probe: bad arguments");
         return NSB_ERR_INVALID;
diff --git a/nshogi-engine_b200/csrc/weights.cc b/nshogi-engine_b200/csrc/weights.cc
--- a/nshogi-engine_b200/csrc/weights.cc
+++ b/nshogi-engine_b200/csrc/weights.cc
@@ -149,25 +149,33 @@
     return 9 * stem_steps(d.in_channels) + 2 * d.blocks * 9 * kc64 * 4 + kc64 * 4;
 }
 
-void pack_weights_ts(const nsb_net_desc& d, const float* blob, uint16_t* stream) {
+void pack_weights_ts(const nsb_net_desc& d, const float* blob, uint16_t* stream, TsOrder order) {
     const int C = d.channels, IN = d.in_channels, NB = d.blocks;
     const int kc64 = C / 64;
     const float* w = blob;
     uint16_t* t = stream;
     auto row_channel = [](int row) { return 64 * ((row >> 4) & 1) + 16 * (row >> 5) + (row & 15); };
     auto pack_conv = [&](const float* cw, int cin_real, int kblocks, int last_block_steps, bool stem = false) {
-        for (int kc = 0; kc < kblocks; ++kc)
-            for (int tap = 0; tap < 9; ++tap)
-                for (int k = 0; k < (kc + 1 == kblocks ? last_block_steps : 4); ++k) {
-                    for (int row = 0; row < 128; ++row)
-                        for (int e = 0; e < 16; ++e) {
-                            const int co = row_channel(row), ci = kc * 64 + k * 16 + e;
-                            const int src = stem ? stem_source_channel(ci, cin_real) : (ci < cin_real ? ci : -1);
-                            const float v = src >= 0 ? cw[((size_t)co * cin_real + src) * 9 + tap] : 0.f;
-                            t[row * 16 + e] = bf16_bits_rne(v);
-                        }
-                    t += 128 * 16;
-                }
+        auto pack_steps = [&](int kc, int tap) {
+            for (int k = 0; k < (kc + 1 == kblocks ? last_block_steps : 4); ++k) {
+                for (int row = 0; row < 128; ++row)
+                    for (int e = 0; e < 16; ++e) {
+                        const int co = row_channel(row), ci = kc * 64 + k * 16 + e;
+                        const int src = stem ? stem_source_channel(ci, cin_real) : (ci < cin_real ? ci : -1);
+                        const float v = src >= 0 ? cw[((size_t)co * cin_real + src) * 9 + tap] : 0.f;
+                        t[row * 16 + e] = bf16_bits_rne(v);
+                    }
+                t += 128 * 16;
+            }
+        };
+        if (order == TsOrder::kBlockMajor) {
+            for (int kc = 0; kc < kblocks; ++kc)
+                for (int tap = 0; tap < 9; ++tap) pack_steps(kc, tap);
+        } else {
+            for (int c = 0; c < 3; ++c)
+                for (int kc = 0; kc < kblocks; ++kc)
+                    for (int i = 0; i < 3; ++i) pack_steps(kc, dw_class_tap(c, i));
+        }
     };
     pack_conv(w, IN, 2, stem_steps(IN) - 4, true);
     w += (size_t)C * IN * 9 + C;
```

Measured after the change: 2.526 million, median of 6. -3.0%, worse.
